# Prunoideae/MitoFlex

Measured on AMD Instinct MI355X. Metric: filtered reads/sec on 5 Gbp PE150 k=31; achieved HBM GB/s vs peak, higher is better.
Workload: dtype u64

## Files before the change

### mitoflex_amd/csrc/mf_api.cpp

```cpp
#include "../../include/mitofilter.h"
#include "mf_common.h"
#include "mf_host.h"
#include "mf_kernels.h"
#include "mf_pipeline.h"
#include "mf_synth.h"
#include "mf_coldtrace.h"
#include "mf_api_internal.h"
#include "mf_devingest.h"

#include <hip/hip_runtime.h>
#include <algorithm>
#include <atomic>
#include <chrono>
#include <map>
#include <mutex>
#include <stdarg.h>
#include <stdio.h>
#include <stdlib.h>
#include <string.h>
#include <sys/stat.h>
#include <string>
#include <thread>
#include <vector>

using namespace mf;

static thread_local std::string t_err;
const std::string &mf_thread_error() { return t_err; }
int fail(int code, const char *fmt, ...)
{
    char buf[1024];
    va_list ap; va_start(ap, fmt); vsnprintf(buf, sizeof buf, fmt, ap); va_end(ap);
    t_err = buf;
    return code;
}

static std::mutex g_ctx_mu;
static std::atomic<int> g_expect_files{0};
static std::map<int, DevCtx> g_ctx;

static int fake_devices()
{
#ifdef MF_TEST_HOOKS
    static const int n = [] { const char *v = getenv("MF_FAKE_DEVICES"); const int k = v ? atoi(v) : 0; return k > 0 && k <= 64 ? k : 0; }();
    return n;
#else
    return 0;
#endif
}
static int physical_count() { int n = 0; return hipGetDeviceCount(&n) == hipSuccess ? n : 0; }
int phys(int device) { const int n = physical_count(); return fake_devices() && n > 0 ? device % n : device; }

int get_ctx(int device, DevCtx **out, int lane)
{
    std::lock_guard<std::mutex> lk(g_ctx_mu);
    auto it = g_ctx.find(device + 4096 * lane);
    if (it != g_ctx.end()) { *out = &it->second; hipError_t e = hipSetDevice(phys(device)); if (e != hipSuccess) return fail(MF_E_HIP, "hipSetDevice(%d): %s", device, hipGetErrorString(e)); return MF_OK; }
    int n = 0;
    mf::cold_mark("get_ctx: a new device context");
    hipError_t e = hipGetDeviceCount(&n);
    mf::cold_mark("get_ctx: HIP runtime answered (initialised)");
    if (e != hipSuccess || n <= 0) return fail(MF_E_NO_DEVICE, "no HIP device visible (%s); libmitofilter_hip has no CPU fallback", e == hipSuccess ? "count=0" : hipGetErrorString(e));
    const int logical = fake_devices() ? fake_devices() : n;
    if (device < 0 || device >= logical) return fail(MF_E_ARG, "device %d out of range (have %d)", device, logical);
    const int pdev = phys(device);
    hipDeviceProp_t prop;
    HIPCHK(hipGetDeviceProperties(&prop, pdev));
    if (strncmp(prop.gcnArchName, "gfx950", 6) != 0)
        return fail(MF_E_NO_DEVICE, "device %d is %s; this library carries gfx950 (MI355X) code only", device, prop.gcnArchName);
    HIPCHK(hipSetDevice(pdev));
    DevCtx c; c.device = device; c.n_cu = prop.multiProcessorCount;
    HIPCHK(hipStreamCreateWithFlags(&c.stream, hipStreamNonBlocking));
    mf::cold_mark("get_ctx: stream made");
    g_ctx[device + 4096 * lane] = c;
    *out = &g_ctx[device + 4096 * lane];
    if (g_expect_files && lane == 0) mf::ingest_prefetch(device);
    return MF_OK;
}

static int ensure_pipeline_streams(DevCtx *c)
{
    { std::lock_guard<std::mutex> lk(g_ctx_mu); if (c->stream2) return MF_OK; }
    int lo = 0, hi = 0;
    hipStream_t s2 = nullptr, s3 = nullptr, s4 = nullptr;
    hipError_t e = hipDeviceGetStreamPriorityRange(&lo, &hi);
    if (e == hipSuccess) e = hipStreamCreateWithPriority(&s2, hipStreamNonBlocking, hi);
    if (e == hipSuccess) e = hipStreamCreateWithPriority(&s4, hipStreamNonBlocking, hi);
    if (e == hipSuccess) e = hipStreamCreateWithFlags(&s3, hipStreamNonBlocking);
    bool publish = e == hipSuccess;
    if (publish) {
        std::lock_guard<std::mutex> lk(g_ctx_mu);
        if (c->stream2) publish = false;
        else { c->stream3 = s3; c->stream4 = s4; c->stream2 = s2; }
    }
    if (!publish) { for (hipStream_t s : {s2, s4, s3}) if (s) (void)hipStreamDestroy(s); }
    if (e != hipSuccess) return fail(MF_E_HIP, "creating the streams of a pipelined call failed: %s", hipGetErrorString(e));
    return MF_OK;
}

struct TablesGuard {
    DevTables *t;
    ~TablesGuard() { if (t) t->release(); }
};
struct EventList {
    std::vector<hipEvent_t> ev;
    hipError_t create(size_t n) { ev.reserve(n); for (size_t i = 0; i < n; i++) { hipEvent_t e; hipError_t r = hipEventCreate(&e); if (r != hipSuccess) return r; ev.push_back(e); } return hipSuccess; }
    ~EventList() { for (hipEvent_t e : ev) hipEventDestroy(e); }
};

static int host_threads()
{
    const char *v = getenv("MF_HOST_THREADS");
    const int n = v && *v ? atoi(v) : (int)std::thread::hardware_concurrency();
    return n < 1 ? 1 : n;
}

static uint32_t env_u32(const char *name, uint32_t dflt)
{
    const char *v = getenv(name);
    return v && *v ? (uint32_t)strtoul(v, nullptr, 10) : dflt;
}

struct PassOptions {
    std::atomic<int> pass{0};
    std::atomic<int> adapt{1};
    std::atomic<int> finish_streams{0};
    std::atomic<int> screen_streams{2};
    std::atomic<int> split_pipe{1};
    std::atomic<int> exact_co{0};
    std::atomic<int> front{-1};
    std::atomic<int> front2_log2b{0};
    std::atomic<int> s8_finish{-1};
    std::atomic<int> canon{-1};
    std::atomic<int> front3_log2b{-1};
    std::atomic<int> depth_index{0};
};
static PassOptions g_opt;
static int set_option(const char *name, const char *value)
{
    const std::string n = name ? name : "", v = value ? value : "";
    if (n == "pass") { if (v == "" || v == "default") g_opt.pass = 0; else if (v == "split") g_opt.pass = 1; else if (v == "serial") g_opt.pass = 2; else return -1; return 0; }
    char *end = nullptr; const long x = strtol(v.c_str(), &end, 10);
    if (v.empty() || *end) return -1;
    if (n == "expect_files") g_expect_files = x != 0;
    else if (n == "short_lived") mf::ingest_short_lived(x != 0);
    else if (n == "adapt") g_opt.adapt = x != 0;
    else if (n == "finish_streams") { if (x < 0 || x > 2) return -1; g_opt.finish_streams = (int)x; }
    else if (n == "screen_streams") { if (x < 1 || x > 2) return -1; g_opt.screen_streams = (int)x; }
    else if (n == "split_pipe") g_opt.split_pipe = x != 0;
    else if (n == "exact_co") g_opt.exact_co = x != 0;
    else if (n == "front") { if (x < -1 || x > 4) return -1; g_opt.front = (int)x; }
    else if (n == "front2_log2b") { if (x != 0 && (x < 6 || x > 24)) return -1; g_opt.front2_log2b = (int)x; }
    else if (n == "s8_finish") { if (x < -1 || x > 1) return -1; g_opt.s8_finish = (int)x; }
    else if (n == "canon") { if (x < -1 || x > 1) return -1; g_opt.canon = (int)x; }
    else if (n == "front3_log2b") { if (x < -1 || (x > 0 && x < 6) || x > 27) return -1; g_opt.front3_log2b = (int)x; }
    else if (n == "depth_index") { if (x < 0 || x > 1) return -1; g_opt.depth_index = (int)x; }
    else return -1;
    return 0;
}
static void options_from_env_once()
{
    static const bool done = [] {
        const char *k = getenv("MF_ENV_KNOBS");
        if (k && k[0] == '1') {
            static const char *const pairs[][2] = {{"pass", "MF_PASS"}, {"adapt", "MF_ADAPT"}, {"finish_streams", "MF_FINISH_STREAMS"}, {"screen_streams", "MF_SCREEN_STREAMS"},
                                                   {"split_pipe", "MF_SPLIT_PIPE"}, {"exact_co", "MF_EXACT_CO"},
                                                   {"front", "MF_FRONT"}, {"front2_log2b", "MF_FRONT2_LOG2B"}, {"front3_log2b", "MF_FRONT3_LOG2B"}, {"canon", "MF_CANON"}, {"s8_finish", "MF_S8_FINISH"},
                                                   {"depth_index", "MF_DEPTH_INDEX"}};
            for (auto &p : pairs) { const char *v = getenv(p[1]); if (v && *v && set_option(p[0], v) != 0) fprintf(stderr, "libmitofilter_hip: %s=%s is not a value of option '%s' (ignored)\n", p[1], v, p[0]); }
        }
        return true;
    }();
    (void)done;
}
int depth_index_option() { return g_opt.depth_index.load(); }

int build_on_device(mf_kmerset *ks, int device, DevTables **out)
{
    std::lock_guard<std::mutex> lk(ks->mu);
    auto it = ks->dev.find(device);
    if (it != ks->dev.end()) { *out = &it->second; return MF_OK; }
    DevCtx *ctx; int rc = get_ctx(device, &ctx); if (rc) return rc;
    hipStream_t st = ctx->stream;
    if (ks->kind == MF_KIND_PROTEIN) {
        const ProtBaitHost &P = ks->pbait;
        DevTables T; TablesGuard guard{&T}; DevScratch tmp;
        uint8_t *d_aa = nullptr, *d_run = nullptr; unsigned long long *d_cnt = nullptr;
        HIPCHK(tmp.alloc(d_aa, P.aa.size())); HIPCHK(tmp.alloc(d_run, P.runlen.size()));
        HIPCHK(hipMemcpyAsync(d_aa, P.aa.data(), P.aa.size(), hipMemcpyHostToDevice, st));
        HIPCHK(hipMemcpyAsync(d_run, P.runlen.data(), P.runlen.size(), hipMemcpyHostToDevice, st));
        HIPCHK(dev_malloc(&T.keys, ks->slots * sizeof(uint64_t)));
        HIPCHK(hipMemsetAsync(T.keys, 0xFF, ks->slots * sizeof(uint64_t), st));
        HIPCHK(launch_build_ptable(d_aa, d_run, P.total, ks->k, T.keys, ks->slots, st));
        HIPCHK(dev_malloc(&T.kbloom, sizeof(uint32_t) << ks->kb_log2w));
        HIPCHK(hipMemsetAsync(T.kbloom, 0, sizeof(uint32_t) << ks->kb_log2w, st));
        HIPCHK(launch_build_pbits(T.keys, ks->slots, T.kbloom, ks->kb_log2w, st));
        HIPCHK(dev_malloc(&T.plut, sizeof ks->codon_lut));
        HIPCHK(hipMemcpyAsync(T.plut, ks->codon_lut, sizeof ks->codon_lut, hipMemcpyHostToDevice, st));
        HIPCHK(tmp.alloc(d_cnt, 16)); HIPCHK(hipMemsetAsync(d_cnt, 0, 16, st));
        HIPCHK(launch_count_keys(T.keys, ks->slots, 1, nullptr, 0, d_cnt, st));
        unsigned long long cnt[2] = {0, 0};
        HIPCHK(hipMemcpyAsync(cnt, d_cnt, 16, hipMemcpyDeviceToHost, st));
        HIPCHK(hipStreamSynchronize(st));
        T.n_keys = cnt[0];
        KmerSetView &V = T.view;
        V.k = ks->k; V.kw = 1; V.slot_mask = ks->slots - 1; V.keys = T.keys;
        V.kb_log2w = ks->kb_log2w; V.kbloom = T.kbloom; V.kb_co_log2w = ks->kb_log2w; V.kbloom_co = T.kbloom;
        V.prot = 1; V.kb_in_lds = ks->kb_in_lds ? 1u : 0u; V.plut = T.plut;
        ks->dev[device] = T; guard.t = nullptr;
        *out = &ks->dev[device];
        return MF_OK;
    }
    const BaitHost &B = ks->bait;
    DevTables T; TablesGuard guard{&T}; DevScratch tmp;
    uint32_t *d_words = nullptr; uint8_t *d_run = nullptr; uint32_t *d_pos = nullptr, *d_flag = nullptr;
    unsigned long long *d_cnt = nullptr;
    HIPCHK(tmp.alloc(d_words, B.words.size() * 4));
    HIPCHK(tmp.alloc(d_run, B.runlen.size()));
    HIPCHK(hipMemcpyAsync(d_words, B.words.data(), B.words.size() * 4, hipMemcpyHostToDevice, st));
    HIPCHK(hipMemcpyAsync(d_run, B.runlen.data(), B.runlen.size(), hipMemcpyHostToDevice, st));
    const size_t key_bytes = ks->slots * ks->kw * sizeof(uint64_t);
    HIPCHK(dev_malloc(&T.keys, key_bytes));
    HIPCHK(hipMemsetAsync(T.keys, 0xFF, key_bytes, st));
    if (ks->kw == 2) {
        if (B.total > 0xFFFFFFF0ull) return fail(MF_E_ARG, "bait longer than 2^32 bases is not supported for k > 32");
        HIPCHK(tmp.alloc(d_pos, ks->slots * 4));
        HIPCHK(hipMemsetAsync(d_pos, 0xFF, ks->slots * 4, st));
    }
    HIPCHK(tmp.alloc(d_flag, 4)); HIPCHK(hipMemsetAsync(d_flag, 0, 4, st));
    HIPCHK(tmp.alloc(d_cnt, 16)); HIPCHK(hipMemsetAsync(d_cnt, 0, 16, st));
    BaitView bv{d_words, B.total, d_run};
    HIPCHK(launch_build_table(bv, ks->k, ks->kw, T.keys, ks->slots, d_pos, st));
    if (ks->geom.s) {
        HIPCHK(dev_malloc(&T.bloom, ks->screen_words() * 4));
        HIPCHK(hipMemsetAsync(T.bloom, 0, ks->screen_words() * 4, st));
        HIPCHK(dev_malloc(&T.stab, (size_t)ks->stab_slots * 4));
        HIPCHK(hipMemsetAsync(T.stab, 0xFF, (size_t)ks->stab_slots * 4, st));
        if (ks->front_mode) {
            HIPCHK(dev_malloc(&T.front2, (size_t)16 << ks->f2_log2b));
            HIPCHK(hipMemsetAsync(T.front2, 0, (size_t)16 << ks->f2_log2b, st));
            if (ks->f3_log2b) {
                HIPCHK(dev_malloc(&T.front3, (size_t)16 << ks->f3_log2b));
                HIPCHK(hipMemsetAsync(T.front3, 0, (size_t)16 << ks->f3_log2b, st));
            }
        }
        if (ks->front_mode == 4) {
            HIPCHK(dev_malloc(&T.pre, sizeof(uint32_t) << ks->pre_log2w));
            HIPCHK(hipMemsetAsync(T.pre, 0, sizeof(uint32_t) << ks->pre_log2w, st));
        }
        HIPCHK(launch_build_screen(bv, ks->geom.s, T.bloom, ks->bloom_log2w, ks->stage2_log2w, T.stab, ks->stab_slots, d_flag,
                                   T.front2, ks->f2_log2b, T.front3, ks->f3_log2b, T.pre, ks->pre_log2w, ks->canon != 0, st));
    }
    HIPCHK(dev_malloc(&T.kbloom, sizeof(uint32_t) << ks->kb_log2w));
    HIPCHK(hipMemsetAsync(T.kbloom, 0, sizeof(uint32_t) << ks->kb_log2w, st));
    HIPCHK(launch_build_kbloom(T.keys, ks->slots, ks->kw, T.kbloom, ks->kb_log2w, st));
    if (ks->kb_log2w > KB_CO_LOG2W) {
        HIPCHK(dev_malloc(&T.kbloom_co, sizeof(uint32_t) << KB_CO_LOG2W));
        HIPCHK(hipMemsetAsync(T.kbloom_co, 0, sizeof(uint32_t) << KB_CO_LOG2W, st));
        HIPCHK(launch_build_kbloom(T.keys, ks->slots, ks->kw, T.kbloom_co, KB_CO_LOG2W, st));
    }
    HIPCHK(launch_count_keys(T.keys, ks->slots, ks->kw, T.stab, T.stab ? ks->stab_slots : 0, d_cnt, st));
    unsigned long long cnt[2] = {0, 0}; uint32_t flag = 0;
    HIPCHK(hipMemcpyAsync(cnt, d_cnt, 16, hipMemcpyDeviceToHost, st));
    HIPCHK(hipMemcpyAsync(&flag, d_flag, 4, hipMemcpyDeviceToHost, st));
    HIPCHK(hipStreamSynchronize(st));
    T.n_keys = cnt[0]; T.n_smers = cnt[1] + (flag ? 1 : 0);
    KmerSetView &V = T.view;
    V.k = ks->k; V.kw = ks->kw; V.slot_mask = ks->slots - 1; V.keys = T.keys;
    V.kb_log2w = ks->kb_log2w; V.kbloom = T.kbloom;
    V.kb_co_log2w = T.kbloom_co ? KB_CO_LOG2W : ks->kb_log2w; V.kbloom_co = T.kbloom_co ? T.kbloom_co : T.kbloom;
    V.s = ks->geom.s; V.stride = ks->geom.stride;
    V.smask = ks->geom.s >= 16 ? 0xFFFFFFFFu : ((1u << (2 * ks->geom.s)) - 1);
    V.bloom_log2w = ks->bloom_log2w; V.stage2_log2w = ks->stage2_log2w; V.bloom = T.bloom;
    V.stab_mask = ks->stab_slots ? ks->stab_slots - 1 : 0; V.stab = T.stab; V.stab_has_ones = flag;
    V.canon = (uint32_t)ks->canon;
    V.s8_finish = ks->s8_finish ? 1u : 0u;
    V.front_mode = ks->front_mode; V.f2_log2b = ks->f2_log2b; V.f3_log2b = ks->f3_log2b; V.front2 = T.front2; V.front3 = T.front3;
    V.pre_log2w = ks->pre_log2w; V.pre = T.pre;
    V.use_stab = (T.n_smers / 2 * STAGE2_K > ((uint64_t)32 << ks->stage2_log2w) * 7 / 10) ? 1u : 0u;
#ifdef MF_DEBUG_KNOBS
    if (getenv("MF_USE_STAB")) V.use_stab = 1u;
#endif
    ks->dev[device] = T; guard.t = nullptr;
    *out = &ks->dev[device];
    return MF_OK;
}

static int kmerset_new(const char *text, size_t len, int k, int device, mf_kmerset **out)
{
    if (!out) return fail(MF_E_ARG, "out is NULL");
    *out = nullptr;
    if (k < 11 || k > 63) return fail(MF_E_ARG, "k=%d out of range [11,63]", k);
    mf_kmerset *ks = new (std::nothrow) mf_kmerset();
    if (!ks) return fail(MF_E_NOMEM, "out of memory");
    ks->k = k; ks->kw = k > 32 ? 2 : 1;
    parse_bait_fasta(text, len, ks->bait);
    ks->n_windows = ks->bait.n_windows(k);
    ks->slots = table_slots_for(ks->n_windows);
    {
        uint32_t lg = 8;
        while (lg < 14 && (1ull << lg) < 2 * ks->n_windows) lg++;
        ks->kb_log2w = env_u32("MF_KBLOOM_LOG2W", lg);
        if (ks->kb_log2w < 8) ks->kb_log2w = 8;
        if (ks->kb_log2w > 15) ks->kb_log2w = 15;
    }
    ks->geom = screen_geom_for(k);
#ifdef MF_DEBUG_KNOBS
    if (getenv("MF_NO_SCREEN")) ks->geom = ScreenGeom{0, 0};
#endif
    if (ks->geom.s) {
        const uint64_t bound = 2 * ks->bait.n_swindows(ks->geom.s);
        uint32_t lg = 8;
        while (lg < 15 && (1ull << lg) < bound) lg++;
        ks->bloom_log2w = env_u32("MF_BLOOM_LOG2W", lg);
        if (ks->bloom_log2w < 8) ks->bloom_log2w = 8;
        if (ks->bloom_log2w > 15) ks->bloom_log2w = 15;
        uint32_t lg2 = 6;
        while (lg2 < 13 && (32ull << lg2) < 8 * bound) lg2++;
        ks->stage2_log2w = env_u32("MF_STAGE2_LOG2W", lg2);
        if (ks->stage2_log2w < 6) ks->stage2_log2w = 6;
        if (ks->stage2_log2w > 13) ks->stage2_log2w = 13;
        uint64_t ss = 1024; while (ss < 2 * bound) ss <<= 1;
        if (ss > (1ull << 31)) { delete ks; return fail(MF_E_ARG, "bait too large for the s-mer screen table"); }
        ks->stab_slots = (uint32_t)ss;
        options_from_env_once();
        uint64_t per_lds_block = bound >> (ks->bloom_log2w - 2);
        ks->s8_finish = ks->geom.stride == 8 && per_lds_block > 5;
        {
            const bool want = g_opt.canon < 0 ? per_lds_block > (ks->geom.stride == 8 ? 18u : 14u) : g_opt.canon == 1;
            ks->canon = !want ? 0 : ks->geom.s == 16 ? 1 : 2;
        }
        const uint64_t keys_bound = ks->canon ? bound / 2 : bound;
        per_lds_block = keys_bound >> (ks->bloom_log2w - 2);
        const uint64_t mode1_max = ks->geom.stride == 8 ? 18 : 26;
        int mode = per_lds_block <= 9 ? 0 : per_lds_block <= mode1_max ? 1 : 2;
        if (ks->geom.stride == 16 && per_lds_block > 5 && per_lds_block <= (ks->canon ? 12u : 14u)) mode = 3;
        if (mode == 2 && keys_bound <= (1u << 21)) mode = 4;
        if (g_opt.front >= 0) mode = g_opt.front;
        ks->front_mode = (uint32_t)mode;
        ks->pre_log2w = mode == 4 ? 15 : 0;
        if (mode) {
            uint32_t lg = 10;
            while (lg < FRONT2_MAX_LOG2B && (4ull << lg) < keys_bound) lg++;
            while (lg < FRONT2_MAX_LOG2B + 2 && (keys_bound >> lg) > 32) lg++;
            if (g_opt.front2_log2b > 0) lg = (uint32_t)g_opt.front2_log2b;
            ks->f2_log2b = lg;
            uint32_t lg3 = 0;
            if ((keys_bound >> lg) > 12) { lg3 = lg + 1; while (lg3 < 27 && (4ull << lg3) < keys_bound) lg3++; }
            if (g_opt.front3_log2b >= 0) lg3 = (uint32_t)g_opt.front3_log2b;
            ks->f3_log2b = (mode == 2 || mode == 4) ? lg3 : 0;
        }
    }
    DevTables *T; int rc = build_on_device(ks, device, &T);
    if (rc) { delete ks; return rc; }
    *out = ks;
    return MF_OK;
}

static int protset_new(const char *text, size_t len, int kp, int genetic_code, int device, mf_kmerset **out)
{
    if (!out) return fail(MF_E_ARG, "out is NULL");
    *out = nullptr;
    if (kp < 4 || kp > 12) return fail(MF_E_ARG, "peptide k=%d out of range [4,12]", kp);
    mf_kmerset *ks = new (std::nothrow) mf_kmerset();
    if (!ks) return fail(MF_E_NOMEM, "out of memory");
    ks->kind = MF_KIND_PROTEIN; ks->k = kp; ks->kw = 1; ks->genetic_code = genetic_code;
    if (!codon_lut_for(genetic_code, kp, ks->codon_lut)) { delete ks; return fail(MF_E_ARG, "genetic code %d is not supported (1, 2, 3, 4, 5, 9, 11, 13, 14, 21)", genetic_code); }
    parse_bait_protein(text, len, ks->pbait);
    ks->n_windows = ks->pbait.n_windows(kp);
    ks->slots = table_slots_for(ks->n_windows);
    {
        uint32_t lg = 8;
        while (lg < 14 && (1ull << lg) < 2 * ks->n_windows) lg++;
        ks->kb_in_lds = ks->n_windows <= (1u << 17);
        if (!ks->kb_in_lds) { lg = 15; while (lg < 24 && (32ull << lg) < 16 * ks->n_windows) lg++; }
        if (getenv("MF_KBLOOM_LOG2W")) {
            lg = env_u32("MF_KBLOOM_LOG2W", lg);
            if (lg < 8) lg = 8;
            if (lg > 24) lg = 24;
            ks->kb_in_lds = lg <= 14;
        }
        ks->kb_log2w = lg;
    }
    DevTables *T; int rc = build_on_device(ks, device, &T);
    if (rc) { delete ks; return rc; }
    *out = ks;
    return MF_OK;
}

extern "C" {

int mf_abi_version(void) { return MF_ABI_VERSION; }
const char *mf_last_error(void) { return t_err.c_str(); }

int mf_device_count(void)
{
    int n = 0;
    hipError_t e = hipGetDeviceCount(&n);
    if (e == hipErrorNoDevice) return 0;
    if (e != hipSuccess) return fail(MF_E_HIP, "hipGetDeviceCount: %s", hipGetErrorString(e));
    return n > 0 && fake_devices() ? fake_devices() : n;
}

int mf_device_name(int device, char *buf, size_t buflen)
{
    if (!buf || !buflen) return fail(MF_E_ARG, "bad buffer");
    hipDeviceProp_t prop;
    HIPCHK(hipGetDeviceProperties(&prop, phys(device)));
    snprintf(buf, buflen, "%s (%s, %d CUs)", prop.name, prop.gcnArchName, prop.multiProcessorCount);
    return MF_OK;
}

int mf_device_synchronize(int device)
{
    HIPCHK(hipSetDevice(phys(device)));
    HIPCHK(hipDeviceSynchronize());
    return MF_OK;
}

int mf_kmerset_build_from_text(const char *text, size_t len, int k, int device, mf_kmerset **out)
{
    if (!text && len) return fail(MF_E_ARG, "fasta_text is NULL");
    return kmerset_new(text ? text : "", len, k, device, out);
}

int mf_kmerset_build_from_fasta(const char *path, int k, int device, mf_kmerset **out)
{
    if (!path) return fail(MF_E_ARG, "fasta_path is NULL");
    std::vector<char> buf; std::string err;
    if (!slurp_file(path, buf, err)) return fail(MF_E_IO, "%s", err.c_str());
    return kmerset_new(buf.data(), buf.size(), k, device, out);
}

int mf_kmerset_build_protein_from_text(const char *text, size_t len, int kp, int genetic_code, int device, mf_kmerset **out)
{
    if (!text && len) return fail(MF_E_ARG, "protein_fasta_text is NULL");
    return protset_new(text ? text : "", len, kp, genetic_code, device, out);
}

int mf_kmerset_build_protein_from_fasta(const char *path, int kp, int genetic_code, int device, mf_kmerset **out)
{
    if (!path) return fail(MF_E_ARG, "protein_fasta_path is NULL");
    std::vector<char> buf; std::string err;
    if (!slurp_file(path, buf, err)) return fail(MF_E_IO, "%s", err.c_str());
    return protset_new(buf.data(), buf.size(), kp, genetic_code, device, out);
}

int mf_kmerset_info(const mf_kmerset *ks, mf_kmerset_info_t *info)
{
    if (!ks || !info) return fail(MF_E_ARG, "NULL argument");
    memset(info, 0, sizeof *info);
    info->k = ks->k; info->key_words = ks->kw; info->slots = ks->slots; info->n_windows = ks->n_windows;
    info->screen_s = ks->geom.s; info->screen_stride = ks->geom.stride;
    info->bloom_words = ks->geom.s ? (uint32_t)ks->screen_words() : 0; info->smer_slots = ks->stab_slots;
    if (!ks->dev.empty()) { info->n_keys = ks->dev.begin()->second.n_keys; info->n_smers = ks->dev.begin()->second.n_smers; }
    info->kind = ks->kind; info->genetic_code = ks->genetic_code;
    info->front_mode = ks->front_mode; info->front2_log2_blocks = ks->front_mode ? ks->f2_log2b : 0; info->front3_log2_blocks = ks->f3_log2b; info->canonical_screen = ks->canon ? 1u : 0u;
    return MF_OK;
}

int mf_kmerset_export(const mf_kmerset *ks_, int device, uint64_t *keys_out, size_t n_u64)
{
    mf_kmerset *ks = const_cast<mf_kmerset *>(ks_);
    if (!ks || !keys_out) return fail(MF_E_ARG, "NULL argument");
    if (n_u64 < ks->slots * ks->kw) return fail(MF_E_ARG, "keys_out too small: need %llu u64", (unsigned long long)(ks->slots * ks->kw));
    DevTables *T; int rc = build_on_device(ks, device, &T); if (rc) return rc;
    HIPCHK(hipMemcpy(keys_out, T->keys, ks->slots * ks->kw * sizeof(uint64_t), hipMemcpyDeviceToHost));
    return MF_OK;
}

int mf_kmerset_free(mf_kmerset *ks)
{
    if (!ks) return MF_OK;
    for (auto &kv : ks->dev) {
        if (hipSetDevice(phys(kv.first)) == hipSuccess) kv.second.release();
    }
    delete ks;
    return MF_OK;
}

}

void reads_release(mf_reads *r)
{
    if (!r) return;
    if (hipSetDevice(phys(r->device)) == hipSuccess) {
        hipFree(r->d_words); hipFree(r->d_offsets); hipFree(r->d_npos); hipFree(r->d_has_n);
        for (int i = 0; i < NSETS; i++) hipFree(r->d_cand[i]);
        for (int i = 0; i < NSETS; i++) {
            hipFree(r->d_bits[i]); hipFree(r->d_recs[i]); hipFree(r->d_rec_counts[i]); if (r->d_counters[i]) hipHostFree(r->d_counters[i]);
            if (r->ev_screen[i]) hipEventDestroy(r->ev_screen[i]);
            if (i < 2 && r->ev_call[i]) hipEventDestroy(r->ev_call[i]);
            if (r->ev_finish[i]) hipEventDestroy(r->ev_finish[i]);
        }
        hipFree(r->d_hits); hipFree(r->d_npos_blk); hipFree(r->d_off_blk);
        hipFree(r->d_alist); hipFree(r->d_assign); hipFree(r->d_apairs); hipFree(r->d_acnt);
        hipFree(r->d_rpos); hipFree(r->d_rtot); hipFree(r->d_rsum); hipFree(r->d_place); hipFree(r->d_score); hipFree(r->d_keep);
        hipFree(r->d_align); hipFree(r->d_awork);
    }
    delete r;
}

#define RCHK(call) do { hipError_t e_ = (call); if (e_ != hipSuccess) return fail(MF_E_HIP, "%s failed: %s", #call, hipGetErrorString(e_)); } while (0)
int reads_reserve(mf_reads *r, bool reuse, uint64_t n_words, uint64_t n_reads, uint32_t uniform_len, uint64_t npos_cap, DevCtx *ctx)
{
    const uint64_t padded = padded_words_for(n_words);
    RCHK(dev_reserve(r->d_words, r->cap_words, padded * 4, reuse));
    if (padded > n_words) RCHK(hipMemsetAsync(r->d_words + n_words, 0, (padded - n_words) * 4, ctx->stream));
    if (!uniform_len) RCHK(dev_reserve(r->d_offsets, r->cap_offsets, (n_reads + 1) * 8, reuse));
    RCHK(dev_reserve(r->d_npos, r->cap_npos, (npos_cap ? npos_cap : 1) * 8, reuse));
    return MF_OK;
}

int reads_finish(mf_reads *r, bool reuse, uint64_t n_words, uint64_t n_reads, uint64_t total_bases, uint32_t uniform_len, uint64_t n_npos, DevCtx *ctx)
{
    hipStream_t st = ctx->stream;
    const uint64_t padded = padded_words_for(n_words);
    if (n_npos >= 0xFFFFFFFFull) return fail(MF_E_ARG, "more than 2^32 invalid bases in one read set");
    const uint64_t n_blk = (total_bases >> NPOS_BLK_SHIFT) + 3;
    RCHK(dev_reserve(r->d_npos_blk, r->cap_npos_blk, n_blk * 4, reuse));
    RCHK(launch_build_npos_blk(r->d_npos, n_npos, n_blk, r->d_npos_blk, st));
    if (!uniform_len) {
        if (n_reads >= 0x7FFFFFFFull) return fail(MF_E_ARG, "more than 2^31 reads in one ragged read set");
        const uint64_t n_oblk = (total_bases >> OFF_BLK_SHIFT) + 2;
        RCHK(dev_reserve(r->d_off_blk, r->cap_off_blk, n_oblk * 8, reuse));
        RCHK(launch_build_off_blk(r->d_offsets, n_reads, n_oblk, r->d_off_blk, st));
    }
    r->bitmap_bytes = ((n_reads + 31) / 32 + 64) * 4;
    if (r->bitmap_bytes > r->cap_bitmap || !r->d_has_n) {
        size_t c[2 + NSETS] = {};
        uint32_t **bm[2 + NSETS] = {&r->d_has_n, &r->d_cand[0]};
        for (int i = 0; i < NSETS; i++) bm[2 + i] = &r->d_bits[i];
        size_t least = ~(size_t)0;
        for (int i = 0; i < 2 + NSETS; i++) {
            if (*bm[i]) { hipFree(*bm[i]); *bm[i] = nullptr; }
            RCHK(dev_reserve(*bm[i], c[i], r->bitmap_bytes, reuse));
            if (c[i] < least) least = c[i];
        }
        r->cap_bitmap = least;
        for (int i = 1; i < NSETS; i++) { hipFree(r->d_cand[i]); r->d_cand[i] = nullptr; }
    }
    RCHK(hipMemsetAsync(r->d_has_n, 0, r->bitmap_bytes, st));
    RCHK(hipMemsetAsync(r->d_cand[0], 0, r->bitmap_bytes, st));
    r->cand_clean[0] = true;
    for (int i = 1; i < NSETS; i++) r->cand_clean[i] = false;
    for (int i = 0; i < NSETS; i++) {
        if (!r->d_counters[i]) RCHK(hipHostMalloc(reinterpret_cast<void **>(&r->d_counters[i]), TallyLayout::bytes(), hipHostMallocDefault));
        memset(r->d_counters[i], 0, TallyLayout::bytes());
        RCHK(hipMemsetAsync(r->d_bits[i], 0, r->bitmap_bytes, st));
        if (!r->ev_screen[i]) RCHK(hipEventCreate(&r->ev_screen[i]));
        if (!r->ev_finish[i]) RCHK(hipEventCreate(&r->ev_finish[i]));
    }
    r->cur = 0;
    ReadsView &V = r->v;
    V = ReadsView{};
    V.words = r->d_words; V.n_words = n_words; V.n_vec = (padded - 16) / 4;
    V.offsets = uniform_len ? nullptr : r->d_offsets; V.off_blk = uniform_len ? nullptr : r->d_off_blk; V.uniform_len = uniform_len; V.n_reads = n_reads; V.total_bases = total_bases;
    V.len_magic = uniform_len > 1 ? ~0ULL / uniform_len + 1 : 0;
    V.len_magic32 = (uniform_len > 1 && uniform_len <= 4096) ? 0xFFFFFFFFu / uniform_len + 1 : 0;
    V.npos = r->d_npos; V.n_npos = n_npos; V.npos_blk = r->d_npos_blk; V.has_n = r->d_has_n;
    {
        uint64_t grid = screen_grid_for(V, ctx->n_cu, 4), cap = screen_rec_cap_for(V, ctx->n_cu, 4);
        for (int key : {8, 16}) { const uint64_t g2 = screen_grid_for(V, ctx->n_cu, key), c2 = screen_rec_cap_for(V, ctx->n_cu, key); if (g2 * c2 > grid * cap) cap = (g2 * c2 + grid - 1) / (grid ? grid : 1); }
        size_t c0 = r->cap_recs, c1 = r->cap_rec_counts;
        RCHK(dev_reserve(r->d_recs[0], c0, (grid * cap ? grid * cap : 1) * 16, reuse));
        RCHK(dev_reserve(r->d_rec_counts[0], c1, (grid ? grid : 1) * 4, reuse));
        if (c0 != r->cap_recs || c1 != r->cap_rec_counts)
            for (int i = 1; i < NSETS; i++) { hipFree(r->d_recs[i]); hipFree(r->d_rec_counts[i]); r->d_recs[i] = nullptr; r->d_rec_counts[i] = nullptr; }
        r->cap_recs = c0; r->cap_rec_counts = c1;
    }
    RCHK(launch_mark_has_n(V, r->d_has_n, st));
    RCHK(hipStreamSynchronize(st));
    return MF_OK;
}

static int reads_fill(mf_reads *r, bool reuse, const uint32_t *words, uint64_t n_words, bool already_padded, const uint64_t *offsets,
                      uint64_t n_reads, uint64_t total_bases, uint32_t uniform_len, const uint64_t *npos, uint64_t n_npos,
                      DevCtx *ctx)
{
    hipStream_t st = ctx->stream;
    int rc = reads_reserve(r, reuse, n_words, n_reads, uniform_len, n_npos, ctx);
    if (rc) return rc;
    const uint64_t copied = already_padded ? padded_words_for(n_words) : n_words;
    if (copied) RCHK(hipMemcpyAsync(r->d_words, words, copied * 4, hipMemcpyHostToDevice, st));
    if (!uniform_len) RCHK(hipMemcpyAsync(r->d_offsets, offsets, (n_reads + 1) * 8, hipMemcpyHostToDevice, st));
    if (n_npos) RCHK(hipMemcpyAsync(r->d_npos, npos, n_npos * 8, hipMemcpyHostToDevice, st));
    return reads_finish(r, reuse, n_words, n_reads, total_bases, uniform_len, n_npos, ctx);
}
#undef RCHK

static int reads_upload(const uint32_t *words, uint64_t n_words, bool already_padded, const uint64_t *offsets, uint64_t n_reads,
                        uint64_t total_bases, uint32_t uniform_len, const uint64_t *npos, uint64_t n_npos, int device,
                        mf_reads **out)
{
    DevCtx *ctx; int rc = get_ctx(device, &ctx); if (rc) return rc;
    mf_reads *r = new (std::nothrow) mf_reads();
    if (!r) return fail(MF_E_NOMEM, "out of memory");
    r->device = device;
    rc = reads_fill(r, false, words, n_words, already_padded, offsets, n_reads, total_bases, uniform_len, npos, n_npos, ctx);
    if (rc) { reads_release(r); return rc; }
    *out = r;
    return MF_OK;
}

extern "C" {

int mf_reads_from_packed(const uint32_t *words, const uint64_t *offsets, uint64_t n_reads,
                         const uint64_t *npos, uint64_t n_npos, int device, mf_reads **out)
{
    if (!out) return fail(MF_E_ARG, "out is NULL");
    *out = nullptr;
    if (!offsets) return fail(MF_E_ARG, "offsets is NULL");
    if (n_npos && !npos) return fail(MF_E_ARG, "npos is NULL");
    if (offsets[0] != 0) return fail(MF_E_ARG, "offsets[0] must be 0");
    for (uint64_t i = 0; i < n_reads; i++) if (offsets[i + 1] < offsets[i]) return fail(MF_E_ARG, "offsets must be non-decreasing");
    for (uint64_t i = 1; i < n_npos; i++) if (npos[i] <= npos[i - 1]) return fail(MF_E_ARG, "npos must be strictly ascending");
    const uint64_t total = offsets[n_reads];
    if (n_npos && npos[n_npos - 1] >= total) return fail(MF_E_ARG, "npos entry beyond the last base");
    const uint64_t n_words = (total + 15) / 16;
    if (n_words && !words) return fail(MF_E_ARG, "words is NULL");
    return reads_upload(words, n_words, false, offsets, n_reads, total, detect_uniform_len(offsets, n_reads), npos, n_npos, device, out);
}

int mf_reads_from_fastq(const char *path, int device, mf_reads **out)
{
    if (!out || !path) return fail(MF_E_ARG, "NULL argument");
    *out = nullptr;
    std::vector<char> buf; std::string err;
    if (!slurp_file(path, buf, err)) return fail(MF_E_IO, "%s", err.c_str());
    std::vector<FqRec> recs; parse_fastq(buf.data(), buf.size(), recs);
    PackedHost P; pack_records(recs.data(), recs.size(), host_threads(), P);
    return reads_upload(P.words.data(), P.n_words, true, P.offsets.data(), recs.size(), P.offsets.back(), P.uniform_len,
                        P.npos.data(), P.npos.size(), device, out);
}

int mf_reads_synth(uint64_t n_reads, uint32_t read_len, uint64_t seed, const char *bait_text, size_t bait_len,
                   uint32_t mito_ppm, uint32_t sub_ppm, uint32_t n_read_ppm, uint32_t n_base_ppm, int device, mf_reads **out,
                   uint32_t **host_words_out, uint64_t *host_n_words_out, uint64_t **host_npos_out, uint64_t *host_n_npos_out)
{
    return mf_reads_synth_ex(n_reads, read_len, seed, bait_text, bait_len, mito_ppm, sub_ppm, n_read_ppm, n_base_ppm, 0, 0, 0, device, out,
                             host_words_out, host_n_words_out, host_npos_out, host_n_npos_out);
}

int mf_reads_synth_ex(uint64_t n_reads, uint32_t read_len, uint64_t seed, const char *bait_text, size_t bait_len,
                      uint32_t mito_ppm, uint32_t sub_ppm, uint32_t n_read_ppm, uint32_t n_base_ppm,
                      uint32_t msat_ppm, uint32_t numt_ppm, uint32_t numt_div_ppm, int device, mf_reads **out,
                      uint32_t **host_words_out, uint64_t *host_n_words_out, uint64_t **host_npos_out, uint64_t *host_n_npos_out)
{
    if (!out) return fail(MF_E_ARG, "out is NULL");
    *out = nullptr;
    if (read_len == 0) return fail(MF_E_ARG, "read_len must be > 0");
    BaitHost B; parse_bait_fasta(bait_text ? bait_text : "", bait_text ? bait_len : 0, B);
    SynthOut S;
    std::string err;
    SynthExtra extra; extra.msat_ppm = msat_ppm; extra.numt_ppm = numt_ppm; extra.numt_div_ppm = numt_div_ppm;
    if (!synth_reads(n_reads, read_len, seed, B, mito_ppm, sub_ppm, n_read_ppm, n_base_ppm,
                     host_threads(), S, err, extra)) return fail(MF_E_ARG, "%s", err.c_str());
    int rc = reads_upload(S.words.data(), S.n_words, true, nullptr, n_reads, n_reads * (uint64_t)read_len, read_len,
                          S.npos.data(), S.npos.size(), device, out);
    if (rc) return rc;
    if (host_words_out) {
        *host_words_out = (uint32_t *)malloc(S.words.size() * 4);
        if (!*host_words_out) return fail(MF_E_NOMEM, "out of memory");
        memcpy(*host_words_out, S.words.data(), S.words.size() * 4);
        if (host_n_words_out) *host_n_words_out = S.n_words;
    }
    if (host_npos_out) {
        *host_npos_out = (uint64_t *)malloc((S.npos.size() + 1) * 8);
        if (!*host_npos_out) return fail(MF_E_NOMEM, "out of memory");
        memcpy(*host_npos_out, S.npos.data(), S.npos.size() * 8);
        if (host_n_npos_out) *host_n_npos_out = S.npos.size();
    }
    return MF_OK;
}

void mf_free_host(void *p) { free(p); }

int mf_reads_info(const mf_reads *r, mf_reads_info_t *info)
{
    if (!r || !info) return fail(MF_E_ARG, "NULL argument");
    info->n_reads = r->v.n_reads; info->total_bases = r->v.total_bases; info->n_invalid = r->v.n_npos;
    info->uniform_len = r->v.uniform_len; info->device = r->device;
    return MF_OK;
}

int mf_reads_free(mf_reads *r) { reads_release(r); return MF_OK; }

}

static uint64_t algorithmic_bytes(const ReadsView &V) { return (2 * V.total_bases + 7) / 8 + (V.n_reads + 7) / 8; }

static unsigned long long *tally_of(mf_reads *r, int set) { return r->tally_override ? r->tally_override : r->d_counters[set]; }
static int clean_cand(mf_reads *r, int q, hipStream_t st)
{
    if (!r->d_cand[q]) { size_t c = 0; HIPCHK(dev_reserve(r->d_cand[q], c, r->cap_bitmap, false)); r->cand_clean[q] = false; }
    if (!r->cand_clean[q]) { HIPCHK(hipMemsetAsync(r->d_cand[q], 0, r->bitmap_bytes, st)); r->cand_clean[q] = true; }
    return MF_OK;
}
static int enqueue_pass(mf_reads *r, const KmerSetView &S, uint32_t thr, int mode, bool count_all, DevCtx *ctx, hipEvent_t *ev, bool overlap, bool more = false)
{
    options_from_env_once();
    const PassKnobs knobs{g_opt.pass, g_opt.finish_streams, g_opt.screen_streams, g_opt.split_pipe, g_opt.exact_co, g_opt.s8_finish};
    const PassInputs in{(int)S.prot, (int)S.s, (int)S.stride, (int)S.kw, (int)S.k, (int)S.s8_finish, thr, mode, count_all, overlap, more, r->fb, r->flip, r->cur, NSETS};
    const PassPlan P = plan_pass(knobs, in);
    const int n_cu = ctx->n_cu, q = P.q; const bool finish = P.kind == PassKind::FINISH;
    hipStream_t const streams[] = {ctx->stream, ctx->stream2, ctx->stream3, ctx->stream4}, ss = streams[(int)P.screen_on], sf = streams[(int)P.later_on];
    const hipEvent_t done = P.two_streams ? r->ev_finish[q] : nullptr;
    KernelTiming tm[3]; const KernelTiming *t0 = nullptr, *t1 = nullptr, *t2 = nullptr;
    if (ev) { for (int i = 0; i < 3; i++) tm[i] = KernelTiming{ev[2 * i], ev[2 * i + 1]}; t0 = &tm[0]; t1 = &tm[1]; t2 = &tm[2]; }
    if (P.screen) {
        size_t c0 = 0, c1 = 0;
        if (!r->d_recs[q]) { HIPCHK(dev_reserve(r->d_recs[q], c0, r->cap_recs, false)); HIPCHK(dev_reserve(r->d_rec_counts[q], c1, r->cap_rec_counts, false)); }
        if (P.wait_prev_finish) HIPCHK(hipStreamWaitEvent(ss, r->ev_finish[q], 0));
        if (P.needs_cand && !finish) { const int rc = clean_cand(r, q, ss); if (rc) return rc; }
        KernelTiming scr_done{nullptr, r->ev_screen[q]};
        HIPCHK(launch_screen(r->v, S, r->d_recs[q], r->d_rec_counts[q], n_cu, ss, t0 ? t0 : (P.two_streams ? &scr_done : nullptr),
                             P.screen_clears_bits ? r->d_bits[q] : nullptr, P.screen_clears_bits ? ((r->v.n_reads + 31) / 32 + 3) / 4 : 0));
        if (P.two_streams) { if (t0) HIPCHK(hipEventRecord(r->ev_screen[q], ss)); HIPCHK(hipStreamWaitEvent(sf, r->ev_screen[q], 0)); }
    }
#ifdef MF_DEBUG_KNOBS
    static const uint32_t nofin = env_u32("MF_NO_FINISH", 0);
    if (finish && nofin) { if (done) HIPCHK(hipEventRecord(done, sf)); } else
#endif
    if (P.kind == PassKind::PROTEIN) HIPCHK(launch_pfilter(r->v, S, thr, count_all, r->d_bits[P.q_out], r->d_hits, tally_of(r, P.q_out), n_cu, sf, t2));
    else if (finish) {
        if (P.exact_behind_finish) { const int rc = clean_cand(r, q, sf); if (rc) return rc; }
        uint32_t *const cand = P.exact_behind_finish ? r->d_cand[q] : nullptr;
        HIPCHK(launch_finish(r->v, S, r->d_recs[q], r->d_rec_counts[q], r->d_bits[q], tally_of(r, q), n_cu, sf, t2, cand ? nullptr : done, cand));
        if (cand) HIPCHK(launch_exact(r->v, S, cand, 1, false, r->d_bits[q], nullptr, tally_of(r, q) + TallyLayout::region(2), n_cu, sf, nullptr, P.exact_coresident, done, true));
    } else {
        uint32_t *const cand = P.needs_cand ? r->d_cand[q] : nullptr;
        if (P.screen) HIPCHK(launch_mark(r->v, S, r->d_recs[q], r->d_rec_counts[q], cand, n_cu, sf, t1));
        HIPCHK(launch_exact(r->v, S, cand, thr, count_all, r->d_bits[P.q_out], P.kind == PassKind::ONE_STREAM ? r->d_hits : nullptr, tally_of(r, P.q_out), n_cu, sf, t2, P.exact_coresident, done));
    }
    r->flip = P.flip; r->cur = P.cur; r->sample_pass = P.sample_pass;
    return MF_OK;
}

int filter_common(const mf_kmerset *ks_, const mf_reads *reads_, uint32_t thr, int mode, uint32_t *out_bits,
                  uint32_t *hits_out, int steps, mf_filter_stats_t *stats, uint64_t *pass_per_step)
{
    mf_kmerset *ks = const_cast<mf_kmerset *>(ks_);
    mf_reads *r = const_cast<mf_reads *>(reads_);
    if (!ks || !r) return fail(MF_E_ARG, "NULL handle");
    if (thr < 1) return fail(MF_E_ARG, "threshold must be >= 1");
    if (mode != MF_MODE_SCREENED && mode != MF_MODE_EXHAUSTIVE) return fail(MF_E_ARG, "bad mode %d", mode);
    if (steps < 1) return fail(MF_E_ARG, "steps must be >= 1");
    static const bool trace = getenv("MF_TRACE") != nullptr;
    const auto tp0 = std::chrono::steady_clock::now();
    auto lap = [&](const char *what) { if (trace) fprintf(stderr, "[mf trace] %-10s %8.1f us\n", what, std::chrono::duration<double, std::micro>(std::chrono::steady_clock::now() - tp0).count()); };
    DevCtx *ctx; int rc = get_ctx(r->device, &ctx, r->lane); if (rc) return rc;
    DevTables *T; rc = build_on_device(ks, r->device, &T); if (rc) return rc;
    hipStream_t st = ctx->stream;
    const bool count_all = hits_out != nullptr;
    lap("setup");
    if (count_all) {
        HIPCHK(dev_reserve(r->d_hits, r->cap_hits, (r->v.n_reads ? r->v.n_reads : 1) * 4, false));
        HIPCHK(hipMemsetAsync(r->d_hits, 0, (r->v.n_reads ? r->v.n_reads : 1) * 4, st));
    }
    int stride = steps <= 8 ? 1 : (int)env_u32("MF_EVENT_STRIDE", 8);
    if (stride < 1) stride = 1;
    const int n_sampled = stride > steps ? 0 : (steps + stride - 1) / stride;
    EventList events;
    HIPCHK(events.create((size_t)n_sampled * 6));
    hipEvent_t *ev = events.ev.data();
    for (int i = 0; i < 2; i++) if (!r->ev_call[i]) HIPCHK(hipEventCreate(&r->ev_call[i]));
    const hipEvent_t e_begin = r->ev_call[0], e_end = r->ev_call[1];
    lap("events");
    const bool pipelined = steps > 1;
    if (pipelined) { rc = ensure_pipeline_streams(ctx); if (rc) return rc; }
    HIPCHK(hipEventRecord(e_begin, st));
    if (pipelined) HIPCHK(hipStreamWaitEvent(ctx->stream3, e_begin, 0));
    struct PinnedTmp { unsigned long long *p = nullptr; ~PinnedTmp() { if (p) (void)hipHostFree(p); } } all_tallies;
    if (pass_per_step) {
        HIPCHK(hipHostMalloc(reinterpret_cast<void **>(&all_tallies.p), (size_t)steps * TallyLayout::bytes(), hipHostMallocDefault));
        memset(all_tallies.p, 0, (size_t)steps * TallyLayout::bytes());
    }
    struct OverrideReset { mf_reads *r; ~OverrideReset() { r->tally_override = nullptr; } } override_reset{r};
    for (int i = 0; i < steps; i++) {
        if (pass_per_step) r->tally_override = all_tallies.p + (size_t)i * TallyLayout::words();
        rc = enqueue_pass(r, T->view, thr, mode, count_all, ctx, n_sampled && i % stride == 0 ? &ev[(size_t)(i / stride) * 6] : nullptr, pipelined, i + 1 < steps);
        if (rc) return rc;
    }
    lap("enqueued");
    for (int i = 0; i < NSETS; i++) HIPCHK(hipStreamWaitEvent(st, r->ev_finish[i], 0));
    HIPCHK(hipEventRecord(e_end, st));
    const int regions = r->sample_pass ? TallyLayout::REGIONS : 1;
    const unsigned long long *part = pass_per_step ? all_tallies.p + (size_t)(steps - 1) * TallyLayout::words() : r->d_counters[r->cur];
    if (out_bits) HIPCHK(hipMemcpyAsync(out_bits, r->d_bits[r->cur], ((r->v.n_reads + 31) / 32) * 4, hipMemcpyDeviceToHost, st));
    if (hits_out && r->v.n_reads) HIPCHK(hipMemcpyAsync(hits_out, r->d_hits, r->v.n_reads * 4, hipMemcpyDeviceToHost, st));
    lap("copies");
    HIPCHK(hipStreamSynchronize(st));
    lap("synced");
    const TallyLayout::Totals cnt = TallyLayout::sum(part, regions);
    for (int s = 0; pass_per_step && s < steps; s++) pass_per_step[s] = TallyLayout::sum(all_tallies.p + (size_t)s * TallyLayout::words(), regions).pass;
    if (g_opt.adapt && !T->view.prot && mode == MF_MODE_SCREENED && T->view.s > 0) r->fb = adapt_after_call(r->fb, r->sample_pass, cnt.cand, r->v.n_reads);
    if (stats) {
        memset(stats, 0, sizeof *stats);
        float tot = 0, scr = 0, mrk = 0, exa = 0, t;
        HIPCHK(hipEventElapsedTime(&tot, e_begin, e_end));
        const bool prot = T->view.prot != 0, screened = !prot && mode == MF_MODE_SCREENED && T->view.s > 0;
        for (int i = 0; i < n_sampled; i++) {
            hipEvent_t *e = &ev[(size_t)i * 6];
            auto span = [&](hipEvent_t a, hipEvent_t b) { t = 0; if (hipEventElapsedTime(&t, a, b) != hipSuccess) { (void)hipGetLastError(); t = 0; } return t; };
            if (screened) { scr += span(e[0], e[1]); mrk += span(e[2], e[3]); }
            exa += span(e[4], e[5]);
        }
        stats->n_reads = r->v.n_reads; stats->n_pass = cnt.pass;
        stats->n_candidates = (mode == MF_MODE_SCREENED && T->view.s > 0) ? cnt.cand : r->v.n_reads;
        stats->ms_total = tot / steps;
        if (n_sampled) { stats->ms_screen = scr / n_sampled; stats->ms_mark = mrk / n_sampled; stats->ms_exact = exa / n_sampled; }
        stats->algorithmic_bytes = algorithmic_bytes(r->v);
    }
    lap("stats");
    return MF_OK;
}

extern "C" {

int mf_filter(const mf_kmerset *ks, const mf_reads *reads, uint32_t threshold, int mode,
              uint32_t *out_bits, uint32_t *hits_out, mf_filter_stats_t *stats)
{
    if (!out_bits && !hits_out && !stats) return fail(MF_E_ARG, "nothing to return: out_bits, hits_out and stats are all NULL");
    return filter_common(ks, reads, threshold, mode, out_bits, hits_out, 1, stats);
}

int mf_filter_resident(const mf_kmerset *ks, const mf_reads *reads, uint32_t threshold, int mode, int steps,
                       mf_filter_stats_t *stats)
{
    return filter_common(ks, reads, threshold, mode, nullptr, nullptr, steps, stats);
}

int mf_filter_resident_passes(const mf_kmerset *ks, const mf_reads *reads, uint32_t threshold, int mode, int steps,
                              uint64_t *n_pass_per_step, mf_filter_stats_t *stats)
{
    if (!n_pass_per_step) return fail(MF_E_ARG, "n_pass_per_step is NULL");
    return filter_common(ks, reads, threshold, mode, nullptr, nullptr, steps, stats, n_pass_per_step);
}

int mf_filter_packed(const mf_kmerset *ks, int device, const uint32_t *words, const uint64_t *offsets, uint64_t n_reads,
                     const uint64_t *npos, uint64_t n_npos, uint32_t threshold, uint32_t *out_bits)
{
    if (!out_bits) return fail(MF_E_ARG, "out_bits is NULL");
    mf_reads *r = nullptr;
    int rc = mf_reads_from_packed(words, offsets, n_reads, npos, n_npos, device, &r);
    if (rc) return rc;
    rc = filter_common(ks, r, threshold, MF_MODE_SCREENED, out_bits, nullptr, 1, nullptr);
    reads_release(r);
    return rc;
}

}

static thread_local mf_ingest_stats_t t_ingest_stats;
static thread_local bool t_ingest_stats_valid = false;
static void publish_ingest_stats(const IngestStats &is)
{
    mf_ingest_stats_t &o = t_ingest_stats;
    memset(&o, 0, sizeof o);
    o.path = MF_INGEST_PATH_DEVICE; o.n_devices = is.n_devices; o.consumers = is.consumers;
    o.input_bytes = is.input_bytes; o.text_bytes = is.text_bytes; o.records = is.records;
    o.seconds = is.seconds; o.decode_busy_seconds = is.decode_busy_seconds;
    o.pool_bytes_peak = is.pool_bytes_peak; o.device_bytes_peak = is.device_bytes_peak;
    o.chunks = is.chunks; o.chunks_linked = is.chunks_linked; o.gaps = is.gaps; o.gap_bytes = is.gap_bytes;
    t_ingest_stats_valid = true;
}

int filter_fastq_files_on(mf_kmerset *ks, const char *fq1, const char *fq2, const char *out1, const char *out2,
                          uint32_t threshold, int pair_mode, const int *devices, int n_devices, uint64_t *kept, uint64_t *total, PassReport *report)
{
    if (!ks || !fq1 || !out1) return fail(MF_E_ARG, "NULL argument");
    if ((fq2 == nullptr) != (out2 == nullptr)) return fail(MF_E_ARG, "fq2 and out2 must be given together");
    if (pair_mode != MF_PAIR_EITHER && pair_mode != MF_PAIR_BOTH) return fail(MF_E_ARG, "bad pair_mode %d", pair_mode);
    if (threshold < 1) return fail(MF_E_ARG, "threshold must be >= 1");
    const int have = mf_device_count();
    if (have <= 0) return fail(MF_E_NO_DEVICE, "no HIP device visible; libmitofilter_hip has no CPU fallback");
    if (!devices || n_devices < 1) return fail(MF_E_ARG, "empty device list");
    for (int i = 0; i < n_devices; i++) {
        if (devices[i] < 0 || devices[i] >= have) return fail(MF_E_ARG, "device %d out of range (have %d)", devices[i], have);
        for (int j = 0; j < i; j++) if (devices[j] == devices[i]) return fail(MF_E_ARG, "device %d listed twice", devices[i]);
    }

    {
        const char *ing = getenv("MF_INGEST");
        const bool force = ing && strcmp(ing, "device") == 0, any_gz = has_gz_ext(fq1) || (fq2 && has_gz_ext(fq2));
        bool big_plain = false;
        if (!any_gz && fq1) {
            struct stat sb; uint64_t sum = 0; bool regular = true;
            for (const char *f : {fq1, fq2}) if (f) { if (stat(f, &sb) == 0 && S_ISREG(sb.st_mode)) sum += (uint64_t)sb.st_size; else regular = false; }
            const char *mn = getenv("MF_INGEST_PLAIN_MIN_MB");
            big_plain = regular && sum > 0 && sum >= (mn && *mn ? strtoull(mn, nullptr, 10) : 0) << 20;
        }
        if (!(ing && strcmp(ing, "host") == 0) && (force || any_gz || big_plain)) {
            std::string derr; IngestStats is;
            const int drc = run_device_ingest(ks, fq1, fq2, out1, out2, threshold, pair_mode == MF_PAIR_BOTH, devices, n_devices, kept, total, derr, &is, report);
            if (drc == MF_OK) {
                publish_ingest_stats(is);
                return MF_OK;
            }
            if (drc != MF_DEVINGEST_DECLINED) return fail(drc, "%s", derr.c_str());
            if (report) report->restart();
            if (getenv("MF_PIPE_TIMING")) fprintf(stderr, "[mf device ingest] declined%s%s: the host pipeline takes the input\n", derr.empty() ? "" : ": ", derr.c_str());
        }
    }
    for (int i = 1; i < n_devices; i++)
        if (devices[i] != devices[0] + i) return fail(MF_E_ARG, "the host pipeline (plain files, pipes, BGZF) takes a run of consecutive devices; got %d after %d", devices[i], devices[i - 1]);
    const int dev_base = devices[0];
    const int hw = (int)std::thread::hardware_concurrency();
    int pack_threads = hw - 4 - n_devices; if (pack_threads < 1) pack_threads = 1; if (pack_threads > 64) pack_threads = 64;
    pack_threads = (int)env_u32("MF_PACK_THREADS", (uint32_t)pack_threads);
    if (pack_threads < 1) pack_threads = 1;
    const uint64_t batch_reads = env_u32("MF_BATCH_READS", 2000000);
    set_dma_allocator([](size_t bytes) -> void * { void *p = nullptr; return hipHostMalloc(&p, bytes, hipHostMallocPortable) == hipSuccess ? p : nullptr; },
                      [](void *p) { (void)hipHostFree(p); });
    struct DmaScope { ~DmaScope() { set_dma_allocator(nullptr, nullptr); } } dma_scope;
    const int lanes = (int)env_u32("MF_WORKERS_PER_DEVICE", 2) < 1 ? 1 : (int)env_u32("MF_WORKERS_PER_DEVICE", 2);
    const int n_workers = n_devices * lanes;
    std::vector<mf_reads *> arena((size_t)n_workers, nullptr);
    if (report) report->held.assign((size_t)n_workers, nullptr);
    BatchFilterFn fn = [ks, threshold, n_devices, dev_base, report, &arena](int worker, const PackedHost &P, uint64_t n, std::vector<uint32_t> &bits, std::string &err) -> int {
        bits.assign((n + 31) / 32 + 1, 0);
        if (report) report->held[(size_t)worker] = nullptr;
        if (n == 0) return MF_OK;
        const int device = dev_base + worker % n_devices, lane = worker / n_devices;
        DevCtx *ctx; int rc = get_ctx(device, &ctx, lane);
        if (rc == MF_OK && !arena[worker]) {
            arena[worker] = new (std::nothrow) mf_reads();
            if (!arena[worker]) rc = fail(MF_E_NOMEM, "out of memory"); else { arena[worker]->device = device; arena[worker]->lane = lane; }
        }
        if (rc == MF_OK)
            rc = reads_fill(arena[worker], true, P.words.data(), P.n_words, true, P.offsets.data(), n, P.offsets[n], P.uniform_len,
                            P.npos.data(), P.npos.size(), ctx);
        if (rc == MF_OK) rc = filter_common(ks, arena[worker], threshold, MF_MODE_SCREENED, bits.data(), nullptr, 1, nullptr);
        if (rc != MF_OK) err = t_err;
        else if (report) report->held[(size_t)worker] = arena[worker];
        return rc;
    };
    PipelineStats ps; std::string perr;
    const auto t_pipe0 = std::chrono::steady_clock::now();
    const int rc = run_fastq_pipeline(fq1, fq2, out1, out2, pair_mode == MF_PAIR_BOTH, n_workers, pack_threads, batch_reads, fn, ps, perr, report);
    {
        mf_ingest_stats_t &o = t_ingest_stats;
        memset(&o, 0, sizeof o);
        o.path = MF_INGEST_PATH_HOST; o.n_devices = n_devices; o.records = ps.total * (fq2 ? 2 : 1);
        o.seconds = std::chrono::duration<double>(std::chrono::steady_clock::now() - t_pipe0).count();
        t_ingest_stats_valid = rc == MF_OK;
    }
    {
        const auto t0 = std::chrono::steady_clock::now();
        for (mf_reads *a : arena) reads_release(a);
        if (getenv("MF_PIPE_TIMING"))
            fprintf(stderr, "[mf pipeline] device buffers released in %.3f s\n", std::chrono::duration<double>(std::chrono::steady_clock::now() - t0).count());
    }
    if (rc != MF_OK) return fail(rc, "%s", perr.c_str());
    if (kept) *kept = ps.kept;
    if (total) *total = ps.total;
    return MF_OK;
}

extern "C" {

int mf_filter_fastq_files(mf_kmerset *ks, const char *fq1, const char *fq2, const char *out1, const char *out2,
                          uint32_t threshold, int pair_mode, int n_devices, uint64_t *kept, uint64_t *total)
{
    const int have = mf_device_count();
    if (have <= 0) return fail(MF_E_NO_DEVICE, "no HIP device visible; libmitofilter_hip has no CPU fallback");
    if (n_devices < 1) n_devices = 1;
    if (n_devices > have) n_devices = have;
    std::vector<int> devs((size_t)n_devices);
    for (int i = 0; i < n_devices; i++) devs[(size_t)i] = i;
    return filter_fastq_files_on(ks, fq1, fq2, out1, out2, threshold, pair_mode, devs.data(), n_devices, kept, total, nullptr);
}

int mf_filter_fastq_files_on(mf_kmerset *ks, const char *fq1, const char *fq2, const char *out1, const char *out2,
                             uint32_t threshold, int pair_mode, const int *devices, int n_devices, uint64_t *kept, uint64_t *total)
{
    return filter_fastq_files_on(ks, fq1, fq2, out1, out2, threshold, pair_mode, devices, n_devices, kept, total, nullptr);
}

int mf_set_option(const char *name, const char *value)
{
    options_from_env_once();
    if (set_option(name, value) != 0) return fail(MF_E_ARG, "unknown option or value: %s=%s (options: pass=default|split|serial, adapt=0|1, finish_streams=0|1|2, screen_streams=1|2, split_pipe=0|1, exact_co=0|1, front=-1|0|1|2|3|4, canon=-1|0|1, s8_finish=-1|0|1, front2_log2b=0|6..24, front3_log2b=-1|0|6..27, expect_files=0|1, short_lived=0|1, depth_index=0|1)", name ? name : "(null)", value ? value : "(null)");
    return MF_OK;
}

int mf_last_ingest_stats(mf_ingest_stats_t *out)
{
    if (!out) return fail(MF_E_ARG, "NULL argument");
    if (!t_ingest_stats_valid) return fail(MF_E_ARG, "no file-level call has succeeded on this thread");
    *out = t_ingest_stats;
    return MF_OK;
}

int mf_release_cached(uint64_t *bytes)
{
    const size_t n = mf::release_cached_device_memory(true);
    if (bytes) *bytes = n;
    return MF_OK;
}

int mf_h2d_bandwidth(int device, size_t bytes, int reps, double *gb_per_s)
{
    if (!gb_per_s || !bytes || reps < 1) return fail(MF_E_ARG, "bad argument");
    DevCtx *ctx; int rc = get_ctx(device, &ctx); if (rc) return rc;
    void *h = nullptr, *d = nullptr; hipEvent_t e0 = nullptr, e1 = nullptr;
    struct Free { void *&h, *&d; hipEvent_t &e0, &e1; ~Free() { if (h) (void)hipHostFree(h); if (d) (void)hipFree(d); if (e0) (void)hipEventDestroy(e0); if (e1) (void)hipEventDestroy(e1); } } fr{h, d, e0, e1};
    HIPCHK(hipHostMalloc(&h, bytes, hipHostMallocDefault));
    memset(h, 0x5A, bytes);
    HIPCHK(dev_malloc(&d, bytes));
    HIPCHK(hipEventCreate(&e0)); HIPCHK(hipEventCreate(&e1));
    double best = 0;
    for (int i = 0; i <= reps; i++) {
        HIPCHK(hipEventRecord(e0, ctx->stream));
        HIPCHK(hipMemcpyAsync(d, h, bytes, hipMemcpyHostToDevice, ctx->stream));
        HIPCHK(hipEventRecord(e1, ctx->stream));
        HIPCHK(hipEventSynchronize(e1));
        float ms = 0; HIPCHK(hipEventElapsedTime(&ms, e0, e1));
        if (i && ms > 0) best = std::max(best, (double)bytes / (ms * 1e-3) / 1e9);
    }
    *gb_per_s = best;
    return MF_OK;
}

}

struct QualDevice {
    const int device;
    DevCtx *ctx = nullptr; hipStream_t st = nullptr;
    struct Scratch { void *p = nullptr; size_t cap = 0; } d_text, d_recs, d_cnt, d_hash, d_flags;
    struct Table {
        unsigned long long *keys = nullptr, *first = nullptr;
        hipError_t release()
        {
            if (!keys && !first) return hipSuccess;
            const hipError_t a = hipFree(keys), b = hipFree(first);
            keys = first = nullptr;
            return a != hipSuccess ? a : b;
// ... 128 lines not shown
```

### mitoflex_amd/csrc/mf_api_internal.h

```cpp
#pragma once
#include "../../include/mitofilter.h"
#include "mf_common.h"
#include "mf_host.h"
#include "mf_kernels.h"
#include "mf_assign.h"
#include "mf_place.h"
#include "mf_align_launch.h"
#include <hip/hip_runtime.h>
#include <algorithm>
#include <map>
#include <mutex>
#include <string>
#include <vector>

struct DevCtx { int device = -1; hipStream_t stream = nullptr, stream2 = nullptr, stream3 = nullptr, stream4 = nullptr; int n_cu = 0; };

int fail(int code, const char *fmt, ...);
const std::string &mf_thread_error();
int phys(int device);
int get_ctx(int device, DevCtx **out, int lane = 0);
#define HIPCHK(call)                                                                                  \
    do { hipError_t e_ = (call);                                                                      \
         if (e_ != hipSuccess) return fail(MF_E_HIP, "%s failed: %s (%s:%d)", #call, hipGetErrorString(e_), __FILE__, __LINE__); \
    } while (0)

namespace mf { size_t release_cached_device_memory(bool all); }
inline hipError_t dev_malloc(void **p, size_t bytes)
{
    hipError_t e = hipMalloc(p, bytes);
    if (e == hipErrorOutOfMemory) {
        (void)hipGetLastError();
        if (mf::release_cached_device_memory(false)) e = hipMalloc(p, bytes);
        if (e != hipSuccess) (void)hipGetLastError();
    }
    return e;
}
template <class T> inline hipError_t dev_malloc(T **p, size_t bytes) { return dev_malloc(reinterpret_cast<void **>(p), bytes); }

template <class T> inline hipError_t dev_reserve(T *&p, size_t &cap, size_t bytes, bool slack)
{
    if (bytes <= cap && p) return hipSuccess;
    if (p) { hipError_t e = hipFree(p); p = nullptr; cap = 0; if (e != hipSuccess) return e; }
    const size_t want = slack ? bytes + bytes / 4 + 4096 : (bytes ? bytes : 16);
    hipError_t e = dev_malloc(&p, want);
    if (e == hipSuccess) cap = want;
    return e;
}


struct DevTables {
    uint64_t *keys = nullptr;
    uint32_t *bloom = nullptr, *stab = nullptr, *kbloom = nullptr, *kbloom_co = nullptr, *plut = nullptr;
    uint32_t *front2 = nullptr, *front3 = nullptr, *pre = nullptr;
    mf::KmerSetView view{};
    uint64_t n_keys = 0, n_smers = 0;
    uint32_t *owner = nullptr;
    uint32_t *gowner = nullptr;
    uint32_t *rep = nullptr, *pos_rep = nullptr; mf::DepthItem *ditems = nullptr; uint32_t n_ditems = 0; uint64_t dcnt_n = 0;
    mf::Anchor *anchor = nullptr; uint64_t *place_starts = nullptr; bool place_built = false;
    uint32_t *pile_words = nullptr; uint8_t *pile_runlen = nullptr; uint32_t *pile_valid = nullptr; bool pile_built = false;
    uint64_t pile_words_n = 0, pile_valid_n = 0;
    template <class T> static hipError_t drop(T *&p) { const hipError_t e = hipFree(p); p = nullptr; return e; }
    void release()
    {
        drop(keys); drop(bloom); drop(stab); drop(kbloom); drop(kbloom_co); drop(plut); drop(front2); drop(front3); drop(pre);
        drop(owner); drop(gowner); drop(rep); drop(pos_rep); drop(ditems);
        drop(anchor); drop(place_starts); place_built = false;
        drop(pile_words); drop(pile_runlen); drop(pile_valid); pile_built = false;
    }
};
struct mf_kmerset {
    int k = 0, kw = 1;
    int kind = MF_KIND_NUCLEOTIDE, genetic_code = 0;
    mf::ProtBaitHost pbait;
    uint32_t codon_lut[256] = {0};
    bool kb_in_lds = true;
    mf::BaitHost bait;
    uint64_t n_windows = 0, slots = 0;
    mf::ScreenGeom geom{0, 0};
    uint32_t bloom_log2w = 0, stage2_log2w = 0, stab_slots = 0, kb_log2w = 0;
    uint32_t front_mode = 0, f2_log2b = 0, f3_log2b = 0, pre_log2w = 0;
    int canon = 0;
    bool s8_finish = false;
    size_t screen_words() const { return ((size_t)1 << bloom_log2w) + ((size_t)1 << stage2_log2w); }
    std::vector<uint32_t> rec_group;
    std::vector<std::string> group_names;
    std::mutex mu;
    std::map<int, DevTables> dev;
    const std::vector<std::string> &names() const { return kind == MF_KIND_PROTEIN ? pbait.names : bait.names; }
    uint32_t n_records() const { return (uint32_t)names().size(); }
    uint32_t n_groups() const { return rec_group.empty() ? n_records() : (uint32_t)group_names.size(); }
    const std::string &group_name(uint64_t i) const { return rec_group.empty() ? names()[i] : group_names[i]; }
    const std::vector<uint64_t> &rec_len() const { return kind == MF_KIND_PROTEIN ? pbait.rec_len : bait.rec_len; }
    uint64_t positions() const { return kind == MF_KIND_PROTEIN ? pbait.total : bait.total; }
};

struct DevScratch {
    std::vector<void *> bufs;
    template <class T> hipError_t alloc(T *&p, size_t bytes) { hipError_t e = dev_malloc(&p, bytes); if (e == hipSuccess) bufs.push_back(p); return e; }
    template <class T> T *release(T *p) { bufs.erase(std::remove(bufs.begin(), bufs.end(), (void *)p), bufs.end()); return p; }
    ~DevScratch() { for (void *p : bufs) hipFree(p); }
};
int build_on_device(mf_kmerset *ks, int device, DevTables **out);
int depth_index_option();

#ifndef MF_NSETS
#define MF_NSETS 3
#endif
constexpr int NSETS = MF_NSETS;
struct mf_reads {
    int device = 0, lane = 0;
    mf::ReadsView v{};
    uint32_t *d_words = nullptr; uint64_t *d_offsets = nullptr, *d_npos = nullptr;
    uint32_t *d_has_n = nullptr, *d_hits = nullptr, *d_npos_blk = nullptr; uint64_t *d_off_blk = nullptr;
    uint32_t *d_cand[NSETS] = {}, *d_bits[NSETS] = {};
    void *d_recs[NSETS] = {}; uint32_t *d_rec_counts[NSETS] = {};
    unsigned long long *d_counters[NSETS] = {};
    hipEvent_t ev_screen[NSETS] = {}, ev_finish[NSETS] = {};
    hipEvent_t ev_call[2] = {};
    bool cand_clean[NSETS] = {}, sample_pass = false;
    mf::PassFeedback fb;
    int cur = 0, flip = 0;
    unsigned long long *tally_override = nullptr;
    size_t bitmap_bytes = 0;
    uint32_t *d_alist = nullptr, *d_assign = nullptr; uint64_t *d_apairs = nullptr; unsigned long long *d_acnt = nullptr;
    size_t cap_alist = 0, cap_assign = 0, cap_apairs = 0, cap_acnt = 0;
    unsigned long long *d_rtot = nullptr, *d_rsum = nullptr; void *d_rpos = nullptr;
    size_t cap_rtot = 0, cap_rsum = 0, cap_rpos = 0;
    uint32_t *rpos_u32() const { return static_cast<uint32_t *>(d_rpos); }
    mf::PlaceOut *d_place = nullptr; size_t cap_place = 0;
    mf::ScoreOut *d_score = nullptr; size_t cap_score = 0;
    uint32_t *d_keep = nullptr; size_t cap_keep = 0;
    mf::AlignOut *d_align = nullptr; size_t cap_align = 0;
    unsigned long long *d_awork = nullptr; size_t cap_awork = 0;
    size_t cap_words = 0, cap_offsets = 0, cap_npos = 0, cap_bitmap = 0, cap_recs = 0, cap_rec_counts = 0, cap_hits = 0, cap_npos_blk = 0, cap_off_blk = 0;
};


void reads_release(mf_reads *r);
int reads_reserve(mf_reads *r, bool reuse, uint64_t n_words, uint64_t n_reads, uint32_t uniform_len, uint64_t npos_cap, DevCtx *ctx);
int reads_finish(mf_reads *r, bool reuse, uint64_t n_words, uint64_t n_reads, uint64_t total_bases, uint32_t uniform_len, uint64_t n_npos, DevCtx *ctx);
int filter_common(const mf_kmerset *ks, const mf_reads *reads, uint32_t thr, int mode, uint32_t *out_bits, uint32_t *hits_out, int steps,
                  mf_filter_stats_t *stats, uint64_t *pass_per_step = nullptr);
namespace mf { struct PassReport; }
int filter_fastq_files_on(mf_kmerset *ks, const char *fq1, const char *fq2, const char *out1, const char *out2,
                          uint32_t threshold, int pair_mode, const int *devices, int n_devices, uint64_t *kept, uint64_t *total, mf::PassReport *report);
```

### mitoflex_amd/csrc/mf_kernels.h

```cpp
#pragma once
#include <hip/hip_runtime.h>
#include "mf_common.h"
#include "mf_kernels_cfg.h"
#include "mf_passplan.h"

namespace mf {

struct BaitView {
    const uint32_t *words;
    uint64_t        total;
    const uint8_t  *runlen;
};

struct KernelTiming { hipEvent_t start, stop; };

uint64_t screen_grid_for(const ReadsView &R, int n_cu, int stride);
uint64_t screen_rec_cap_for(const ReadsView &R, int n_cu, int stride);
hipError_t launch_screen(const ReadsView &R, const KmerSetView &S, void *recs, uint32_t *rec_counts, int n_cu, hipStream_t st,
                         const KernelTiming *tm = nullptr, uint32_t *clear = nullptr, uint64_t clear_vec4 = 0);
hipError_t launch_finish(const ReadsView &R, const KmerSetView &S, const void *recs, const uint32_t *rec_counts, uint32_t *bits,
                         unsigned long long *partials, int n_cu, hipStream_t st, const KernelTiming *tm = nullptr, hipEvent_t done = nullptr, uint32_t *cand = nullptr);
hipError_t launch_mark(const ReadsView &R, const KmerSetView &S, const void *recs, const uint32_t *rec_counts, uint32_t *cand, int n_cu,
                       hipStream_t st, const KernelTiming *tm = nullptr);
hipError_t launch_exact(const ReadsView &R, const KmerSetView &S, uint32_t *cand, uint32_t thr, bool count_all,
                        uint32_t *out_bits, uint32_t *hits_out, unsigned long long *counters, int n_cu, hipStream_t st,
                        const KernelTiming *tm = nullptr, bool coresident = false, hipEvent_t done = nullptr, bool merge = false);
hipError_t launch_build_kbloom(const uint64_t *keys, uint64_t slots, int kw, uint32_t *kbloom, uint32_t kb_log2w, hipStream_t st);
hipError_t launch_build_table(const BaitView &B, int k, int kw, uint64_t *keys, uint64_t slots, uint32_t *postab_scratch,
                              hipStream_t st);
hipError_t launch_build_screen(const BaitView &B, int s, uint32_t *bloom, uint32_t log2w, uint32_t log2w2, uint32_t *stab,
                               uint32_t stab_slots, uint32_t *has_ones, uint32_t *front2, uint32_t f2_log2b, uint32_t *front3, uint32_t f3_log2b,
                               uint32_t *pre, uint32_t pre_log2w, bool canon, hipStream_t st);
hipError_t launch_count_keys(const uint64_t *keys, uint64_t slots, int kw, const uint32_t *stab, uint64_t stab_slots,
                             unsigned long long *out2, hipStream_t st);
struct QualRec { uint32_t s_off, s_len, q_off, q_len; };
hipError_t launch_qualscan(const uint8_t *text, const QualRec *recs, uint32_t n, uint32_t quality, uint32_t *n_count, uint32_t *bad_count,
                           uint64_t *hashes , hipStream_t st);
hipError_t launch_dedup(const uint64_t *hashes, const uint8_t *alive, uint32_t n, uint64_t base, unsigned long long *keys,
                        unsigned long long *first, uint64_t slots, unsigned long long *zero_idx, unsigned long long *n_keys, uint8_t *dup,
                        hipStream_t st);
hipError_t launch_dedup_rehash(const unsigned long long *old_keys, const unsigned long long *old_first, uint64_t old_slots,
                               unsigned long long *keys, unsigned long long *first, uint64_t slots, hipStream_t st);
hipError_t launch_build_ptable(const uint8_t *aa, const uint8_t *runlen, uint64_t total, int kp, uint64_t *keys, uint64_t slots,
                               hipStream_t st);
hipError_t launch_build_pbits(const uint64_t *keys, uint64_t slots, uint32_t *kbloom, uint32_t kb_log2w, hipStream_t st);
hipError_t launch_pfilter(const ReadsView &R, const KmerSetView &S, uint32_t thr, bool count_all, uint32_t *out_bits,
                          uint32_t *hits_out, unsigned long long *counters, int n_cu, hipStream_t st, const KernelTiming *tm = nullptr);
hipError_t launch_build_npos_blk(const uint64_t *npos, uint64_t n_npos, uint64_t n_blk, uint32_t *blk, hipStream_t st);
hipError_t launch_build_off_blk(const uint64_t *offsets, uint64_t n_reads, uint64_t n_blk, uint64_t *blk, hipStream_t st);
hipError_t launch_mark_has_n(const ReadsView &R, uint32_t *has_n, hipStream_t st);

}
```

### mitoflex_amd/csrc/mf_kernels.hip

```cpp
#include "mf_common.h"
#include "mf_kernels.h"
#include "mf_keys_dev.h"
#include <hip/hip_ext.h>
#include <stdlib.h>
#include <algorithm>
#include <atomic>

namespace mf {

__device__ __forceinline__ uint64_t lower_bound_u64(const uint64_t *__restrict__ a, uint64_t n, uint64_t v)
{
    uint64_t lo = 0, hi = n;
    while (lo < hi) { uint64_t mid = (lo + hi) >> 1; if (a[mid] < v) lo = mid + 1; else hi = mid; }
    return lo;
}

__device__ __forceinline__ uint64_t read_holding(const ReadsView &R, uint64_t g, uint32_t s, uint64_t *start = nullptr, uint64_t *end = nullptr)
{
    if (g + s > R.total_bases) return ~0ULL;
    if (R.uniform_len) {
        uint64_t r = R.uniform_len > 1 ? __umul64hi(g, R.len_magic) : g;
        uint64_t off = g - r * R.uniform_len;
        if (start) *start = g - off;
        if (end) *end = g - off + R.uniform_len;
        return off + s <= R.uniform_len ? r : ~0ULL;
    }
    return offblk_lookup(R.off_blk, R.offsets, R.n_reads, g, s, start, end);
}

__device__ __forceinline__ bool stab_contains(const KmerSetView &S, uint32_t sm)
{
    if (sm == EMPTY32) return S.stab_has_ones != 0;
    uint32_t slot = smer_hash(sm) & S.stab_mask;
    uint32_t e = S.stab[slot];
    while (e < sm) { slot = (slot + 1) & S.stab_mask; e = S.stab[slot]; }
    return e == sm;
}


typedef uint32_t u32x4 __attribute__((ext_vector_type(4)));
typedef __attribute__((address_space(3))) uint32_t lds_u32;
typedef __attribute__((address_space(3))) unsigned long long lds_u64;
__device__ __forceinline__ uint32_t lds_ld(const lds_u32 *p) { return __hip_atomic_load(p, __ATOMIC_RELAXED, __HIP_MEMORY_SCOPE_WORKGROUP); }
__device__ __forceinline__ void lds_st(lds_u32 *p, uint32_t v) { __hip_atomic_store(p, v, __ATOMIC_RELAXED, __HIP_MEMORY_SCOPE_WORKGROUP); }
__device__ __forceinline__ unsigned long long lds_ld(const lds_u64 *p) { return __hip_atomic_load(p, __ATOMIC_RELAXED, __HIP_MEMORY_SCOPE_WORKGROUP); }
__device__ __forceinline__ void lds_st(lds_u64 *p, unsigned long long v) { __hip_atomic_store(p, v, __ATOMIC_RELAXED, __HIP_MEMORY_SCOPE_WORKGROUP); }
__device__ __forceinline__ uint32_t lds_add(lds_u32 *p, uint32_t v) { return __hip_atomic_fetch_add(p, v, __ATOMIC_RELAXED, __HIP_MEMORY_SCOPE_WORKGROUP); }
#define MF_COMPILER_FENCE() __atomic_signal_fence(__ATOMIC_SEQ_CST)

template <int BYTE>
__device__ __forceinline__ uint32_t lshl_by_byte(uint32_t amt, uint32_t data)
{
    uint32_t r;
    if (BYTE == 0) return data << (amt & 31u);
    if (BYTE == 1) asm("v_lshlrev_b32_sdwa %0, %1, %2 dst_sel:DWORD dst_unused:UNUSED_PAD src0_sel:BYTE_1 src1_sel:DWORD" : "=v"(r) : "v"(amt), "v"(data));
    if (BYTE == 2) asm("v_lshlrev_b32_sdwa %0, %1, %2 dst_sel:DWORD dst_unused:UNUSED_PAD src0_sel:BYTE_2 src1_sel:DWORD" : "=v"(r) : "v"(amt), "v"(data));
    if (BYTE == 3) asm("v_lshlrev_b32_sdwa %0, %1, %2 dst_sel:DWORD dst_unused:UNUSED_PAD src0_sel:BYTE_3 src1_sel:DWORD" : "=v"(r) : "v"(amt), "v"(data));
    return r;
}

__device__ __forceinline__ uint32_t canon16(uint32_t x)
{
    const uint32_t y = __brev(~x);
    const uint32_t rc = (0xAAAAAAAAu & (y << 1)) | (0x55555555u & (y >> 1));
    return x < rc ? x : rc;
}
template <int CANON>
__device__ __forceinline__ uint32_t canon_key(uint32_t x, uint32_t smask, uint32_t rc_shift)
{
    if (CANON == 0) return x;
    if (CANON == 1) return canon16(x);
    const uint32_t y = __brev(~x);
    const uint32_t rc = ((0xAAAAAAAAu & (y << 1)) | (0x55555555u & (y >> 1))) >> rc_shift;
    const uint32_t xm = x & smask;
    return xm < rc ? xm : rc;
}

struct __attribute__((aligned(16))) ScreenRec { uint32_t chunk, tid, hitmask, pad; };

template <int SPW, int U, int CANON = 0>
__global__ void __launch_bounds__(1024)
screen_kernel(ReadsView R, KmerSetView S, ScreenRec *__restrict__ recs, uint32_t rec_cap, uint32_t *__restrict__ rec_counts,
              uint4 *__restrict__ clear, uint64_t clear_vec4)
{
    extern __shared__ uint4 s_tab4[];
    const uint32_t nb4 = (1u << S.bloom_log2w) >> 2;
    uint32_t &s_nrec = *reinterpret_cast<uint32_t *>(s_tab4 + nb4);
    const u32x4 *__restrict__ w4 = reinterpret_cast<const u32x4 *>(R.words);
    const uint64_t chunk = (uint64_t)blockDim.x * U;
    const uint64_t n_chunks = R.n_vec / chunk;
    const uint32_t idx_lo = stage1_index_lo(S.s, S.bloom_log2w), idx_bits = S.bloom_log2w - 2;
    const uint64_t cstep = gridDim.x;
    ScreenRec *__restrict__ my_recs = recs + (size_t)blockIdx.x * rec_cap;

    auto load = [&](uint64_t c, u32x4 (&d)[U], uint32_t (&x)[U]) {
#pragma unroll
        for (int u = 0; u < U; u++) {
            const uint64_t v = c * chunk + (uint64_t)u * blockDim.x + threadIdx.x;
            d[u] = __builtin_nontemporal_load(&w4[v]);
            if (SPW == 2) x[u] = R.words[4 * v + 4];
        }
    };
    auto stage1 = [&](uint64_t c, const u32x4 (&d)[U], const uint32_t (&x)[U]) {
        uint32_t hitmask = 0;
#pragma unroll
        for (int u = 0; u < U; u++) {
            const uint32_t wv[5] = {d[u].x, d[u].y, d[u].z, d[u].w, SPW == 2 ? x[u] : 0u};
#pragma unroll
            for (int q = 0; q < 4; q++) {
#pragma unroll
                for (int j = 0; j < SPW; j++) {
                    static_assert(CANON != 1 || SPW == 1, "sixteen-base samples come with stride 16");
                    const uint32_t raw = (SPW == 1 || j == 0) ? wv[q] : alignbit(wv[q + 1], wv[q], 16u);
                    const uint32_t sm = canon_key<CANON>(raw, S.smask, 32u - 2u * (uint32_t)S.s);
                    const uint32_t h = bloom_hash(sm);
                    const uint4 blk = s_tab4[__builtin_amdgcn_ubfe(h, idx_lo, idx_bits)];
                    const uint32_t t = lshl_by_byte<0>(sm, blk.x) & lshl_by_byte<1>(sm, blk.y) & lshl_by_byte<2>(sm, blk.z) & lshl_by_byte<1>(h, blk.w);
                    hitmask = alignbit(hitmask, t, 31);
                }
            }
        }
        if (hitmask) {
            const uint32_t slot = atomicAdd(&s_nrec, 1u);
            ScreenRec rec; rec.chunk = (uint32_t)c; rec.tid = threadIdx.x; rec.hitmask = hitmask; rec.pad = 0;
            my_recs[slot] = rec;
        }
    };

    u32x4 a[U], b[U]; uint32_t ax[U], bx[U];
    uint64_t c = blockIdx.x;
    if (c < n_chunks) load(c, a, ax);
    {
        const uint4 z = make_uint4(0, 0, 0, 0);
        for (uint64_t i = (uint64_t)blockIdx.x * blockDim.x + threadIdx.x; i < clear_vec4; i += cstep * blockDim.x) clear[i] = z;
        const uint4 *__restrict__ src = reinterpret_cast<const uint4 *>(S.bloom);
        for (uint32_t i = threadIdx.x; i < nb4; i += blockDim.x) s_tab4[i] = src[i];
        if (threadIdx.x == 0) s_nrec = 0;
    }
    __syncthreads();
    if (c < n_chunks) for (;;) {
        if (c + cstep >= n_chunks) { stage1(c, a, ax); break; }
        load(c + cstep, b, bx);
        stage1(c, a, ax);
        c += cstep;
        if (c + cstep >= n_chunks) { stage1(c, b, bx); break; }
        load(c + cstep, a, ax);
        stage1(c, b, bx);
        c += cstep;
    }
    __syncthreads();
    if (threadIdx.x == 0) rec_counts[blockIdx.x] = s_nrec;
}

constexpr int S2_QCAP = 64;
constexpr size_t S2_LDS_EXTRA = 16 + (size_t)(SCREEN_BLOCK / 64) * (64 * 4 + S2_QCAP * 8);

__device__ __forceinline__ uint32_t lds_or(lds_u32 *p, uint32_t v) { return __hip_atomic_fetch_or(p, v, __ATOMIC_RELAXED, __HIP_MEMORY_SCOPE_WORKGROUP); }
__device__ __forceinline__ uint32_t lds_xchg(lds_u32 *p, uint32_t v) { return __hip_atomic_exchange(p, v, __ATOMIC_RELAXED, __HIP_MEMORY_SCOPE_WORKGROUP); }
__device__ __forceinline__ uint32_t block_test(uint32_t sm, uint32_t h, const uint4 blk)
{
    return lshl_by_byte<0>(sm, blk.x) & lshl_by_byte<1>(sm, blk.y) & lshl_by_byte<2>(sm, blk.z) & lshl_by_byte<1>(h, blk.w);
}

template <int SPW, int U, bool LDSF, int G = 8, bool PRE = false, int CANON = 0>
__global__ void __launch_bounds__(1024, G == 8 ? 4 : 8)
screen2_kernel(ReadsView R, KmerSetView S, ScreenRec *__restrict__ recs, uint32_t rec_cap, uint32_t *__restrict__ rec_counts,
               uint4 *__restrict__ clear, uint64_t clear_vec4)
{
    extern __shared__ uint4 s_tab4[];
    constexpr int NS = U * 4 * SPW;
    const uint32_t nb4 = LDSF ? (1u << S.bloom_log2w) >> 2 : PRE ? (1u << S.pre_log2w) >> 2 : 0u;
    uint32_t &s_nrec = *reinterpret_cast<uint32_t *>(s_tab4 + nb4);
    const uint32_t lane = threadIdx.x & 63, wid = threadIdx.x >> 6;
    const lds_u32 *s_pre = (const lds_u32 *)reinterpret_cast<const uint32_t *>(s_tab4);
    const uint32_t pre_lo = PRE ? pre_index_lo(S.s, S.pre_log2w) : 0u, pre_bits = PRE ? S.pre_log2w + 5 : 0u;
    lds_u32 *s_ver = (lds_u32 *)(reinterpret_cast<uint32_t *>(s_tab4 + nb4 + 1)) + wid * 64;
    lds_u32 *s_qsm = (lds_u32 *)(reinterpret_cast<uint32_t *>(s_tab4 + nb4 + 1 + (SCREEN_BLOCK / 64) * 16)) + wid * (2 * S2_QCAP);
    lds_u32 *s_qid = s_qsm + S2_QCAP;
    const u32x4 *__restrict__ w4 = reinterpret_cast<const u32x4 *>(R.words);
    const uint4 *__restrict__ f2 = reinterpret_cast<const uint4 *>(S.front2);
    const uint4 *__restrict__ f3 = reinterpret_cast<const uint4 *>(S.front3);
    const uint64_t chunk = (uint64_t)blockDim.x * U;
    const uint64_t n_chunks = R.n_vec / chunk;
    const uint32_t idx_lo = LDSF ? stage1_index_lo(S.s, S.bloom_log2w) : 0u, idx_bits = LDSF ? S.bloom_log2w - 2 : 0u;
    const uint32_t lo2 = stage1_index_lo(S.s, S.f2_log2b + 2), b2 = S.f2_log2b;
    const uint32_t lo3 = stage1_index_lo(S.s, S.f3_log2b + 2), b3 = S.f3_log2b;
    const uint64_t cstep = gridDim.x;
    ScreenRec *__restrict__ my_recs = recs + (size_t)blockIdx.x * rec_cap;

    auto load = [&](uint64_t c, u32x4 (&d)[U], uint32_t (&x)[U]) {
#pragma unroll
        for (int u = 0; u < U; u++) {
            const uint64_t v = c * chunk + (uint64_t)u * blockDim.x + threadIdx.x;
            d[u] = __builtin_nontemporal_load(&w4[v]);
            if (SPW == 2) x[u] = R.words[4 * v + 4];
        }
    };
    auto record = [&](uint64_t c, uint32_t mask) {
        const uint32_t slot = atomicAdd(&s_nrec, 1u);
        ScreenRec rec; rec.chunk = (uint32_t)c; rec.tid = threadIdx.x; rec.hitmask = mask; rec.pad = 0;
        my_recs[slot] = rec;
    };
    auto samples = [&](const u32x4 (&d)[U], const uint32_t (&x)[U], uint32_t (&sm)[NS]) {
#pragma unroll
        for (int u = 0; u < U; u++) {
            const uint32_t wv[5] = {d[u].x, d[u].y, d[u].z, d[u].w, SPW == 2 ? x[u] : 0u};
#pragma unroll
            for (int q = 0; q < 4; q++)
#pragma unroll
                for (int j = 0; j < SPW; j++) {
                    static_assert(CANON != 1 || SPW == 1, "sixteen-base samples come with stride 16");
                    const uint32_t raw = (SPW == 1 || j == 0) ? wv[q] : alignbit(wv[q + 1], wv[q], 16u);
                    sm[(u * 4 + q) * SPW + j] = canon_key<CANON>(raw, S.smask, 32u - 2u * (uint32_t)S.s);
                }
        }
    };

    uint32_t p_n = 0, p_sm = 0, p_id = 0, p_off = 0; uint4 p_blk = make_uint4(0, 0, 0, 0);
    uint64_t prev_c = 0;
    const char *__restrict__ f2_bytes = reinterpret_cast<const char *>(S.front2);
    auto issue_prev = [&] {
        p_blk = *reinterpret_cast<const uint4 *>(f2_bytes + p_off);
    };
    auto settle_prev = [&] {
        const uint32_t pt = block_test(p_sm, bloom_hash(p_sm), p_blk);
        if (lane < p_n && (int32_t)pt < 0) lds_or(&s_ver[p_id & 63u], 1u << (p_id >> 8));
        MF_COMPILER_FENCE();
        const uint32_t v = lds_xchg(&s_ver[lane], 0u);
        if (v) record(prev_c, v);
    };

    auto process = [&](uint64_t c, const u32x4 (&d)[U], const uint32_t (&x)[U]) {
        uint32_t sm[NS];
        samples(d, x, sm);
        if (LDSF) {
            uint32_t base = 0;
            uint32_t hms[NS / 8];
#pragma unroll
            for (int g0 = 0; g0 < NS; g0 += 8) {
                uint32_t hm = 0;
#pragma unroll
                for (int i = 0; i < 8; i++) {
                    const uint32_t h = bloom_hash(sm[g0 + i]);
                    const uint4 blk = s_tab4[__builtin_amdgcn_ubfe(h, idx_lo, idx_bits)];
                    hm = alignbit(hm, block_test(sm[g0 + i], h, blk), 31);
                }
                hms[g0 / 8] = hm;
            }
            settle_prev();
            constexpr int GL = 8;
#pragma unroll
            for (int g0 = 0; g0 < NS; g0 += GL) {
                const uint32_t hm = hms[g0 / GL];
#pragma unroll
                for (int i = 0; i < GL; i++) {
                    const bool hit = (hm >> (GL - 1 - i)) & 1u;
                    const uint64_t bm = __builtin_amdgcn_ballot_w64(hit);
                    if (bm) {
                        const uint32_t off = base + __builtin_amdgcn_mbcnt_hi((uint32_t)(bm >> 32), __builtin_amdgcn_mbcnt_lo((uint32_t)bm, 0u));
                        const uint32_t bit = (uint32_t)(NS - 1 - (g0 + i));
                        if (hit) {
                            if (off < (uint32_t)S2_QCAP) { lds_st(&s_qsm[off], sm[g0 + i]); lds_st(&s_qid[off], lane | (bit << 8)); }
                            else lds_or(&s_ver[lane], 1u << bit);
                        }
                        base += (uint32_t)__popcll(bm);
                    }
                }
            }
            MF_COMPILER_FENCE();
            p_n = base < (uint32_t)S2_QCAP ? base : (uint32_t)S2_QCAP;
            prev_c = c;
            p_sm = lds_ld(&s_qsm[lane]); p_id = lds_ld(&s_qid[lane]);
            p_off = lane < p_n ? __builtin_amdgcn_ubfe(bloom_hash(p_sm), lo2, b2) << 4 : 0u;
        } else {
            uint32_t mask = 0;
#pragma unroll
            for (int g0 = 0; g0 < NS; g0 += G) {
                uint4 blk[G];
                uint32_t pre = (1u << G) - 1u;
                if (PRE) {
                    pre = 0;
#pragma unroll
                    for (int i = 0; i < G; i++) {
                        const uint32_t bi = __builtin_amdgcn_ubfe(bloom_hash(sm[g0 + i]), pre_lo, pre_bits);
                        const uint32_t w = lds_ld(&s_pre[bi >> 5]);
                        pre = alignbit(pre, w << (~bi & 31u), 31);
                    }
                }
#pragma unroll
                for (int i = 0; i < G; i++) if (!PRE || ((pre >> (G - 1 - i)) & 1u)) blk[i] = f2[__builtin_amdgcn_ubfe(bloom_hash(sm[g0 + i]), lo2, b2)];
                uint32_t m = 0;
#pragma unroll
                for (int i = 0; i < G; i++) {
                    const uint32_t t = (!PRE || ((pre >> (G - 1 - i)) & 1u)) ? block_test(sm[g0 + i], bloom_hash(sm[g0 + i]), blk[i]) : 0u;
                    m = alignbit(m, t, 31);
                }
                if (b3 && __ballot(m != 0)) {
#pragma unroll
                    for (int i = 0; i < G; i++) if ((m >> (G - 1 - i)) & 1u) blk[i] = f3[__builtin_amdgcn_ubfe(bloom_hash(sm[g0 + i]), lo3, b3)];
                    uint32_t m3 = 0;
#pragma unroll
                    for (int i = 0; i < G; i++) {
                        const uint32_t t = ((m >> (G - 1 - i)) & 1u) ? block_test(sm[g0 + i], bloom_hash(sm[g0 + i]), blk[i]) : 0u;
                        m3 = alignbit(m3, t, 31);
                    }
                    m = m3;
                }
                mask = (mask << G) | m;
            }
            if (mask) record(c, mask);
        }
    };

    u32x4 a[U], b[U]; uint32_t ax[U], bx[U];
    uint64_t c = blockIdx.x;
    if (c < n_chunks) load(c, a, ax);
    {
        const uint4 z = make_uint4(0, 0, 0, 0);
        for (uint64_t i = (uint64_t)blockIdx.x * blockDim.x + threadIdx.x; i < clear_vec4; i += cstep * blockDim.x) clear[i] = z;
        if (LDSF || PRE) {
            const uint4 *__restrict__ src = reinterpret_cast<const uint4 *>(LDSF ? S.bloom : S.pre);
            for (uint32_t i = threadIdx.x; i < nb4; i += blockDim.x) s_tab4[i] = src[i];
        }
        lds_st(&s_ver[lane], 0u); lds_st(&s_qsm[lane], 0u); lds_st(&s_qid[lane], 0u);
        if (threadIdx.x == 0) s_nrec = 0;
    }
    __syncthreads();
    if (c < n_chunks) for (;;) {
        {
            const bool last = c + cstep >= n_chunks;
            const uint64_t cn = last ? c : c + cstep;
            if (LDSF) issue_prev();
            load(cn, b, bx);
            process(c, a, ax);
            if (last) break;
            c = cn;
        }
        {
            const bool last = c + cstep >= n_chunks;
            const uint64_t cn = last ? c : c + cstep;
            if (LDSF) issue_prev();
            load(cn, a, ax);
            process(c, b, bx);
            if (last) break;
            c = cn;
        }
    }
    if (LDSF) { issue_prev(); settle_prev(); }
    __syncthreads();
    if (threadIdx.x == 0) rec_counts[blockIdx.x] = s_nrec;
}

constexpr int S3_QN = 128;
constexpr size_t S3_LDS_EXTRA = 16 + (size_t)(SCREEN_BLOCK / 64) * (S3_QN * 10);

template <int U, int CANON = 0>
__global__ void __launch_bounds__(1024)
screen3_kernel(ReadsView R, KmerSetView S, ScreenRec *__restrict__ recs, uint32_t rec_cap, uint32_t *__restrict__ rec_counts,
               uint4 *__restrict__ clear, uint64_t clear_vec4)
{
    extern __shared__ uint4 s_tab4[];
    constexpr int NS = U * 4;
    static_assert(NS == 8, "the sample select below is written for eight samples a slice");
    const uint32_t nb4 = (1u << S.bloom_log2w) >> 2;
    uint32_t &s_nrec = *reinterpret_cast<uint32_t *>(s_tab4 + nb4);
    const uint32_t lane = threadIdx.x & 63, wid = threadIdx.x >> 6;
    typedef __attribute__((address_space(3))) unsigned short lds_u16;
    lds_u32 *s_qsm = (lds_u32 *)(reinterpret_cast<uint32_t *>(s_tab4 + nb4 + 1)) + wid * (S3_QN * 10 / 4);
    lds_u32 *s_qch = s_qsm + S3_QN;
    lds_u16 *s_qid = (lds_u16 *)(s_qch + S3_QN);
    const u32x4 *__restrict__ w4 = reinterpret_cast<const u32x4 *>(R.words);
    const uint4 *__restrict__ f2 = reinterpret_cast<const uint4 *>(S.front2);
    const uint64_t chunk = (uint64_t)blockDim.x * U;
    const uint64_t n_chunks = R.n_vec / chunk;
    const uint32_t idx_lo = stage1_index_lo(S.s, S.bloom_log2w), idx_bits = S.bloom_log2w - 2;
    const uint32_t lo2 = stage1_index_lo(S.s, S.f2_log2b + 2), b2 = S.f2_log2b;
    const uint64_t cstep = gridDim.x;
    ScreenRec *__restrict__ my_recs = recs + (size_t)blockIdx.x * rec_cap;
    uint32_t q_n = 0;
    uint32_t e_w = 0, t_w = 0;

    auto load = [&](uint64_t c, u32x4 (&d)[U]) {
#pragma unroll
        for (int u = 0; u < U; u++) d[u] = __builtin_nontemporal_load(&w4[c * chunk + (uint64_t)u * blockDim.x + threadIdx.x]);
    };
    auto record = [&](uint32_t c32, uint32_t tid, uint32_t mask) {
        const uint32_t slot = atomicAdd(&s_nrec, 1u);
        ScreenRec rec; rec.chunk = c32; rec.tid = tid; rec.hitmask = mask; rec.pad = 0;
        my_recs[slot] = rec;
    };
    auto drain = [&] {
        const uint32_t cnt = q_n < 64u ? q_n : 64u;
        const uint32_t esm = lds_ld(&s_qsm[lane]), ech = lds_ld(&s_qch[lane]), eid = s_qid[lane];
        const uint32_t tsm = lds_ld(&s_qsm[64 + lane]), tch = lds_ld(&s_qch[64 + lane]), tid2 = s_qid[64 + lane];
        if (lane < cnt) {
            const uint32_t hh = bloom_hash(esm);
            const uint4 blk = f2[__builtin_amdgcn_ubfe(hh, lo2, b2)];
            if ((int32_t)block_test(esm, hh, blk) < 0) record(ech, eid & 1023u, 1u << (eid >> 10));
        }
        MF_COMPILER_FENCE();
        lds_st(&s_qsm[lane], tsm); lds_st(&s_qch[lane], tch); s_qid[lane] = (unsigned short)tid2;
        q_n -= cnt;
    };
    auto stage1 = [&](uint64_t c, const u32x4 (&d)[U]) {
        uint32_t hitmask = 0;
        uint32_t sm[NS] = {d[0].x, d[0].y, d[0].z, d[0].w, d[1].x, d[1].y, d[1].z, d[1].w};
        if (CANON) {
#pragma unroll
            for (int i = 0; i < NS; i++) sm[i] = canon_key<CANON>(sm[i], S.smask, 32u - 2u * (uint32_t)S.s);
        }
#pragma unroll
        for (int i = 0; i < NS; i++) {
            const uint32_t h = bloom_hash(sm[i]);
            const uint4 blk = s_tab4[__builtin_amdgcn_ubfe(h, idx_lo, idx_bits)];
            hitmask = alignbit(hitmask, block_test(sm[i], h, blk), 31);
        }
        uint32_t todo = hitmask;
        {
            t_w++;
            const bool roomy = e_w + 256u <= 64u * t_w;
            const bool single = (hitmask & (hitmask - 1u)) == 0;
            const bool direct = hitmask != 0 && ((hitmask & (hitmask << 1)) != 0 || (!single && !roomy));
            if (direct) { record((uint32_t)c, threadIdx.x, hitmask); todo = 0; }
            e_w += (uint32_t)__popcll(__builtin_amdgcn_ballot_w64(direct));
        }
        for (;;) {
            const uint64_t bm = __builtin_amdgcn_ballot_w64(todo != 0);
            if (!bm) break;
            const uint32_t off = q_n + __builtin_amdgcn_mbcnt_hi((uint32_t)(bm >> 32), __builtin_amdgcn_mbcnt_lo((uint32_t)bm, 0u));
            if (todo) {
                const uint32_t bit = 31u - (uint32_t)__clz(todo), i = (uint32_t)(NS - 1) - bit;
                const uint32_t lo = (i & 1u) ? ((i & 2u) ? sm[3] : sm[1]) : ((i & 2u) ? sm[2] : sm[0]);
                const uint32_t hi = (i & 1u) ? ((i & 2u) ? sm[7] : sm[5]) : ((i & 2u) ? sm[6] : sm[4]);
                lds_st(&s_qsm[off], (i & 4u) ? hi : lo); lds_st(&s_qch[off], (uint32_t)c); s_qid[off] = (unsigned short)(threadIdx.x | (bit << 10));
                todo &= ~(1u << bit);
            }
            q_n += (uint32_t)__popcll(bm);
            e_w += (uint32_t)__popcll(bm);
            MF_COMPILER_FENCE();
            if (q_n >= 64u) drain();
        }
    };

    u32x4 a[U], b[U];
    uint64_t c = blockIdx.x;
    if (c < n_chunks) load(c, a);
    {
        const uint4 z = make_uint4(0, 0, 0, 0);
        for (uint64_t i = (uint64_t)blockIdx.x * blockDim.x + threadIdx.x; i < clear_vec4; i += cstep * blockDim.x) clear[i] = z;
        const uint4 *__restrict__ src = reinterpret_cast<const uint4 *>(S.bloom);
        for (uint32_t i = threadIdx.x; i < nb4; i += blockDim.x) s_tab4[i] = src[i];
        if (threadIdx.x == 0) s_nrec = 0;
    }
    __syncthreads();
    if (c < n_chunks) for (;;) {
        if (c + cstep >= n_chunks) { stage1(c, a); break; }
        load(c + cstep, b);
        stage1(c, a);
        c += cstep;
        if (c + cstep >= n_chunks) { stage1(c, b); break; }
        load(c + cstep, a);
        stage1(c, b);
        c += cstep;
    }
    while (q_n) drain();
    __syncthreads();
    if (threadIdx.x == 0) rec_counts[blockIdx.x] = s_nrec;
}

constexpr int MARK_SPLIT = 1;
constexpr int MARK_BLOCK = 1024;

template <int SPW, int U>
__global__ void __launch_bounds__(MARK_BLOCK)
mark_kernel(ReadsView R, KmerSetView S, const ScreenRec *__restrict__ recs, uint32_t rec_cap, const uint32_t *__restrict__ rec_counts,
            uint32_t screen_block, uint32_t split, uint32_t *__restrict__ cand)
{
    const uint32_t *__restrict__ s_st2 = S.bloom + ((size_t)1 << S.bloom_log2w);
    const uint32_t st2_shift = 32 - (S.stage2_log2w + 5);
    const uint32_t smask = S.smask;
    const uint64_t chunk = (uint64_t)screen_block * U;
    const bool fast = R.len_magic32 != 0;
    const uint32_t list = blockIdx.x / split, part = blockIdx.x % split;
    const uint32_t n = rec_counts[list];
    const ScreenRec *__restrict__ my = recs + (size_t)list * rec_cap;
    const uint32_t lane = threadIdx.x & 63;
    for (uint32_t base = part * blockDim.x + (threadIdx.x & ~63u); base < n; base += split * blockDim.x) {
        const uint32_t i = base + lane;
        uint32_t pend_w = EMPTY32, pend_b = 0;
        auto mark = [&](uint64_t r) {
            const uint32_t w = (uint32_t)(r >> 5), b = 1u << (r & 31);
            if (w == pend_w) { pend_b |= b; return; }
            if (pend_b) atomicOr(&cand[pend_w], pend_b);
            pend_w = w; pend_b = b;
        };
        if (i < n) {
        const ScreenRec rec = my[i];
        constexpr int NS = U * 4 * SPW;
        auto off_of = [&](int idx) -> uint32_t {
            const int j = idx % SPW, q = (idx / SPW) & 3, u = idx / (4 * SPW);
            return ((((uint32_t)u * screen_block + rec.tid) * 4 + q) << 4) + (uint32_t)j * 8;
        };
        const uint64_t cb = (uint64_t)rec.chunk * chunk * 64;
        uint64_t rq = 0; uint32_t rrem = 0;
        if (fast) { rq = __umul64hi(cb, R.len_magic); rrem = (uint32_t)(cb - rq * R.uniform_len); }
        uint32_t m = rec.hitmask;
        auto verify = [&](int idx, uint64_t r_known) {
            const uint64_t g0 = cb + off_of(idx);
            const uint64_t wi = g0 >> 4;
            uint32_t sm = R.words[wi];
            if (SPW == 2) sm = alignbit(R.words[wi + 1], sm, 16u * (idx % SPW));
            sm &= smask;
            const uint32_t rc = revcomp_s(sm, S.s);
            const uint32_t cn_ = sm < rc ? sm : rc;
            const uint32_t ha = stage2_hash_a(cn_), hb = stage2_hash_b(cn_);
            uint32_t ok = 1;
#pragma unroll
            for (int p = 0; p < STAGE2_K; p++) {
                const uint32_t pos = (ha + (uint32_t)p * hb) >> st2_shift;
                ok &= s_st2[pos >> 5] >> (pos & 31);
            }
            if (!(ok & 1u)) return;
            if (S.use_stab && !stab_contains(S, sm)) return;
            uint64_t r = r_known;
            if (r == ~0ULL) { r = read_holding(R, g0, (uint32_t)S.s); if (r == ~0ULL) return; }
            mark(r);
        };
        if (!fast) {
            uint64_t cur_r = ~0ULL, cur_lo = 0, cur_hi = 0; int cur_idx = 0; uint32_t cur_n = 0;
            auto flush = [&] {
                if (cur_n >= 2) mark(cur_r);
                else if (cur_n == 1) verify(cur_idx, cur_r);
            };
            while (m) {
                const int bit = 31 - __clz(m);
                m &= ~(1u << bit);
                const int idx = NS - 1 - bit;
                const uint64_t g0 = cb + off_of(idx);
                if (cur_r != ~0ULL && g0 >= cur_lo && g0 + (uint64_t)S.s <= cur_hi) { cur_n++; continue; }
                flush();
                cur_n = 0; cur_r = ~0ULL;
                if (g0 < cur_hi && cur_hi != 0 && g0 >= cur_lo) continue;
                uint64_t lo_, hi_;
                const uint64_t r = read_holding(R, g0, (uint32_t)S.s, &lo_, &hi_);
                if (r == ~0ULL) continue;
                cur_r = r; cur_lo = lo_; cur_hi = hi_; cur_idx = idx; cur_n = 1;
            }
            flush();
        } else {
        uint64_t cur_r = ~0ULL; int cur_idx = 0; uint32_t cur_n = 0;
        auto flush = [&] {
            if (cur_n >= 2) mark(cur_r);
            else if (cur_n == 1) verify(cur_idx, cur_r);
        };
        while (m) {
            const int bit = 31 - __clz(m);
            m &= ~(1u << bit);
            const int idx = NS - 1 - bit;
            const uint32_t off = off_of(idx);
            const uint32_t t = rrem + off;
            const uint32_t dq = __umulhi(t, R.len_magic32);
            const uint32_t offr = t - dq * R.uniform_len;
            if (offr + (uint32_t)S.s > R.uniform_len || cb + off + S.s > R.total_bases) continue;
            const uint64_t r = rq + dq;
            if (r == cur_r) { cur_n++; continue; }
            flush();
            cur_r = r; cur_idx = idx; cur_n = 1;
        }
        flush();
        }
        }
#pragma unroll
        for (int d = 1; d < 64; d <<= 1) {
            const uint32_t ow = __shfl_up(pend_w, d), ob = __shfl_up(pend_b, d);
            if (lane >= (uint32_t)d && ow == pend_w) pend_b |= ob;
        }
        const uint32_t next_w = __shfl_down(pend_w, 1);
        if (pend_b && (lane == 63 || next_w != pend_w)) atomicOr(&cand[pend_w], pend_b);
    }
}

constexpr int ITEM_POS = 16;
constexpr int EXACT_BLOCK = 1024;
constexpr int EXACT_BLOCK_CO = 512;

__device__ __forceinline__ uint64_t funnel64(uint64_t lo, uint64_t hi, int sh)
{
    return sh ? (lo >> sh) | (hi << (64 - sh)) : lo;
}

typedef uint32_t u32x4_a4 __attribute__((ext_vector_type(4), aligned(4)));
typedef uint32_t u32x2_a4 __attribute__((ext_vector_type(2), aligned(4)));

template <int KW>
__device__ __forceinline__ bool table_has(const KmerSetView &S, uint64_t klo, uint64_t khi, uint32_t h)
{
    uint64_t slot = h & S.slot_mask;
    if (KW == 1) {
        uint64_t e = S.keys[slot];
        while (e < klo) { slot = (slot + 1) & S.slot_mask; e = S.keys[slot]; }
        return e == klo;
    } else {
        const ulonglong2 *__restrict__ kt = reinterpret_cast<const ulonglong2 *>(S.keys);
        ulonglong2 e = kt[slot];
        while ((e.y < khi) || (e.y == khi && e.x < klo)) { slot = (slot + 1) & S.slot_mask; e = kt[slot]; }
        return e.x == klo && e.y == khi;
    }
}

template <int KW>
__device__ __forceinline__ void item_hits(const ReadsView &R, const KmerSetView &S, const uint2 *__restrict__ s_kb2,
                                          uint32_t kb_shift, uint64_t b0, uint64_t n_pos, uint64_t p0, bool hasn,
                                          uint32_t thr, lds_u32 *cnt, const bool COUNT_ALL)
{
    const int k = S.k;
    const uint64_t mask_lo = (KW == 1 && k < 32) ? (1ULL << (2 * k)) - 1 : ~0ULL;
    const uint64_t mask_hi = KW == 2 ? (1ULL << (2 * k - 64)) - 1 : 0;
    const uint64_t bit = 2 * (b0 + p0);
    const uint32_t *__restrict__ w = R.words + (bit >> 5);
    const uint32_t sh = (uint32_t)bit & 31;
    constexpr int NW = KW == 1 ? 4 : 6;
    uint32_t raw[NW + 1];
    {
        const u32x4_a4 v = *reinterpret_cast<const u32x4_a4 *>(w);
        raw[0] = v.x; raw[1] = v.y; raw[2] = v.z; raw[3] = v.w;
        if (KW == 1) raw[4] = w[4];
        else { const u32x2_a4 v2 = *reinterpret_cast<const u32x2_a4 *>(w + 4); raw[4] = v2.x; raw[5] = v2.y; raw[NW] = w[6]; }
    }
    uint32_t a[NW];
#pragma unroll
    for (int i = 0; i < NW; i++) a[i] = alignbit(raw[i + 1], raw[i], sh);
    const uint64_t x0 = (uint64_t)a[0] | ((uint64_t)a[1] << 32), x1 = (uint64_t)a[2] | ((uint64_t)a[3] << 32);
    uint64_t x2 = 0;
    if (KW == 2) x2 = (uint64_t)a[NW - 2] | ((uint64_t)a[NW - 1] << 32);

    uint64_t r0 = 0, r1 = 0;
    if (KW == 1) {
        const uint64_t y0 = ~swap_pairs_rev64(x1), y1 = ~swap_pairs_rev64(x0);
        const int drop = 2 * (64 - k - (ITEM_POS - 1));
        if (drop >= 64) { r0 = y1 >> (drop - 64); r1 = 0; }
        else { r0 = (y0 >> drop) | (y1 << (64 - drop)); r1 = y1 >> drop; }
    }
    auto key_at = [&](int i, uint64_t &klo, uint64_t &khi) {
        if (KW == 1) {
            const uint64_t fwd = funnel64(x0, x1, 2 * i) & mask_lo;
            const uint64_t rc = funnel64(r0, r1, 2 * (ITEM_POS - 1 - i)) & mask_lo;
            klo = fwd < rc ? fwd : rc; khi = 0;
        } else {
            const uint64_t lo = funnel64(x0, x1, 2 * i), hi = funnel64(x1, x2, 2 * i) & mask_hi;
            uint64_t rlo, rhi; revcomp2(lo, hi, k, rlo, rhi);
            const bool f = (hi < rhi) || (hi == rhi && lo < rlo);
            klo = f ? lo : rlo; khi = f ? hi : rhi;
        }
    };

    uint32_t pos_mask = 0;
#pragma unroll
    for (int i = 0; i < ITEM_POS; i++) {
        uint64_t klo, khi;
        key_at(i, klo, khi);
        const uint32_t hb = KW == 1 ? kbit_hash1(klo) : kbit_hash2(klo, khi);
        const uint2 blk = s_kb2[hb >> kb_shift];
        const uint32_t g = kbit_pos(hb);
        const uint32_t t = (blk.x >> (g & 31)) & (blk.y >> ((g >> 5) & 31));
        pos_mask |= (t & 1u) << i;
    }
    const uint64_t left = n_pos - p0;
    if (left < ITEM_POS) pos_mask &= (1u << left) - 1;
    if (hasn && pos_mask) {
        const uint64_t len = n_pos + k - 1;
        const uint64_t n_lo = npos_lower_bound(R, b0), n_hi = npos_lower_bound(R, b0 + len);
        for (uint64_t n = n_lo; n < n_hi; n++) {
            const int64_t d = (int64_t)(R.npos[n] - (b0 + p0));
#pragma unroll
            for (int i = 0; i < ITEM_POS; i++) if (d >= i && d < i + k) pos_mask &= ~(1u << i);
        }
    }
    while (pos_mask) {
        if (!COUNT_ALL && lds_ld(cnt) >= thr) break;
        const int i = __ffs(pos_mask) - 1;
        pos_mask &= pos_mask - 1;
        uint64_t klo, khi;
        key_at(i, klo, khi);
        const uint32_t h = (uint32_t)(KW == 1 ? hash_key1(klo) : hash_key2(klo, khi));
        if (table_has<KW>(S, klo, khi, h)) lds_add(cnt, 1u);
    }
}

__device__ __forceinline__ uint32_t nth_set_bit(uint32_t w, uint32_t n)
{
    uint32_t pos = 0;
#pragma unroll
    for (int s = 16; s >= 1; s >>= 1) {
        const uint32_t c = __popc((w >> pos) & ((1u << s) - 1));
        if (n >= c) { n -= c; pos += s; }
    }
    return pos;
}

__device__ __forceinline__ uint32_t nth_set_lane(uint64_t ballot, uint32_t m)
{
    uint32_t posn = 0;
#pragma unroll
    for (int sft = 32; sft >= 1; sft >>= 1) {
        const uint32_t cnt_lo = (uint32_t)__popcll(ballot & ((1ull << sft) - 1));
        if (m >= cnt_lo) { m -= cnt_lo; ballot >>= sft; posn += sft; } else ballot &= (1ull << sft) - 1;
    }
    return posn;
}

template <int KW>
__device__ __forceinline__ void run_candidates(const ReadsView &R, const KmerSetView &S, const uint2 *__restrict__ s_kb2, uint32_t kb_shift,
                                               uint32_t thr, bool two_phase, int lane, bool owner, uint64_t b0, uint32_t np,
                                               uint32_t hasn, lds_u32 *my_cnt, const bool COUNT_ALL)
{
    my_cnt[lane] = 0;
    const uint32_t b0_lo = (uint32_t)b0, b0_hi = (uint32_t)(b0 >> 32);
    auto wave_max = [&](uint32_t v) -> uint32_t {
#pragma unroll
        for (int o = 32; o > 0; o >>= 1) { const uint32_t t = __shfl_xor(v, o); v = t > v ? t : v; }
        return v;
    };
    constexpr uint32_t EARLY_ITEMS = 2;
    const uint32_t items_all = (wave_max(owner ? np : 0) + ITEM_POS - 1) / ITEM_POS;
    uint32_t it_lo = 0, it_hi = (COUNT_ALL || !two_phase || items_all <= EARLY_ITEMS) ? items_all : EARLY_ITEMS;
    uint64_t who = __ballot(owner);
    for (int phase = 0; phase < 2; phase++) {
        if (phase == 1) {
            if (it_hi >= items_all) break;
            const bool need = owner && my_cnt[lane] < thr && np > EARLY_ITEMS * ITEM_POS;
            who = __ballot(need);
            it_lo = EARLY_ITEMS;
            it_hi = (wave_max(need ? np : 0) + ITEM_POS - 1) / ITEM_POS;
        }
        const uint32_t nc = (uint32_t)__popcll(who);
        if (!nc) break;
        const uint32_t map = phase == 0 ? (uint32_t)lane : nth_set_lane(who, (uint32_t)lane);
        for (uint32_t ib = it_lo; ib < it_hi; ib += 32) {
            const uint32_t nit = it_hi - ib < 32 ? it_hi - ib : 32;
            int lg = 0; while (lg < 5 && (1u << lg) < nit) lg++;
            const uint32_t n_items = nc << lg;
            for (uint32_t t0 = 0; t0 < n_items; t0 += 64) {
                const uint32_t t = t0 + lane;
                const int ci = (int)__shfl(map, (int)((t >> lg) & 63)) & 63;
                const uint32_t it = ib + (t & ((1u << lg) - 1));
                const uint64_t cb0 = ((uint64_t)__shfl(b0_hi, ci) << 32) | __shfl(b0_lo, ci);
                const uint32_t cnp = __shfl(np, ci), chn = __shfl(hasn, ci);
                const uint32_t p0 = it * ITEM_POS;
                if (t < n_items && it < it_hi && p0 < cnp)
                    item_hits<KW>(R, S, s_kb2, kb_shift, cb0, cnp, p0, chn != 0, thr, &my_cnt[ci], COUNT_ALL);
            }
        }
    }
}

constexpr int WC_PER_LANE = 4;
constexpr int WC_WORDS = 64 * WC_PER_LANE;

template <int KW, bool COUNT_ALL, int BLOCK>
__global__ void __launch_bounds__(BLOCK)
exact_kernel(ReadsView R, KmerSetView S, uint32_t *__restrict__ cand, uint32_t thr,
             uint32_t *__restrict__ out_bits, uint32_t *__restrict__ hits_out, unsigned long long *__restrict__ partials, uint32_t merge)
{
    extern __shared__ uint4 s_mem4[];
    constexpr int WAVES = BLOCK / 64;
    uint32_t *s_res = reinterpret_cast<uint32_t *>(s_mem4);
    uint32_t *s_cnt = s_res + WAVES * WC_WORDS;
    constexpr int HEAD4 = (WAVES * WC_WORDS + WAVES * 64) / 4;
    const uint2 *s_kb2 = reinterpret_cast<const uint2 *>(s_mem4 + HEAD4);
    {
        const uint32_t nb4 = (1u << S.kb_log2w) >> 2;
        const uint4 *__restrict__ src = reinterpret_cast<const uint4 *>(S.kbloom);
        uint4 *dst = s_mem4 + HEAD4;
        for (uint32_t i = threadIdx.x; i < nb4; i += blockDim.x) dst[i] = src[i];
    }
    __syncthreads();
    const uint32_t kb_shift = 32 - (S.kb_log2w - 1);
    const int lane = threadIdx.x & 63, wid = threadIdx.x >> 6;
    uint32_t *my_res = s_res + wid * WC_WORDS; lds_u32 *my_cnt = (lds_u32 *)(s_cnt + wid * 64);
    const uint64_t n_bw = (R.n_reads + 31) >> 5;
    const uint64_t n_wc = (n_bw + WC_WORDS - 1) / WC_WORDS;
    const int k = S.k;
    uint32_t tot_pass = 0, tot_cand = 0;

    const uint64_t wc_step = (uint64_t)gridDim.x * WAVES;
    static_assert(WC_PER_LANE == 4, "a lane's words are a uint4");
    auto load_cw = [&](uint64_t wc) -> uint4 {
        const uint64_t wi = wc * WC_WORDS + (uint64_t)lane * WC_PER_LANE;
        uint32_t w[WC_PER_LANE];
#pragma unroll
        for (int j = 0; j < WC_PER_LANE; j++) {
            const bool in = wc < n_wc && wi + j < n_bw;
            w[j] = in ? (cand ? cand[wi + j] : 0xFFFFFFFFu) : 0u;
            if (in && cand && w[j]) cand[wi + j] = 0;
        }
        return make_uint4(w[0], w[1], w[2], w[3]);
    };
    uint4 cw_next = load_cw((uint64_t)blockIdx.x * WAVES + wid);
    for (uint64_t wc = (uint64_t)blockIdx.x * WAVES + wid; wc < n_wc; wc += wc_step) {
        const uint64_t wbase = wc * WC_WORDS;
        uint32_t cw[WC_PER_LANE] = {cw_next.x, cw_next.y, cw_next.z, cw_next.w}, pre[WC_PER_LANE + 1];
        pre[0] = 0;
#pragma unroll
        for (int j = 0; j < WC_PER_LANE; j++) {
            const uint64_t wi = wbase + (uint64_t)lane * WC_PER_LANE + j;
            if (wi < n_bw) { const uint64_t rem = R.n_reads - wi * 32; if (rem < 32) cw[j] &= (1u << rem) - 1; }
            pre[j + 1] = pre[j] + __popc(cw[j]);
            my_res[lane * WC_PER_LANE + j] = 0;
        }
        cw_next = load_cw(wc + wc_step);
        tot_cand += pre[WC_PER_LANE];
        uint32_t incl = pre[WC_PER_LANE];
#pragma unroll
        for (int o = 1; o < 64; o <<= 1) { const uint32_t t = __shfl_up(incl, o); if (lane >= o) incl += t; }
        const uint32_t total = __shfl(incl, 63);
        const uint32_t pre_packed = pre[1] | (pre[2] << 8) | (pre[3] << 16);
        for (uint32_t cbase = 0; cbase < total; cbase += 64) {
            const uint32_t ncand = total - cbase < 64 ? total - cbase : 64;
            const bool active = (uint32_t)lane < ncand;
            const uint32_t c = active ? cbase + lane : total - 1;
            int lo = 0, hi = 63;
#pragma unroll
            for (int it = 0; it < 6; it++) { const int mid = (lo + hi) >> 1; if (__shfl(incl, mid) > c) hi = mid; else lo = mid + 1; }
            const int src = lo;
            const uint32_t sp = __shfl(pre_packed, src);
            const uint32_t w0 = __shfl(cw[0], src), w1 = __shfl(cw[1], src), w2 = __shfl(cw[2], src), w3 = __shfl(cw[3], src);
            const uint32_t tot_src = (sp >> 16 & 255u) + __popc(w3);
            uint32_t n = c - (__shfl(incl, src) - tot_src);
            const uint32_t p1 = sp & 255u, p2 = (sp >> 8) & 255u, p3 = (sp >> 16) & 255u;
            const int j = n >= p3 ? 3 : n >= p2 ? 2 : n >= p1 ? 1 : 0;
            const uint32_t w = j == 3 ? w3 : j == 2 ? w2 : j == 1 ? w1 : w0;
            n -= j == 3 ? p3 : j == 2 ? p2 : j == 1 ? p1 : 0u;
            const uint32_t b = nth_set_bit(w, n);
            const uint32_t wslot = (uint32_t)src * WC_PER_LANE + j;
            const uint64_t r = (wbase + wslot) * 32 + b;
            uint64_t b0 = 0; uint32_t np = 0, hasn = 0;
            if (active) {
                uint64_t len;
                if (R.uniform_len) { b0 = r * R.uniform_len; len = R.uniform_len; }
                else { b0 = R.offsets[r]; len = R.offsets[r + 1] - b0; }
                const uint64_t n_pos = len >= (uint64_t)k ? len - k + 1 : 0;
                np = n_pos > 0xFFFFFFFFull ? 0xFFFFFFFFu : (uint32_t)n_pos;
                hasn = (R.has_n[r >> 5] >> (r & 31)) & 1u;
            }
            run_candidates<KW>(R, S, s_kb2, kb_shift, thr, cand != nullptr, lane, active, b0, np, hasn, my_cnt, COUNT_ALL);
            if (active) {
                const uint32_t h = my_cnt[lane];
                if (COUNT_ALL) hits_out[r] = h;
                if (h >= thr) atomicOr(&my_res[wslot], 1u << b);
            }
        }
#pragma unroll
        for (int j = 0; j < WC_PER_LANE; j++) {
            const uint64_t wi = wbase + (uint64_t)lane * WC_PER_LANE + j;
            const uint32_t res = my_res[lane * WC_PER_LANE + j];
            if (wi < n_bw) { if (!merge) out_bits[wi] = res; else if (res) atomicOr(&out_bits[wi], res); }
            tot_pass += __popc(res);
        }
    }
#pragma unroll
    for (int o = 32; o > 0; o >>= 1) { tot_pass += __shfl_down(tot_pass, o); tot_cand += __shfl_down(tot_cand, o); }
    __syncthreads();
    if (lane == 0) { s_cnt[wid * 2] = tot_pass; s_cnt[wid * 2 + 1] = tot_cand; }
    __syncthreads();
    if (threadIdx.x == 0) {
        unsigned long long p = 0, c = 0;
        for (int w = 0; w < WAVES; w++) { p += s_cnt[w * 2]; c += s_cnt[w * 2 + 1]; }
        partials[2 * blockIdx.x] = p; partials[2 * blockIdx.x + 1] = c;
    }
    if (blockIdx.x == 0)
        for (uint32_t i = 2 * gridDim.x + threadIdx.x; i < 2 * EXACT_MAX_GRID; i += blockDim.x) partials[i] = 0;
}

template <int KW>
__device__ __forceinline__ bool sample_item(const ReadsView &R, const KmerSetView &S, const uint2 *__restrict__ s_kb2, uint32_t kb_shift,
                                            bool active, uint64_t r, uint64_t b0, uint64_t n_pos, uint64_t p0)
{
    const int k = S.k;
    const uint64_t mask_lo = (KW == 1 && k < 32) ? (1ULL << (2 * k)) - 1 : ~0ULL;
    const uint64_t mask_hi = KW == 2 ? (1ULL << (2 * k - 64)) - 1 : 0;
    constexpr int NW = KW == 1 ? 4 : 6;
    uint64_t x0 = 0, x1 = 0, x2 = 0, r0 = 0, r1 = 0;
    uint32_t hasn = 0, pm = 0;
    auto key_at = [&](int i, uint64_t &klo, uint64_t &khi) {
        if (KW == 1) {
            const uint64_t fwd = funnel64(x0, x1, 2 * i) & mask_lo;
            const uint64_t rc = funnel64(r0, r1, 2 * (ITEM_POS - 1 - i)) & mask_lo;
            klo = fwd < rc ? fwd : rc; khi = 0;
        } else {
            const uint64_t lo = funnel64(x0, x1, 2 * i), hi = funnel64(x1, x2, 2 * i) & mask_hi;
            uint64_t rlo, rhi; revcomp2(lo, hi, k, rlo, rhi);
            const bool fl = (hi < rhi) || (hi == rhi && lo < rlo);
            klo = fl ? lo : rlo; khi = fl ? hi : rhi;
        }
    };
    if (active) {
        const uint64_t bit = 2 * (b0 + p0);
        const uint32_t *__restrict__ w = R.words + (bit >> 5);
        const uint32_t sh = (uint32_t)bit & 31;
        uint32_t raw[NW + 1];
        {
            const u32x4_a4 v = *reinterpret_cast<const u32x4_a4 *>(w);
            raw[0] = v.x; raw[1] = v.y; raw[2] = v.z; raw[3] = v.w;
            if (KW == 1) raw[4] = w[4];
            else { const u32x2_a4 v2 = *reinterpret_cast<const u32x2_a4 *>(w + 4); raw[4] = v2.x; raw[5] = v2.y; raw[NW] = w[6]; }
        }
        hasn = (R.has_n[r >> 5] >> (r & 31)) & 1u;
        uint32_t a[NW];
#pragma unroll
        for (int i = 0; i < NW; i++) a[i] = alignbit(raw[i + 1], raw[i], sh);
        x0 = (uint64_t)a[0] | ((uint64_t)a[1] << 32); x1 = (uint64_t)a[2] | ((uint64_t)a[3] << 32);
        if (KW == 2) x2 = (uint64_t)a[NW - 2] | ((uint64_t)a[NW - 1] << 32);
        if (KW == 1) {
            const uint64_t y0 = ~swap_pairs_rev64(x1), y1 = ~swap_pairs_rev64(x0);
            const int drop = 2 * (64 - k - (ITEM_POS - 1));
            if (drop >= 64) { r0 = y1 >> (drop - 64); r1 = 0; }
            else { r0 = (y0 >> drop) | (y1 << (64 - drop)); r1 = y1 >> drop; }
        }
#pragma unroll
        for (int i = 0; i < ITEM_POS; i++) {
            uint64_t klo, khi;
            key_at(i, klo, khi);
            const uint32_t hb = KW == 1 ? kbit_hash1(klo) : kbit_hash2(klo, khi);
            const uint2 blk = s_kb2[hb >> kb_shift];
            const uint32_t g = kbit_pos(hb);
            const uint32_t t = (blk.x >> (g & 31)) & (blk.y >> ((g >> 5) & 31));
            pm |= (t & 1u) << i;
        }
        const uint64_t left = n_pos - p0;
        if (left < (uint64_t)ITEM_POS) pm &= (1u << left) - 1;
        if (hasn && pm) {
            const uint64_t len = n_pos + k - 1;
            const uint64_t n_lo = npos_lower_bound(R, b0), n_hi = npos_lower_bound(R, b0 + len);
            for (uint64_t n = n_lo; n < n_hi; n++) {
                const int64_t d = (int64_t)(R.npos[n] - (b0 + p0));
#pragma unroll
                for (int i = 0; i < ITEM_POS; i++) if (d >= i && d < i + k) pm &= ~(1u << i);
            }
        }
    }
    bool hit = false;
    while (__ballot(pm != 0)) {
        uint64_t klo[4], khi[4], slot[4]; bool v[4];
#pragma unroll
        for (int j = 0; j < 4; j++) {
            v[j] = pm != 0;
            const int i = v[j] ? __ffs(pm) - 1 : 0;
            pm &= pm - 1;
            key_at(i, klo[j], khi[j]);
            slot[j] = (KW == 1 ? hash_key1(klo[j]) : hash_key2(klo[j], khi[j])) & S.slot_mask;
        }
        if (KW == 1) {
            uint64_t e[4];
#pragma unroll
            for (int j = 0; j < 4; j++) e[j] = v[j] ? S.keys[slot[j]] : EMPTY64;
#pragma unroll
            for (int j = 0; j < 4; j++) {
                while (e[j] < klo[j]) { slot[j] = (slot[j] + 1) & S.slot_mask; e[j] = S.keys[slot[j]]; }
                hit |= v[j] && e[j] == klo[j];
            }
        } else {
            const ulonglong2 *__restrict__ kt = reinterpret_cast<const ulonglong2 *>(S.keys);
            ulonglong2 e[4];
#pragma unroll
            for (int j = 0; j < 4; j++) e[j] = v[j] ? kt[slot[j]] : make_ulonglong2(EMPTY64, EMPTY64);
#pragma unroll
            for (int j = 0; j < 4; j++) {
                while ((e[j].y < khi[j]) || (e[j].y == khi[j] && e[j].x < klo[j])) { slot[j] = (slot[j] + 1) & S.slot_mask; e[j] = kt[slot[j]]; }
                hit |= v[j] && e[j].x == klo[j] && e[j].y == khi[j];
            }
        }
        if (hit) pm = 0;
    }
    return hit;
}

constexpr int FINISH_BLOCK = 256;
constexpr int FINISH_GRID = 1024;
static_assert(FINISH_GRID <= EXACT_MAX_GRID, "tally buffer");

template <int SPW, int U, int KW, int PHASE>
__global__ void __launch_bounds__(FINISH_BLOCK)
finish_kernel(ReadsView R, KmerSetView S, const ScreenRec *__restrict__ recs, uint32_t rec_cap, const uint32_t *__restrict__ rec_counts,
              uint32_t n_lists, uint32_t screen_block, uint32_t *__restrict__ bits, unsigned long long *__restrict__ partials, uint32_t *__restrict__ cand)
{
    __shared__ uint32_t s_pre[EXACT_MAX_GRID + 1];
    __shared__ uint32_t s_tot[2];
    {
        uint32_t c[4], sum = 0;
#pragma unroll
        for (int j = 0; j < 4; j++) { const uint32_t i = threadIdx.x * 4 + j; c[j] = i < n_lists ? rec_counts[i] : 0u; sum += c[j]; }
        uint32_t incl = sum;
#pragma unroll
        for (int o = 1; o < 64; o <<= 1) { const uint32_t t = __shfl_up(incl, o); if ((threadIdx.x & 63) >= (uint32_t)o) incl += t; }
        __shared__ uint32_t s_wave[FINISH_BLOCK / 64];
        if ((threadIdx.x & 63) == 63) s_wave[threadIdx.x >> 6] = incl;
        if (threadIdx.x < 2) s_tot[threadIdx.x] = 0;
        __syncthreads();
        uint32_t base = incl - sum;
        for (uint32_t w = 0; w < (threadIdx.x >> 6); w++) base += s_wave[w];
#pragma unroll
        for (int j = 0; j < 4; j++) { const uint32_t i = threadIdx.x * 4 + j; if (i <= n_lists) s_pre[i] = base; base += c[j]; }
        __syncthreads();
    }
    const uint32_t total = s_pre[n_lists];
    constexpr int NSAMP = U * 4 * SPW, SPP = 4 * SPW;
    const int k = S.k;
    const uint32_t smask = S.smask;
    const bool fast = R.len_magic32 != 0;
    const uint64_t chunk_bases = (uint64_t)screen_block * U * 64;
    const uint64_t mask_lo = (KW == 1 && k < 32) ? (1ULL << (2 * k)) - 1 : ~0ULL;
    const uint64_t mask_hi = KW == 2 ? (1ULL << (2 * k - 64)) - 1 : 0;
    const uint32_t n_adj = (uint32_t)((S.k - S.s + S.stride - 1) / S.stride) + 1;
    const uint32_t run_span = (uint32_t)S.s + (n_adj - 1) * (uint32_t)S.stride;
    uint32_t run_ok = 0;
    for (int i = 0; i < NSAMP; i++) if ((uint32_t)(i % SPP) + n_adj <= (uint32_t)SPP) run_ok |= 1u << (NSAMP - 1 - i);
    uint32_t n_pass = 0, n_items = 0;
    uint32_t pend_old = 0, pend_bit = 0;
    auto load_rec = [&](uint32_t ri) -> ScreenRec {
        uint32_t lo = 0, hi = n_lists;
        while (hi - lo > 1) { const uint32_t mid = (lo + hi) >> 1; if (s_pre[mid] <= ri) lo = mid; else hi = mid; }
        return recs[(size_t)lo * rec_cap + (ri - s_pre[lo])];
    };
    const uint32_t stride_r = gridDim.x * FINISH_BLOCK;
    uint32_t ri = blockIdx.x * FINISH_BLOCK + threadIdx.x;
    const ScreenRec no_rec{0xFFFFFFFFu, 0xFFFFFFFFu, 0, 0};
    ScreenRec rec_next = no_rec;
    if (ri < total) rec_next = load_rec(ri);
    for (uint32_t base = blockIdx.x * FINISH_BLOCK; base < total; base += stride_r, ri += stride_r) {
        const ScreenRec rec = rec_next;
        rec_next = no_rec;
        if (ri + stride_r < total) rec_next = load_rec(ri + stride_r);
        const uint64_t cb = (uint64_t)rec.chunk * chunk_bases;
        uint64_t rq = 0; uint32_t rrem = 0;
        if (fast) { rq = __umul64hi(cb, R.len_magic); rrem = (uint32_t)(cb - rq * R.uniform_len); }
        uint32_t m = rec.hitmask;
        uint32_t runs = m & run_ok;
        for (uint32_t j = 1; j < n_adj; j++) runs &= m << j;
        if (PHASE == 0 && SPW == 1 && KW == 2 && fast) {
            const uint32_t nb_chunk = __shfl_down(rec.chunk, 1), nb_tid = __shfl_down(rec.tid, 1), nb_mask = __shfl_down(rec.hitmask, 1);
            const bool nb = (threadIdx.x & 63) != 63 && nb_chunk == rec.chunk && nb_tid == rec.tid + 1 && rec.hitmask != 0;
            runs = 0;
#pragma unroll
            for (int u = 0; u < U; u++) {
                const int sh = 4 * (U - 1 - u);
                const uint32_t e = (((rec.hitmask >> sh) & 15u) << 4) | (nb ? (nb_mask >> sh) & 15u : 0u);
                uint32_t re = e;
                for (uint32_t j = 1; j < n_adj; j++) re &= e << j;
                runs |= ((re >> 4) & 15u) << sh;
            }
        }
        uint32_t lf_runs = 0; bool lf = false;
        if (PHASE == 0 && SPW == 1) {
            const uint32_t lc = __shfl_up(rec.chunk, 1), lt = __shfl_up(rec.tid, 1);
            lf_runs = __shfl_up(runs, 1);
            lf = (threadIdx.x & 63) != 0 && lc == rec.chunk && lt + 1 == rec.tid;
        }
        if (PHASE == 0) m = runs; else runs = 0;
        uint64_t passed_r = ~0ULL, passed_r2 = ~0ULL;
        while (m) {
            bool is_run = false, got = false; uint64_t g0 = 0, r = 0;
            constexpr int NKW = KW == 1 ? 3 : 5;
            uint32_t raw[NKW];
            while (m) {
                is_run = PHASE == 0;
                const int bit = 31 - __clz(m);
                m &= ~(1u << bit);
                const int idx = NSAMP - 1 - bit;
                const int sj = idx % SPW, sq = (idx / SPW) & 3, su = idx / (4 * SPW);
                const uint32_t off = ((((uint32_t)su * screen_block + rec.tid) * 4 + sq) << 4) + (uint32_t)sj * 8;
                g0 = cb + off;
                const uint32_t span = is_run ? run_span : (uint32_t)S.s;
                if (fast) {
                    const uint32_t t = rrem + off;
                    const uint32_t dq = __umulhi(t, R.len_magic32);
                    const uint32_t offr = t - dq * R.uniform_len;
                    if (offr + span > R.uniform_len || g0 + span > R.total_bases) continue;
// ... 177 lines not shown
        slot = (slot + 1) & stab_mask;
    }
}

__global__ void build_screen_kernel(BaitView B, int s, uint32_t *bloom, uint32_t log2w, uint32_t log2w2, uint32_t *stab,
                                    uint32_t stab_mask, uint32_t *has_ones, uint32_t *front2, uint32_t f2_log2b, uint32_t *front3, uint32_t f3_log2b,
                                    uint32_t *pre, uint32_t pre_log2w, bool canon)
{
    const uint64_t p = (uint64_t)blockIdx.x * blockDim.x + threadIdx.x;
    if (p >= B.total || B.runlen[p] < s) return;
    const uint64_t bit = 2 * p; const uint64_t wi = bit >> 5; const uint32_t sh = (uint32_t)bit & 31;
    uint32_t fwd = alignbit(B.words[wi + 1], B.words[wi], sh);
    if (s < 16) fwd &= (1u << (2 * s)) - 1;
    const uint32_t rc = revcomp_s(fwd, s);
    const uint32_t cn = fwd < rc ? fwd : rc;
    const uint32_t k0 = canon ? cn : fwd, k1 = canon ? cn : rc;
    stage1_insert(k0, s, bloom, log2w); if (!canon) stage1_insert(k1, s, bloom, log2w);
    if (front2) { stage1_insert(k0, s, front2, f2_log2b + 2); if (!canon) stage1_insert(k1, s, front2, f2_log2b + 2); }
    if (front3) { stage1_insert(k0, s, front3, f3_log2b + 2); if (!canon) stage1_insert(k1, s, front3, f3_log2b + 2); }
    if (pre) {
        const uint32_t lo = pre_index_lo(s, pre_log2w), nb = pre_log2w + 5;
        for (uint32_t v : {k0, k1}) { const uint32_t bi = (bloom_hash(v) >> lo) & ((1u << nb) - 1u); atomicOr(&pre[bi >> 5], 1u << (bi & 31u)); }
    }
    stab_insert(fwd, stab, stab_mask, has_ones); stab_insert(rc, stab, stab_mask, has_ones);
    const uint32_t ha = stage2_hash_a(cn), hb = stage2_hash_b(cn);
    uint32_t *st2 = bloom + ((size_t)1 << log2w);
#pragma unroll
    for (int i = 0; i < STAGE2_K; i++) {
        const uint32_t pos = (ha + (uint32_t)i * hb) >> (32 - (log2w2 + 5));
        atomicOr(&st2[pos >> 5], 1u << (pos & 31));
    }
}

__global__ void build_kbloom_kernel(const uint64_t *keys, uint64_t slots, int kw, uint32_t *kbloom, uint32_t kb_log2w)
{
    const uint64_t i = (uint64_t)blockIdx.x * blockDim.x + threadIdx.x;
    if (i >= slots) return;
    const uint64_t lo = keys[i * kw], hi = kw == 2 ? keys[i * kw + 1] : 0;
    if (lo == EMPTY64 && (kw == 1 || hi == EMPTY64)) return;
    const uint32_t hb = kw == 1 ? kbit_hash1(lo) : kbit_hash2(lo, hi), g = kbit_pos(hb);
    uint32_t *blk = kbloom + 2 * (size_t)(hb >> (32 - (kb_log2w - 1)));
    atomicOr(&blk[0], 1u << (g & 31));
    atomicOr(&blk[1], 1u << ((g >> 5) & 31));
}

__global__ void count_keys_kernel(const uint64_t *keys, uint64_t slots, int kw, const uint32_t *stab, uint64_t stab_slots,
                                  unsigned long long *out)
{
    const uint64_t i = (uint64_t)blockIdx.x * blockDim.x + threadIdx.x;
    uint32_t a = 0, b = 0;
    if (i < slots) a = !(keys[i * kw] == EMPTY64 && (kw == 1 || keys[i * kw + 1] == EMPTY64));
    if (stab && i < stab_slots) b = stab[i] != EMPTY32;
    const uint32_t ca = (uint32_t)__popcll(__ballot(a)), cb = (uint32_t)__popcll(__ballot(b));
    if ((threadIdx.x & 63) == 0) {
        if (ca) atomicAdd(&out[0], (unsigned long long)ca);
        if (cb) atomicAdd(&out[1], (unsigned long long)cb);
    }
}

__global__ void build_npos_blk_kernel(const uint64_t *__restrict__ npos, uint64_t n_npos, uint64_t n_blk, uint32_t *__restrict__ blk)
{
    const uint64_t b = (uint64_t)blockIdx.x * blockDim.x + threadIdx.x;
    if (b >= n_blk) return;
    blk[b] = (uint32_t)lower_bound_u64(npos, n_npos, b << NPOS_BLK_SHIFT);
}

__global__ void build_off_blk_kernel(const uint64_t *__restrict__ offsets, uint64_t n_reads, uint64_t n_blk, uint64_t *__restrict__ blk)
{
    const uint64_t b = (uint64_t)blockIdx.x * blockDim.x + threadIdx.x;
    if (b >= n_blk) return;
    blk[b] = offblk_make(offsets, n_reads, b).pack();
}

__global__ void mark_has_n_kernel(ReadsView R, uint32_t *has_n)
{
    const uint64_t i = (uint64_t)blockIdx.x * blockDim.x + threadIdx.x;
    if (i >= R.n_npos) return;
    const uint64_t r = read_holding(R, R.npos[i], 1);
    if (r != ~0ULL) atomicOr(&has_n[r >> 5], 1u << (r & 31));
}

__device__ __forceinline__ uint32_t byte_window80(uint32_t addr, uint32_t lo, uint32_t hi)
{
    const uint32_t b0 = lo > addr ? lo - addr : 0u, b1 = hi < addr + 4 ? (hi > addr ? hi - addr : 0u) : 4u;
    if (b1 <= b0) return 0u;
    const uint32_t upto1 = b1 >= 4 ? 0xFFFFFFFFu : ((1u << (8 * b1)) - 1), upto0 = b0 >= 4 ? 0xFFFFFFFFu : ((1u << (8 * b0)) - 1);
    return upto1 & ~upto0 & 0x80808080u;
}

constexpr int QS_LANES = 8;

__device__ __forceinline__ uint32_t count_n_bytes(const uint4 v, uint32_t blk, uint32_t lo, uint32_t hi)
{
    const uint32_t w[4] = {v.x, v.y, v.z, v.w};
    uint32_t c = 0;
#pragma unroll
    for (int j = 0; j < 4; j++) {
        const uint32_t x = w[j] ^ 0x4E4E4E4Eu;
        const uint32_t z = ~(((x & 0x7F7F7F7Fu) + 0x7F7F7F7Fu) | x | 0x7F7F7F7Fu);
        c += __popc(z & byte_window80(blk * 16 + 4 * j, lo, hi));
    }
    return c;
}

__device__ __forceinline__ uint32_t count_lowq_bytes(const uint4 v, uint32_t blk, uint32_t lo, uint32_t hi, uint32_t q1)
{
    const uint32_t w[4] = {v.x, v.y, v.z, v.w};
    uint32_t c = 0;
#pragma unroll
    for (int j = 0; j < 4; j++) {
        const uint32_t d = (w[j] | 0x80808080u) - q1;
        c += __popc(~d & ~w[j] & byte_window80(blk * 16 + 4 * j, lo, hi));
    }
    return c;
}

__global__ void __launch_bounds__(256)
qualscan_kernel(const uint8_t *__restrict__ text, const QualRec *__restrict__ recs, uint32_t n, uint32_t quality,
                uint32_t *__restrict__ n_count, uint32_t *__restrict__ bad_count)
{
    const uint32_t t = blockIdx.x * blockDim.x + threadIdx.x;
    const uint32_t r = t / QS_LANES, l = t % QS_LANES;
    uint32_t nn = 0, nb = 0;
    if (r < n) {
        const QualRec rec = recs[r];
        const uint4 *__restrict__ t4 = reinterpret_cast<const uint4 *>(text);
        const uint32_t s_lo = rec.s_off, s_hi = rec.s_off + rec.s_len, q_lo = rec.q_off, q_hi = rec.q_off + rec.q_len;
        const uint32_t sb0 = s_lo >> 4, nsb = rec.s_len ? ((s_hi - 1) >> 4) - sb0 + 1 : 0;
        const uint32_t qb0 = q_lo >> 4, nqb = rec.q_len ? ((q_hi - 1) >> 4) - qb0 + 1 : 0;
        const uint32_t q1 = (quality + 1) * 0x01010101u;
        const uint32_t nmax = nsb > nqb ? nsb : nqb;
        const uint4 zero = make_uint4(0, 0, 0, 0);
        for (uint32_t i = l; i < nmax; i += 2 * QS_LANES) {
            const uint32_t i2 = i + QS_LANES;
            const uint4 s0 = i < nsb ? t4[sb0 + i] : zero, s1 = i2 < nsb ? t4[sb0 + i2] : zero;
            const uint4 q0 = i < nqb ? t4[qb0 + i] : zero, q2 = i2 < nqb ? t4[qb0 + i2] : zero;
            if (i < nsb) nn += count_n_bytes(s0, sb0 + i, s_lo, s_hi);
            if (i2 < nsb) nn += count_n_bytes(s1, sb0 + i2, s_lo, s_hi);
            if (i < nqb) nb += count_lowq_bytes(q0, qb0 + i, q_lo, q_hi, q1);
            if (i2 < nqb) nb += count_lowq_bytes(q2, qb0 + i2, q_lo, q_hi, q1);
        }
    }
#pragma unroll
    for (int o = QS_LANES / 2; o > 0; o >>= 1) { nn += __shfl_xor(nn, o, QS_LANES); nb += __shfl_xor(nb, o, QS_LANES); }
    if (r < n && l == 0) { n_count[r] = nn; bad_count[r] = nb; }
}

__device__ __forceinline__ void sip_round(uint64_t &v0, uint64_t &v1, uint64_t &v2, uint64_t &v3)
{
    auto rotl = [](uint64_t x, int b) { return (x << b) | (x >> (64 - b)); };
    v0 += v1; v1 = rotl(v1, 13); v1 ^= v0; v0 = rotl(v0, 32);
    v2 += v3; v3 = rotl(v3, 16); v3 ^= v2;
    v0 += v3; v3 = rotl(v3, 21); v3 ^= v0;
    v2 += v1; v1 = rotl(v1, 17); v1 ^= v2; v2 = rotl(v2, 32);
}

__global__ void __launch_bounds__(256)
seqhash_kernel(const uint8_t *__restrict__ text, const QualRec *__restrict__ recs, uint32_t n, uint64_t *__restrict__ hashes)
{
    const uint32_t r = blockIdx.x * blockDim.x + threadIdx.x;
    if (r >= n) return;
    const QualRec rec = recs[r];
    const uint32_t *__restrict__ w = reinterpret_cast<const uint32_t *>(text) + (rec.s_off >> 2);
    const uint32_t sh = (rec.s_off & 3) * 8;
    const uint64_t len = (uint64_t)rec.s_len + 1;
    uint64_t v0 = 0x736F6D6570736575ULL, v1 = 0x646F72616E646F6DULL, v2 = 0x6C7967656E657261ULL, v3 = 0x7465646279746573ULL;
    uint32_t d0 = w[0];
    uint64_t i = 0;
    auto block = [&](uint64_t at) -> uint64_t {
        const uint32_t *p = w + (at >> 2);
        const uint32_t d1 = p[1], d2 = p[2];
        const uint64_t m = ((uint64_t)alignbit(d2, d1, sh) << 32) | alignbit(d1, d0, sh);
        d0 = d2;
        return m;
    };
    for (; i + 8 <= (uint64_t)rec.s_len; i += 8) {
        const uint64_t m = block(i);
        v3 ^= m; sip_round(v0, v1, v2, v3); v0 ^= m;
    }
    const uint32_t t = (uint32_t)(rec.s_len - i);
    uint64_t tailv = block(i);
    tailv = t == 0 ? 0 : (tailv & (~0ULL >> (64 - 8 * t)));
    tailv |= 0xFFULL << (8 * t);
    if (t == 7) { v3 ^= tailv; sip_round(v0, v1, v2, v3); v0 ^= tailv; tailv = 0; }
    const uint64_t b = ((len & 0xFF) << 56) | tailv;
    v3 ^= b; sip_round(v0, v1, v2, v3); v0 ^= b;
    v2 ^= 0xFF;
    sip_round(v0, v1, v2, v3); sip_round(v0, v1, v2, v3); sip_round(v0, v1, v2, v3);
    hashes[r] = v0 ^ v1 ^ v2 ^ v3;
}

__device__ __forceinline__ uint64_t dedup_mix(uint64_t x) { x ^= x >> 32; x *= 0xD6E8FEB86659FD93ULL; x ^= x >> 32; return x; }

__global__ void __launch_bounds__(256)
dedup_insert_kernel(const uint64_t *__restrict__ hashes, const uint8_t *__restrict__ alive, uint32_t n, uint64_t base,
                    unsigned long long *__restrict__ keys, unsigned long long *__restrict__ first, uint64_t mask,
                    unsigned long long *__restrict__ zero_idx, unsigned long long *__restrict__ n_keys)
{
    const uint32_t i = blockIdx.x * blockDim.x + threadIdx.x;
    if (i >= n || !alive[i]) return;
    const uint64_t h = hashes[i];
    if (h == 0) { atomicMin(zero_idx, (unsigned long long)(base + i)); return; }
    uint64_t slot = dedup_mix(h) & mask;
    for (;;) {
        unsigned long long k = keys[slot];
        if (k == 0) { k = atomicCAS(&keys[slot], 0ull, (unsigned long long)h); if (k == 0) { atomicAdd(n_keys, 1ull); k = h; } }
        if (k == h) { atomicMin(&first[slot], (unsigned long long)(base + i)); return; }
        slot = (slot + 1) & mask;
    }
}

__global__ void __launch_bounds__(256)
dedup_check_kernel(const uint64_t *__restrict__ hashes, const uint8_t *__restrict__ alive, uint32_t n, uint64_t base,
                   const unsigned long long *__restrict__ keys, const unsigned long long *__restrict__ first, uint64_t mask,
                   const unsigned long long *__restrict__ zero_idx, uint8_t *__restrict__ dup)
{
    const uint32_t i = blockIdx.x * blockDim.x + threadIdx.x;
    if (i >= n) return;
    uint8_t d = 0;
    if (alive[i]) {
        const uint64_t h = hashes[i];
        if (h == 0) d = *zero_idx != base + i;
        else {
            uint64_t slot = dedup_mix(h) & mask;
            while (keys[slot] != h) slot = (slot + 1) & mask;
            d = first[slot] != base + i;
        }
    }
    dup[i] = d;
}

__global__ void __launch_bounds__(256)
dedup_rehash_kernel(const unsigned long long *__restrict__ old_keys, const unsigned long long *__restrict__ old_first, uint64_t old_slots,
                    unsigned long long *__restrict__ keys, unsigned long long *__restrict__ first, uint64_t mask)
{
    const uint64_t i = (uint64_t)blockIdx.x * blockDim.x + threadIdx.x;
    if (i >= old_slots) return;
    const unsigned long long h = old_keys[i];
    if (h == 0) return;
    uint64_t slot = dedup_mix(h) & mask;
    while (atomicCAS(&keys[slot], 0ull, h) != 0) slot = (slot + 1) & mask;
    first[slot] = old_first[i];
}

hipError_t launch_dedup(const uint64_t *hashes, const uint8_t *alive, uint32_t n, uint64_t base, unsigned long long *keys,
                        unsigned long long *first, uint64_t slots, unsigned long long *zero_idx, unsigned long long *n_keys, uint8_t *dup,
                        hipStream_t st)
{
    if (n == 0) return hipSuccess;
    hipLaunchKernelGGL(dedup_insert_kernel, dim3((n + 255) / 256), dim3(256), 0, st, hashes, alive, n, base, keys, first, slots - 1, zero_idx, n_keys);
    hipLaunchKernelGGL(dedup_check_kernel, dim3((n + 255) / 256), dim3(256), 0, st, hashes, alive, n, base, keys, first, slots - 1, zero_idx, dup);
    return hipGetLastError();
}

hipError_t launch_dedup_rehash(const unsigned long long *old_keys, const unsigned long long *old_first, uint64_t old_slots,
                               unsigned long long *keys, unsigned long long *first, uint64_t slots, hipStream_t st)
{
    hipLaunchKernelGGL(dedup_rehash_kernel, dim3((unsigned)((old_slots + 255) / 256)), dim3(256), 0, st, old_keys, old_first, old_slots, keys, first, slots - 1);
    return hipGetLastError();
}

hipError_t launch_qualscan(const uint8_t *text, const QualRec *recs, uint32_t n, uint32_t quality, uint32_t *n_count, uint32_t *bad_count,
                           uint64_t *hashes, hipStream_t st)
{
    if (n == 0) return hipSuccess;
    hipLaunchKernelGGL(qualscan_kernel, dim3((unsigned)(((uint64_t)n * QS_LANES + 255) / 256)), dim3(256), 0, st, text, recs, n, quality, n_count, bad_count);
    if (hashes) hipLaunchKernelGGL(seqhash_kernel, dim3((n + 255) / 256), dim3(256), 0, st, text, recs, n, hashes);
    return hipGetLastError();
}

static inline unsigned grid_for(uint64_t n, unsigned block) { return (unsigned)((n + block - 1) / block); }

uint64_t screen_grid_for(const ReadsView &R, int n_cu, int stride)
{
    const uint64_t n_chunks = R.n_vec / ((uint64_t)SCREEN_BLOCK * SCREEN_U);
    uint64_t wg = (uint64_t)n_cu;
    if (stride == 16 && n_cu >= 16) wg = (uint64_t)n_cu * SCREEN_CU_NUM / SCREEN_CU_DEN;
    if (stride == 4) wg = (uint64_t)n_cu * 2;
    return n_chunks < wg ? n_chunks : wg;
}
uint64_t screen_rec_cap_for(const ReadsView &R, int n_cu, int stride)
{
    const uint64_t n_chunks = R.n_vec / ((uint64_t)SCREEN_BLOCK * SCREEN_U);
    const uint64_t grid = screen_grid_for(R, n_cu, stride);
    return grid ? (n_chunks + grid - 1) / grid * SCREEN_BLOCK : 0;
}

#define MF_LAUNCH(kernel, grid, block, lds, st, tm, ...)                                                             \
    do {                                                                                                             \
        if (tm) hipExtLaunchKernelGGL(kernel, grid, block, (uint32_t)(lds), st, (tm)->start, (tm)->stop, 0, __VA_ARGS__); \
        else hipLaunchKernelGGL(kernel, grid, block, lds, st, __VA_ARGS__);                                           \
    } while (0)

template <auto Kernel> static void raise_lds_limit_once(size_t max_bytes)
{
    static std::atomic<uint64_t> done{0};
    int dev = 0; (void)hipGetDevice(&dev);
    const uint64_t bit = 1ull << (dev & 63);
    if (done.load(std::memory_order_acquire) & bit) return;
    (void)hipFuncSetAttribute(reinterpret_cast<const void *>(Kernel), hipFuncAttributeMaxDynamicSharedMemorySize, (int)max_bytes);
    done.fetch_or(bit, std::memory_order_release);
}

template <int SPW, int CANON>
static void launch_screen_spw(const ReadsView &R, const KmerSetView &S, void *recs, uint32_t *rec_counts, int n_cu, hipStream_t st,
                              const KernelTiming *tm, uint32_t *clear, uint64_t clear_vec4)
{
    const int key = screen_grid_key(S.stride, S.front_mode, S.canon);
    const uint64_t grid = screen_grid_for(R, n_cu, key);
    if (grid == 0) return;
    const uint32_t cap = (uint32_t)screen_rec_cap_for(R, n_cu, key);
    if constexpr (SPW == 1) if (S.front_mode == 3) {
        const size_t lds = (sizeof(uint32_t) << S.bloom_log2w) + S3_LDS_EXTRA;
        raise_lds_limit_once<&screen3_kernel<SCREEN_U, CANON>>(128 * 1024 + S3_LDS_EXTRA);
        MF_LAUNCH((screen3_kernel<SCREEN_U, CANON>), dim3((unsigned)grid), dim3(SCREEN_BLOCK), lds, st, tm, R, S,
                  static_cast<ScreenRec *>(recs), cap, rec_counts, reinterpret_cast<uint4 *>(clear), clear ? clear_vec4 : (uint64_t)0);
        return;
    }
    if (S.front_mode == 1 || S.front_mode == 3) {
        const size_t lds = (sizeof(uint32_t) << S.bloom_log2w) + S2_LDS_EXTRA;
        raise_lds_limit_once<&screen2_kernel<SPW, SCREEN_U, true, 8, false, CANON>>(128 * 1024 + S2_LDS_EXTRA);
        MF_LAUNCH((screen2_kernel<SPW, SCREEN_U, true, 8, false, CANON>), dim3((unsigned)grid), dim3(SCREEN_BLOCK), lds, st, tm, R, S,
                  static_cast<ScreenRec *>(recs), cap, rec_counts, reinterpret_cast<uint4 *>(clear), clear ? clear_vec4 : (uint64_t)0);
        return;
    }
    if (S.front_mode == 4) {
        const size_t lds = (sizeof(uint32_t) << S.pre_log2w) + S2_LDS_EXTRA;
        raise_lds_limit_once<&screen2_kernel<SPW, SCREEN_U, false, 8, true, CANON>>(128 * 1024 + S2_LDS_EXTRA);
        MF_LAUNCH((screen2_kernel<SPW, SCREEN_U, false, 8, true, CANON>), dim3((unsigned)grid), dim3(SCREEN_BLOCK), lds, st, tm, R, S,
                  static_cast<ScreenRec *>(recs), cap, rec_counts, reinterpret_cast<uint4 *>(clear), clear ? clear_vec4 : (uint64_t)0);
        return;
    }
    if (S.front_mode == 2) {
        MF_LAUNCH((screen2_kernel<SPW, SCREEN_U, false, 4, false, CANON>), dim3((unsigned)grid), dim3(SCREEN_BLOCK), S2_LDS_EXTRA, st, tm, R, S,
                  static_cast<ScreenRec *>(recs), cap, rec_counts, reinterpret_cast<uint4 *>(clear), clear ? clear_vec4 : (uint64_t)0);
        return;
    }
    const size_t lds1 = (sizeof(uint32_t) << S.bloom_log2w) + 16;
    raise_lds_limit_once<&screen_kernel<SPW, SCREEN_U, CANON>>(128 * 1024 + 16);
    MF_LAUNCH((screen_kernel<SPW, SCREEN_U, CANON>), dim3((unsigned)grid), dim3(SCREEN_BLOCK), lds1, st, tm, R, S,
              static_cast<ScreenRec *>(recs), cap, rec_counts, reinterpret_cast<uint4 *>(clear), clear ? clear_vec4 : (uint64_t)0);
}

template <int SPW>
static void launch_mark_spw(const ReadsView &R, const KmerSetView &S, const void *recs, const uint32_t *rec_counts, uint32_t *cand, int n_cu,
                            hipStream_t st, const KernelTiming *tm)
{
    const int key = screen_grid_key(S.stride, S.front_mode, S.canon);
    const uint64_t grid = screen_grid_for(R, n_cu, key);
    if (grid == 0) return;
    const uint32_t cap = (uint32_t)screen_rec_cap_for(R, n_cu, key);
    static const uint32_t split = getenv("MF_MARK_SPLIT") ? (uint32_t)atoi(getenv("MF_MARK_SPLIT")) : (uint32_t)MARK_SPLIT;
    static const uint32_t mblock = getenv("MF_MARK_BLOCK") ? (uint32_t)atoi(getenv("MF_MARK_BLOCK")) : (uint32_t)MARK_BLOCK;
    MF_LAUNCH((mark_kernel<SPW, SCREEN_U>), dim3((unsigned)grid * split), dim3(mblock), 0, st, tm, R, S,
              static_cast<const ScreenRec *>(recs), cap, rec_counts, (uint32_t)SCREEN_BLOCK, split, cand);
}

hipError_t launch_screen(const ReadsView &R, const KmerSetView &S, void *recs, uint32_t *rec_counts, int n_cu, hipStream_t st,
                         const KernelTiming *tm, uint32_t *clear, uint64_t clear_vec4)
{
    if (S.stride == 16 && S.canon == 1) launch_screen_spw<1, 1>(R, S, recs, rec_counts, n_cu, st, tm, clear, clear_vec4);
    else if (S.stride == 16 && S.canon) launch_screen_spw<1, 2>(R, S, recs, rec_counts, n_cu, st, tm, clear, clear_vec4);
    else if (S.stride == 16) launch_screen_spw<1, 0>(R, S, recs, rec_counts, n_cu, st, tm, clear, clear_vec4);
    else if (S.canon) launch_screen_spw<2, 2>(R, S, recs, rec_counts, n_cu, st, tm, clear, clear_vec4);
    else launch_screen_spw<2, 0>(R, S, recs, rec_counts, n_cu, st, tm, clear, clear_vec4);
    return hipGetLastError();
}

hipError_t launch_finish(const ReadsView &R, const KmerSetView &S, const void *recs, const uint32_t *rec_counts, uint32_t *bits,
                         unsigned long long *partials, int n_cu, hipStream_t st, const KernelTiming *tm, hipEvent_t done, uint32_t *cand)
{
    const int key = screen_grid_key(S.stride, S.front_mode, S.canon);
    const uint64_t lists = screen_grid_for(R, n_cu, key);
    if (lists == 0) {
        (void)hipMemsetAsync(partials, 0, TallyLayout::bytes(), st);
        if (done) (void)hipEventRecord(done, st);
        return hipGetLastError();
    }
    const uint32_t cap = (uint32_t)screen_rec_cap_for(R, n_cu, key);
    const ScreenRec *rc = static_cast<const ScreenRec *>(recs);
    static const bool time_phase1 = getenv("MF_TIME_PHASE1") != nullptr;
    const KernelTiming *none = nullptr, *tm0 = time_phase1 ? none : tm, *tm1 = time_phase1 ? tm : none;
    KernelTiming last{nullptr, done};
    bool done_attached = false;
    if (done && !tm1) { tm1 = &last; done_attached = true; }
    static const unsigned fgrid = std::min<unsigned>(EXACT_MAX_GRID, std::max<unsigned>(64, getenv("MF_FINISH_GRID") ? (unsigned)atoi(getenv("MF_FINISH_GRID")) : FINISH_GRID));
#define MF_LAUNCH_FINISH(SPW, KW) do { \
        MF_LAUNCH((finish_kernel<SPW, SCREEN_U, KW, 0>), dim3(fgrid), dim3(FINISH_BLOCK), 0, st, tm0, R, S, rc, cap, rec_counts, \
                  (uint32_t)lists, (uint32_t)SCREEN_BLOCK, bits, partials, cand); \
        MF_LAUNCH((finish_kernel<SPW, SCREEN_U, KW, 1>), dim3(fgrid), dim3(FINISH_BLOCK), 0, st, tm1, R, S, rc, cap, rec_counts, \
                  (uint32_t)lists, (uint32_t)SCREEN_BLOCK, bits, partials, cand); } while (0)
    if (S.stride == 16) { if (S.kw == 1) MF_LAUNCH_FINISH(1, 1); else MF_LAUNCH_FINISH(1, 2); }
    else                { if (S.kw == 1) MF_LAUNCH_FINISH(2, 1); else MF_LAUNCH_FINISH(2, 2); }
#undef MF_LAUNCH_FINISH
    if (done && !done_attached) (void)hipEventRecord(done, st);
    return hipGetLastError();
}

hipError_t launch_mark(const ReadsView &R, const KmerSetView &S, const void *recs, const uint32_t *rec_counts, uint32_t *cand, int n_cu,
                       hipStream_t st, const KernelTiming *tm)
{
    if (S.stride == 16) launch_mark_spw<1>(R, S, recs, rec_counts, cand, n_cu, st, tm);
    else launch_mark_spw<2>(R, S, recs, rec_counts, cand, n_cu, st, tm);
    return hipGetLastError();
}

hipError_t launch_exact(const ReadsView &R, const KmerSetView &S_, uint32_t *cand, uint32_t thr, bool count_all,
                        uint32_t *out_bits, uint32_t *hits_out, unsigned long long *partials, int n_cu, hipStream_t st,
                        const KernelTiming *tm, bool coresident, hipEvent_t done, bool merge)
{
    const uint64_t n_bw = (R.n_reads + 31) >> 5;
    const uint64_t n_wc = (n_bw + WC_WORDS - 1) / WC_WORDS;
    if (n_wc == 0) { if (done) (void)hipEventRecord(done, st); return hipGetLastError(); }
    KmerSetView S = S_;
    if (coresident && !count_all) { S.kbloom = S_.kbloom_co; S.kb_log2w = S_.kb_co_log2w; } else coresident = false;
    const int waves = (coresident ? EXACT_BLOCK_CO : EXACT_BLOCK) / 64;
    const size_t lds = (sizeof(uint32_t) << S.kb_log2w) + (size_t)(waves * WC_WORDS + waves * 64) * sizeof(uint32_t);
    const int per_cu = coresident ? 1 : 2 * lds <= 160 * 1024 ? 2 : 1;
    uint64_t grid = (n_wc + waves - 1) / waves;
    if (grid > (uint64_t)n_cu * per_cu) grid = (uint64_t)n_cu * per_cu;
    if (grid > EXACT_MAX_GRID) grid = EXACT_MAX_GRID;
    KernelTiming with_done{nullptr, done};
    const KernelTiming *tmx = tm ? tm : (done ? &with_done : nullptr);
#define MF_LAUNCH_EXACT(KW, CA, BLK) do { \
        raise_lds_limit_once<&exact_kernel<KW, CA, BLK>>(160 * 1024); \
        MF_LAUNCH((exact_kernel<KW, CA, BLK>), dim3((unsigned)grid), dim3(BLK), lds, st, tmx, R, S, cand, thr, out_bits, hits_out, partials, merge ? 1u : 0u); } while (0)
    if (coresident) { if (S.kw == 1) MF_LAUNCH_EXACT(1, false, EXACT_BLOCK_CO); else MF_LAUNCH_EXACT(2, false, EXACT_BLOCK_CO); }
    else if (S.kw == 1) { if (count_all) MF_LAUNCH_EXACT(1, true, EXACT_BLOCK); else MF_LAUNCH_EXACT(1, false, EXACT_BLOCK); }
    else                { if (count_all) MF_LAUNCH_EXACT(2, true, EXACT_BLOCK); else MF_LAUNCH_EXACT(2, false, EXACT_BLOCK); }
#undef MF_LAUNCH_EXACT
    if (done && tm) (void)hipEventRecord(done, st);
    return hipGetLastError();
}

hipError_t launch_build_kbloom(const uint64_t *keys, uint64_t slots, int kw, uint32_t *kbloom, uint32_t kb_log2w, hipStream_t st)
{
    hipLaunchKernelGGL(build_kbloom_kernel, dim3(grid_for(slots, 256)), dim3(256), 0, st, keys, slots, kw, kbloom, kb_log2w);
    return hipGetLastError();
}

hipError_t launch_build_table(const BaitView &B, int k, int kw, uint64_t *keys, uint64_t slots, uint32_t *postab_scratch, hipStream_t st)
{
    if (B.total == 0) return hipSuccess;
    const unsigned grid = grid_for(B.total, 256);
    if (kw == 1) {
        hipLaunchKernelGGL(build_keys1_kernel, dim3(grid), dim3(256), 0, st, B, k, keys, slots - 1);
    } else {
        hipLaunchKernelGGL(build_pos2_kernel, dim3(grid), dim3(256), 0, st, B, k, postab_scratch, slots - 1);
        hipLaunchKernelGGL(materialize2_kernel, dim3(grid_for(slots, 256)), dim3(256), 0, st, B, k, postab_scratch, slots, keys);
    }
    return hipGetLastError();
}

hipError_t launch_build_screen(const BaitView &B, int s, uint32_t *bloom, uint32_t log2w, uint32_t log2w2, uint32_t *stab,
                               uint32_t stab_slots, uint32_t *has_ones, uint32_t *front2, uint32_t f2_log2b, uint32_t *front3, uint32_t f3_log2b,
                               uint32_t *pre, uint32_t pre_log2w, bool canon, hipStream_t st)
{
    if (B.total == 0) return hipSuccess;
    hipLaunchKernelGGL(build_screen_kernel, dim3(grid_for(B.total, 256)), dim3(256), 0, st, B, s, bloom, log2w, log2w2, stab, stab_slots - 1, has_ones,
                       front2, f2_log2b, front3, f3_log2b, pre, pre_log2w, canon);
    return hipGetLastError();
}

hipError_t launch_count_keys(const uint64_t *keys, uint64_t slots, int kw, const uint32_t *stab, uint64_t stab_slots,
                             unsigned long long *out2, hipStream_t st)
{
    const uint64_t n = slots > stab_slots ? slots : stab_slots;
    hipLaunchKernelGGL(count_keys_kernel, dim3(grid_for(n, 256)), dim3(256), 0, st, keys, slots, kw, stab, stab_slots, out2);
    return hipGetLastError();
}

hipError_t launch_build_npos_blk(const uint64_t *npos, uint64_t n_npos, uint64_t n_blk, uint32_t *blk, hipStream_t st)
{
    hipLaunchKernelGGL(build_npos_blk_kernel, dim3(grid_for(n_blk, 256)), dim3(256), 0, st, npos, n_npos, n_blk, blk);
    return hipGetLastError();
}

hipError_t launch_build_off_blk(const uint64_t *offsets, uint64_t n_reads, uint64_t n_blk, uint64_t *blk, hipStream_t st)
{
    hipLaunchKernelGGL(build_off_blk_kernel, dim3(grid_for(n_blk, 256)), dim3(256), 0, st, offsets, n_reads, n_blk, blk);
    return hipGetLastError();
}

hipError_t launch_mark_has_n(const ReadsView &R, uint32_t *has_n, hipStream_t st)
{
    if (R.n_npos == 0) return hipSuccess;
    hipLaunchKernelGGL(mark_has_n_kernel, dim3(grid_for(R.n_npos, 256)), dim3(256), 0, st, R, has_n);
    return hipGetLastError();
}

}
```

### mitoflex_amd/csrc/mf_passplan.h

```cpp
#pragma once
#include "../../include/mitofilter.h"
#include "mf_kernels_cfg.h"
namespace mf {
struct TallyLayout {
    static constexpr int REGIONS = 3;
    static constexpr size_t region(int i) { return (size_t)i * EXACT_MAX_GRID * 2; }
    static constexpr size_t words() { return region(REGIONS); }
    static constexpr size_t bytes() { return words() * sizeof(unsigned long long); }
    struct Totals { unsigned long long pass = 0, cand = 0; };
    static Totals sum(const unsigned long long *block, int regions) { Totals t; for (size_t i = 0; i < region(regions); i += 2) { t.pass += block[i]; t.cand += block[i + 1]; } return t; }
};
struct PassKnobs { int pass, finish_streams, screen_streams, split_pipe, exact_co, s8_finish; };
struct PassFeedback { bool prefer_split = false, finish_two = false, split_serial = false; };
struct PassInputs {
    int prot, s, stride, kw, k, s8_finish;
    unsigned thr; int mode; bool count_all, overlap, more;
    PassFeedback fb; int flip, cur, nsets;
};
enum class PassKind { PROTEIN, FINISH, SPLIT_PIPELINED, ONE_STREAM };
enum class PassStream { MAIN, FINISH_A, SCREEN_ALT, FINISH_B };
struct PassPlan {
    PassKind kind = PassKind::ONE_STREAM; int q = 0, q_out = 0;
    PassStream screen_on = PassStream::MAIN, later_on = PassStream::MAIN;
    bool two_streams = false, wait_prev_finish = false, screen = false, screen_clears_bits = false, needs_cand = false, exact_behind_finish = false, exact_coresident = false;
    int flip = 0, cur = 0; bool sample_pass = false;
};
inline PassPlan plan_pass(const PassKnobs &kn, const PassInputs &in)
{
    PassPlan p; p.flip = in.flip; p.cur = p.q_out = in.cur;
    if (in.prot) { p.kind = PassKind::PROTEIN; return p; }
    const bool screened = in.mode == MF_MODE_SCREENED && in.s > 0;
    const bool s8 = kn.s8_finish < 0 ? in.s8_finish != 0 : kn.s8_finish == 1;
    const bool finish = screened && kn.pass != 1 && !in.fb.prefer_split && in.thr == 1 && !in.count_all && (in.stride == 16 || kn.pass == 2 || s8);
    const bool split = !finish && screened && !in.count_all && in.overlap && kn.split_pipe && kn.pass != 2 && !in.fb.split_serial;
    if (!finish && !split) { p.screen = p.needs_cand = screened; return p; }
    const bool two = split || (in.overlap && kn.pass == 0);
    const int odd = (p.flip ^= 1);
    p.kind = finish ? PassKind::FINISH : PassKind::SPLIT_PIPELINED;
    p.screen = true; p.two_streams = p.wait_prev_finish = two;
    p.q = p.q_out = p.cur = (in.cur + 1) % (two && in.kw == 2 ? in.nsets : 2);
    p.screen_on = two && kn.screen_streams == 2 && odd ? PassStream::SCREEN_ALT : PassStream::MAIN;
    const bool fin2 = finish && (kn.finish_streams == 2 || (kn.finish_streams == 0 && (in.fb.finish_two || in.kw == 2)));
    p.later_on = !two ? PassStream::MAIN : fin2 && odd ? PassStream::FINISH_B : PassStream::FINISH_A;
    p.screen_clears_bits = p.sample_pass = finish;
#ifndef MF_FINISH_EXACT
#define MF_FINISH_EXACT (in.k >= 48)
#endif
    p.exact_behind_finish = finish && MF_FINISH_EXACT;
    p.needs_cand = split || p.exact_behind_finish;
    p.exact_coresident = finish ? p.exact_behind_finish && in.more : in.more || kn.exact_co;
    return p;
}
inline PassFeedback adapt_after_call(PassFeedback f, bool sample_pass, unsigned long long cand, unsigned long long n_reads)
{
    if (n_reads < 100000) return f;
    if (sample_pass) { if (cand > n_reads) f.prefer_split = true; f.finish_two = cand > n_reads / 20; return f; }
    if (f.prefer_split && cand < n_reads / 8) f.prefer_split = false;
    if (cand > n_reads / 20) f.split_serial = true; else if (cand < n_reads / 40) f.split_serial = false;
    return f;
}
}
```

Measured before the change: 163.3 billion.

## Alternate screen sweep direction and keep the tail in cache across passes

The screen kernels now walk the read chunks forward on one pass and backward on the next. The final chunks of each sweep, about 128 MB, are loaded with normal cached loads instead of nontemporal ones, so the next reversed pass can find them still in the last-level cache and read less from HBM. Bloom-table staging into LDS is also batched into a 4-deep unrolled load-then-store loop. The cost is extra sweep state kept across calls, and the cached tail may evict other data.

```diff
diff --git a/mitoflex_amd/csrc/mf_api.cpp b/mitoflex_amd/csrc/mf_api.cpp
--- a/mitoflex_amd/csrc/mf_api.cpp
+++ b/mitoflex_amd/csrc/mf_api.cpp
@@ -128,6 +128,7 @@
     std::atomic<int> screen_streams{2};
     std::atomic<int> split_pipe{1};
     std::atomic<int> exact_co{0};
+    std::atomic<int> sweep{1};
     std::atomic<int> front{-1};
     std::atomic<int> front2_log2b{0};
     std::atomic<int> s8_finish{-1};
@@ -140,6 +141,7 @@
 {
     const std::string n = name ? name : "", v = value ? value : "";
     if (n == "pass") { if (v == "" || v == "default") g_opt.pass = 0; else if (v == "split") g_opt.pass = 1; else if (v == "serial") g_opt.pass = 2; else return -1; return 0; }
+    if (n == "sweep") { if (v == "alternate") g_opt.sweep = 1; else if (v == "forward") g_opt.sweep = 0; else return -1; return 0; }
     char *end = nullptr; const long x = strtol(v.c_str(), &end, 10);
     if (v.empty() || *end) return -1;
     if (n == "expect_files") g_expect_files = x != 0;
@@ -164,7 +166,7 @@
         const char *k = getenv("MF_ENV_KNOBS");
         if (k && k[0] == '1') {
             static const char *const pairs[][2] = {{"pass", "MF_PASS"}, {"adapt", "MF_ADAPT"}, {"finish_streams", "MF_FINISH_STREAMS"}, {"screen_streams", "MF_SCREEN_STREAMS"},
-                                                   {"split_pipe", "MF_SPLIT_PIPE"}, {"exact_co", "MF_EXACT_CO"},
+                                                   {"split_pipe", "MF_SPLIT_PIPE"}, {"exact_co", "MF_EXACT_CO"}, {"sweep", "MF_SWEEP"},
                                                    {"front", "MF_FRONT"}, {"front2_log2b", "MF_FRONT2_LOG2B"}, {"front3_log2b", "MF_FRONT3_LOG2B"}, {"canon", "MF_CANON"}, {"s8_finish", "MF_S8_FINISH"},
                                                    {"depth_index", "MF_DEPTH_INDEX"}};
             for (auto &p : pairs) { const char *v = getenv(p[1]); if (v && *v && set_option(p[0], v) != 0) fprintf(stderr, "libmitofilter_hip: %s=%s is not a value of option '%s' (ignored)\n", p[1], v, p[0]); }
@@ -701,7 +703,7 @@
 {
     options_from_env_once();
     const PassKnobs knobs{g_opt.pass, g_opt.finish_streams, g_opt.screen_streams, g_opt.split_pipe, g_opt.exact_co, g_opt.s8_finish};
-    const PassInputs in{(int)S.prot, (int)S.s, (int)S.stride, (int)S.kw, (int)S.k, (int)S.s8_finish, thr, mode, count_all, overlap, more, r->fb, r->flip, r->cur, NSETS};
+    const PassInputs in{(int)S.prot, (int)S.s, (int)S.stride, (int)S.kw, (int)S.k, (int)S.s8_finish, thr, mode, count_all, overlap, more, r->fb, r->flip, r->cur, NSETS, r->sweep, g_opt.sweep != 0};
     const PassPlan P = plan_pass(knobs, in);
     const int n_cu = ctx->n_cu, q = P.q; const bool finish = P.kind == PassKind::FINISH;
     hipStream_t const streams[] = {ctx->stream, ctx->stream2, ctx->stream3, ctx->stream4}, ss = streams[(int)P.screen_on], sf = streams[(int)P.later_on];
@@ -715,7 +717,7 @@
         if (P.needs_cand && !finish) { const int rc = clean_cand(r, q, ss); if (rc) return rc; }
         KernelTiming scr_done{nullptr, r->ev_screen[q]};
         HIPCHK(launch_screen(r->v, S, r->d_recs[q], r->d_rec_counts[q], n_cu, ss, t0 ? t0 : (P.two_streams ? &scr_done : nullptr),
-                             P.screen_clears_bits ? r->d_bits[q] : nullptr, P.screen_clears_bits ? ((r->v.n_reads + 31) / 32 + 3) / 4 : 0));
+                             P.screen_clears_bits ? r->d_bits[q] : nullptr, P.screen_clears_bits ? ((r->v.n_reads + 31) / 32 + 3) / 4 : 0, P.rev, P.keep_tail));
         if (P.two_streams) { if (t0) HIPCHK(hipEventRecord(r->ev_screen[q], ss)); HIPCHK(hipStreamWaitEvent(sf, r->ev_screen[q], 0)); }
     }
 #ifdef MF_DEBUG_KNOBS
@@ -733,7 +735,7 @@
         if (P.screen) HIPCHK(launch_mark(r->v, S, r->d_recs[q], r->d_rec_counts[q], cand, n_cu, sf, t1));
         HIPCHK(launch_exact(r->v, S, cand, thr, count_all, r->d_bits[P.q_out], P.kind == PassKind::ONE_STREAM ? r->d_hits : nullptr, tally_of(r, P.q_out), n_cu, sf, t2, P.exact_coresident, done));
     }
-    r->flip = P.flip; r->cur = P.cur; r->sample_pass = P.sample_pass;
+    r->flip = P.flip; r->cur = P.cur; r->sample_pass = P.sample_pass; r->sweep = P.sweep;
     return MF_OK;
 }
 
diff --git a/mitoflex_amd/csrc/mf_api_internal.h b/mitoflex_amd/csrc/mf_api_internal.h
--- a/mitoflex_amd/csrc/mf_api_internal.h
+++ b/mitoflex_amd/csrc/mf_api_internal.h
@@ -121,6 +121,7 @@
     bool cand_clean[NSETS] = {}, sample_pass = false;
     mf::PassFeedback fb;
     int cur = 0, flip = 0;
+    int sweep = 0;
     unsigned long long *tally_override = nullptr;
     size_t bitmap_bytes = 0;
     uint32_t *d_alist = nullptr, *d_assign = nullptr; uint64_t *d_apairs = nullptr; unsigned long long *d_acnt = nullptr;
diff --git a/mitoflex_amd/csrc/mf_kernels.h b/mitoflex_amd/csrc/mf_kernels.h
--- a/mitoflex_amd/csrc/mf_kernels.h
+++ b/mitoflex_amd/csrc/mf_kernels.h
@@ -17,7 +17,7 @@
 uint64_t screen_grid_for(const ReadsView &R, int n_cu, int stride);
 uint64_t screen_rec_cap_for(const ReadsView &R, int n_cu, int stride);
 hipError_t launch_screen(const ReadsView &R, const KmerSetView &S, void *recs, uint32_t *rec_counts, int n_cu, hipStream_t st,
-                         const KernelTiming *tm = nullptr, uint32_t *clear = nullptr, uint64_t clear_vec4 = 0);
+                         const KernelTiming *tm = nullptr, uint32_t *clear = nullptr, uint64_t clear_vec4 = 0, bool rev = false, bool keep_tail = false);
 hipError_t launch_finish(const ReadsView &R, const KmerSetView &S, const void *recs, const uint32_t *rec_counts, uint32_t *bits,
                          unsigned long long *partials, int n_cu, hipStream_t st, const KernelTiming *tm = nullptr, hipEvent_t done = nullptr, uint32_t *cand = nullptr);
 hipError_t launch_mark(const ReadsView &R, const KmerSetView &S, const void *recs, const uint32_t *rec_counts, uint32_t *cand, int n_cu,
diff --git a/mitoflex_amd/csrc/mf_kernels.hip b/mitoflex_amd/csrc/mf_kernels.hip
--- a/mitoflex_amd/csrc/mf_kernels.hip
+++ b/mitoflex_amd/csrc/mf_kernels.hip
@@ -4,6 +4,7 @@
 #include <hip/hip_ext.h>
 #include <stdlib.h>
 #include <algorithm>
+#include <type_traits>
 #include <atomic>
 
 namespace mf {
@@ -76,28 +77,81 @@
     return xm < rc ? xm : rc;
 }
 
+template <int BLOCK>
+__device__ __forceinline__ void stage_lds_table(uint4 *dst, const uint4 *__restrict__ src, uint32_t nb4)
+{
+    constexpr int B = 4;
+    for (uint32_t base = 0; base < nb4; base += (uint32_t)(B * BLOCK)) {
+        uint4 t[B]; uint32_t off[B];
+#pragma unroll
+        for (int j = 0; j < B; j++) {
+            const uint32_t i = base + (uint32_t)(j * BLOCK) + threadIdx.x;
+            off[j] = (i < nb4 ? i : nb4 - 1u) << 4;
+            t[j] = *reinterpret_cast<const uint4 *>(reinterpret_cast<const char *>(src) + off[j]);
+        }
+#pragma unroll
+        for (int j = 0; j < B; j++) *reinterpret_cast<uint4 *>(reinterpret_cast<char *>(dst) + off[j]) = t[j];
+    }
+}
+template <int U> struct ScreenChunk {
+    static constexpr uint32_t VECS = (uint32_t)SCREEN_BLOCK * U;
+    static_assert((VECS & (VECS - 1)) == 0, "a chunk is a power of two of vectors");
+    static constexpr uint32_t LOG2 = 31 - __builtin_clz(VECS);
+};
+constexpr uint64_t SWEEP_KEEP_BYTES = 128ull << 20;
+constexpr std::true_type NT{}; constexpr std::false_type KEEP{};
+template <class LA, class LB, class SA, class SB>
+__device__ __forceinline__ void sweep_turns(uint64_t c, uint64_t cstep, uint64_t n_chunks, uint64_t nt_turns, LA loadA, LB loadB, SA stageA, SB stageB)
+{
+    if (c < nt_turns) {
+        for (;;) {
+            loadB(NT, c + cstep);
+            stageA(c);
+            c += cstep;
+            if (c + cstep >= nt_turns) break;
+            loadA(NT, c + cstep);
+            stageB(c);
+            c += cstep;
+        }
+        loadA(KEEP, c + cstep < n_chunks ? c + cstep : c);
+        stageB(c);
+        c += cstep;
+    }
+    if (c < n_chunks) for (;;) {
+        if (c + cstep >= n_chunks) { stageA(c); break; }
+        loadB(KEEP, c + cstep);
+        stageA(c);
+        c += cstep;
+        if (c + cstep >= n_chunks) { stageB(c); break; }
+        loadA(KEEP, c + cstep);
+        stageB(c);
+        c += cstep;
+    }
+}
+
 struct __attribute__((aligned(16))) ScreenRec { uint32_t chunk, tid, hitmask, pad; };
 
 template <int SPW, int U, int CANON = 0>
 __global__ void __launch_bounds__(1024)
 screen_kernel(ReadsView R, KmerSetView S, ScreenRec *__restrict__ recs, uint32_t rec_cap, uint32_t *__restrict__ rec_counts,
-              uint4 *__restrict__ clear, uint64_t clear_vec4)
+              uint4 *__restrict__ clear, uint64_t clear_vec4, uint32_t rev, uint64_t nt_turns)
 {
     extern __shared__ uint4 s_tab4[];
     const uint32_t nb4 = (1u << S.bloom_log2w) >> 2;
     uint32_t &s_nrec = *reinterpret_cast<uint32_t *>(s_tab4 + nb4);
     const u32x4 *__restrict__ w4 = reinterpret_cast<const u32x4 *>(R.words);
-    const uint64_t chunk = (uint64_t)blockDim.x * U;
-    const uint64_t n_chunks = R.n_vec / chunk;
+    const uint64_t chunk = ScreenChunk<U>::VECS;
+    const uint64_t n_chunks = R.n_vec >> ScreenChunk<U>::LOG2;
+    auto chunk_of = [&](uint64_t c) { return rev ? n_chunks - 1 - c : c; };
     const uint32_t idx_lo = stage1_index_lo(S.s, S.bloom_log2w), idx_bits = S.bloom_log2w - 2;
     const uint64_t cstep = gridDim.x;
     ScreenRec *__restrict__ my_recs = recs + (size_t)blockIdx.x * rec_cap;
 
-    auto load = [&](uint64_t c, u32x4 (&d)[U], uint32_t (&x)[U]) {
+    auto load = [&](auto nt, uint64_t c, u32x4 (&d)[U], uint32_t (&x)[U]) {
 #pragma unroll
         for (int u = 0; u < U; u++) {
-            const uint64_t v = c * chunk + (uint64_t)u * blockDim.x + threadIdx.x;
-            d[u] = __builtin_nontemporal_load(&w4[v]);
+            const uint64_t v = chunk_of(c) * chunk + (uint64_t)u * blockDim.x + threadIdx.x;
+            d[u] = decltype(nt)::value ? __builtin_nontemporal_load(&w4[v]) : w4[v];
             if (SPW == 2) x[u] = R.words[4 * v + 4];
         }
     };
@@ -122,32 +176,23 @@
         }
         if (hitmask) {
             const uint32_t slot = atomicAdd(&s_nrec, 1u);
-            ScreenRec rec; rec.chunk = (uint32_t)c; rec.tid = threadIdx.x; rec.hitmask = hitmask; rec.pad = 0;
+            ScreenRec rec; rec.chunk = (uint32_t)chunk_of(c); rec.tid = threadIdx.x; rec.hitmask = hitmask; rec.pad = 0;
             my_recs[slot] = rec;
         }
     };
 
     u32x4 a[U], b[U]; uint32_t ax[U], bx[U];
     uint64_t c = blockIdx.x;
-    if (c < n_chunks) load(c, a, ax);
+    if (c < n_chunks) load(NT, c, a, ax);
     {
+        stage_lds_table<SCREEN_BLOCK>(s_tab4, reinterpret_cast<const uint4 *>(S.bloom), nb4);
+        if (threadIdx.x == 0) s_nrec = 0;
         const uint4 z = make_uint4(0, 0, 0, 0);
         for (uint64_t i = (uint64_t)blockIdx.x * blockDim.x + threadIdx.x; i < clear_vec4; i += cstep * blockDim.x) clear[i] = z;
-        const uint4 *__restrict__ src = reinterpret_cast<const uint4 *>(S.bloom);
-        for (uint32_t i = threadIdx.x; i < nb4; i += blockDim.x) s_tab4[i] = src[i];
-        if (threadIdx.x == 0) s_nrec = 0;
     }
     __syncthreads();
-    if (c < n_chunks) for (;;) {
-        if (c + cstep >= n_chunks) { stage1(c, a, ax); break; }
-        load(c + cstep, b, bx);
-        stage1(c, a, ax);
-        c += cstep;
-        if (c + cstep >= n_chunks) { stage1(c, b, bx); break; }
-        load(c + cstep, a, ax);
-        stage1(c, b, bx);
-        c += cstep;
-    }
+    sweep_turns(c, cstep, n_chunks, nt_turns, [&](auto nt, uint64_t t) { load(nt, t, a, ax); }, [&](auto nt, uint64_t t) { load(nt, t, b, bx); },
+                [&](uint64_t t) { stage1(t, a, ax); }, [&](uint64_t t) { stage1(t, b, bx); });
     __syncthreads();
     if (threadIdx.x == 0) rec_counts[blockIdx.x] = s_nrec;
 }
@@ -165,7 +210,7 @@
 template <int SPW, int U, bool LDSF, int G = 8, bool PRE = false, int CANON = 0>
 __global__ void __launch_bounds__(1024, G == 8 ? 4 : 8)
 screen2_kernel(ReadsView R, KmerSetView S, ScreenRec *__restrict__ recs, uint32_t rec_cap, uint32_t *__restrict__ rec_counts,
-               uint4 *__restrict__ clear, uint64_t clear_vec4)
+               uint4 *__restrict__ clear, uint64_t clear_vec4, uint32_t rev)
 {
     extern __shared__ uint4 s_tab4[];
     constexpr int NS = U * 4 * SPW;
@@ -180,8 +225,9 @@
     const u32x4 *__restrict__ w4 = reinterpret_cast<const u32x4 *>(R.words);
     const uint4 *__restrict__ f2 = reinterpret_cast<const uint4 *>(S.front2);
     const uint4 *__restrict__ f3 = reinterpret_cast<const uint4 *>(S.front3);
-    const uint64_t chunk = (uint64_t)blockDim.x * U;
-    const uint64_t n_chunks = R.n_vec / chunk;
+    const uint64_t chunk = ScreenChunk<U>::VECS;
+    const uint64_t n_chunks = R.n_vec >> ScreenChunk<U>::LOG2;
+    auto chunk_of = [&](uint64_t c) { return rev ? n_chunks - 1 - c : c; };
     const uint32_t idx_lo = LDSF ? stage1_index_lo(S.s, S.bloom_log2w) : 0u, idx_bits = LDSF ? S.bloom_log2w - 2 : 0u;
     const uint32_t lo2 = stage1_index_lo(S.s, S.f2_log2b + 2), b2 = S.f2_log2b;
     const uint32_t lo3 = stage1_index_lo(S.s, S.f3_log2b + 2), b3 = S.f3_log2b;
@@ -191,14 +237,14 @@
     auto load = [&](uint64_t c, u32x4 (&d)[U], uint32_t (&x)[U]) {
 #pragma unroll
         for (int u = 0; u < U; u++) {
-            const uint64_t v = c * chunk + (uint64_t)u * blockDim.x + threadIdx.x;
+            const uint64_t v = chunk_of(c) * chunk + (uint64_t)u * blockDim.x + threadIdx.x;
             d[u] = __builtin_nontemporal_load(&w4[v]);
             if (SPW == 2) x[u] = R.words[4 * v + 4];
         }
     };
     auto record = [&](uint64_t c, uint32_t mask) {
         const uint32_t slot = atomicAdd(&s_nrec, 1u);
-        ScreenRec rec; rec.chunk = (uint32_t)c; rec.tid = threadIdx.x; rec.hitmask = mask; rec.pad = 0;
+        ScreenRec rec; rec.chunk = (uint32_t)chunk_of(c); rec.tid = threadIdx.x; rec.hitmask = mask; rec.pad = 0;
         my_recs[slot] = rec;
     };
     auto samples = [&](const u32x4 (&d)[U], const uint32_t (&x)[U], uint32_t (&sm)[NS]) {
@@ -316,14 +362,11 @@
     uint64_t c = blockIdx.x;
     if (c < n_chunks) load(c, a, ax);
     {
+        if (LDSF || PRE) stage_lds_table<SCREEN_BLOCK>(s_tab4, reinterpret_cast<const uint4 *>(LDSF ? S.bloom : S.pre), nb4);
+        lds_st(&s_ver[lane], 0u); lds_st(&s_qsm[lane], 0u); lds_st(&s_qid[lane], 0u);
+        if (threadIdx.x == 0) s_nrec = 0;
         const uint4 z = make_uint4(0, 0, 0, 0);
         for (uint64_t i = (uint64_t)blockIdx.x * blockDim.x + threadIdx.x; i < clear_vec4; i += cstep * blockDim.x) clear[i] = z;
-        if (LDSF || PRE) {
-            const uint4 *__restrict__ src = reinterpret_cast<const uint4 *>(LDSF ? S.bloom : S.pre);
-            for (uint32_t i = threadIdx.x; i < nb4; i += blockDim.x) s_tab4[i] = src[i];
-        }
-        lds_st(&s_ver[lane], 0u); lds_st(&s_qsm[lane], 0u); lds_st(&s_qid[lane], 0u);
-        if (threadIdx.x == 0) s_nrec = 0;
     }
     __syncthreads();
     if (c < n_chunks) for (;;) {
@@ -357,7 +400,7 @@
 template <int U, int CANON = 0>
 __global__ void __launch_bounds__(1024)
 screen3_kernel(ReadsView R, KmerSetView S, ScreenRec *__restrict__ recs, uint32_t rec_cap, uint32_t *__restrict__ rec_counts,
-               uint4 *__restrict__ clear, uint64_t clear_vec4)
+               uint4 *__restrict__ clear, uint64_t clear_vec4, uint32_t rev, uint64_t nt_turns)
 {
     extern __shared__ uint4 s_tab4[];
     constexpr int NS = U * 4;
@@ -371,8 +414,9 @@
     lds_u16 *s_qid = (lds_u16 *)(s_qch + S3_QN);
     const u32x4 *__restrict__ w4 = reinterpret_cast<const u32x4 *>(R.words);
     const uint4 *__restrict__ f2 = reinterpret_cast<const uint4 *>(S.front2);
-    const uint64_t chunk = (uint64_t)blockDim.x * U;
-    const uint64_t n_chunks = R.n_vec / chunk;
+    const uint64_t chunk = ScreenChunk<U>::VECS;
+    const uint64_t n_chunks = R.n_vec >> ScreenChunk<U>::LOG2;
+    auto chunk_of = [&](uint64_t c) { return rev ? n_chunks - 1 - c : c; };
     const uint32_t idx_lo = stage1_index_lo(S.s, S.bloom_log2w), idx_bits = S.bloom_log2w - 2;
     const uint32_t lo2 = stage1_index_lo(S.s, S.f2_log2b + 2), b2 = S.f2_log2b;
     const uint64_t cstep = gridDim.x;
@@ -380,9 +424,12 @@
     uint32_t q_n = 0;
     uint32_t e_w = 0, t_w = 0;
 
-    auto load = [&](uint64_t c, u32x4 (&d)[U]) {
-#pragma unroll
-        for (int u = 0; u < U; u++) d[u] = __builtin_nontemporal_load(&w4[c * chunk + (uint64_t)u * blockDim.x + threadIdx.x]);
+    auto load = [&](auto nt, uint64_t c, u32x4 (&d)[U]) {
+#pragma unroll
+        for (int u = 0; u < U; u++) {
+            const u32x4 *p = &w4[chunk_of(c) * chunk + (uint64_t)u * blockDim.x + threadIdx.x];
+            d[u] = decltype(nt)::value ? __builtin_nontemporal_load(p) : *p;
+        }
     };
     auto record = [&](uint32_t c32, uint32_t tid, uint32_t mask) {
         const uint32_t slot = atomicAdd(&s_nrec, 1u);
@@ -421,7 +468,7 @@
             const bool roomy = e_w + 256u <= 64u * t_w;
             const bool single = (hitmask & (hitmask - 1u)) == 0;
             const bool direct = hitmask != 0 && ((hitmask & (hitmask << 1)) != 0 || (!single && !roomy));
-            if (direct) { record((uint32_t)c, threadIdx.x, hitmask); todo = 0; }
+            if (direct) { record((uint32_t)chunk_of(c), threadIdx.x, hitmask); todo = 0; }
             e_w += (uint32_t)__popcll(__builtin_amdgcn_ballot_w64(direct));
         }
         for (;;) {
@@ -432,7 +479,7 @@
                 const uint32_t bit = 31u - (uint32_t)__clz(todo), i = (uint32_t)(NS - 1) - bit;
                 const uint32_t lo = (i & 1u) ? ((i & 2u) ? sm[3] : sm[1]) : ((i & 2u) ? sm[2] : sm[0]);
                 const uint32_t hi = (i & 1u) ? ((i & 2u) ? sm[7] : sm[5]) : ((i & 2u) ? sm[6] : sm[4]);
-                lds_st(&s_qsm[off], (i & 4u) ? hi : lo); lds_st(&s_qch[off], (uint32_t)c); s_qid[off] = (unsigned short)(threadIdx.x | (bit << 10));
+                lds_st(&s_qsm[off], (i & 4u) ? hi : lo); lds_st(&s_qch[off], (uint32_t)chunk_of(c)); s_qid[off] = (unsigned short)(threadIdx.x | (bit << 10));
                 todo &= ~(1u << bit);
             }
             q_n += (uint32_t)__popcll(bm);
@@ -444,25 +491,16 @@
 
     u32x4 a[U], b[U];
     uint64_t c = blockIdx.x;
-    if (c < n_chunks) load(c, a);
+    if (c < n_chunks) load(NT, c, a);
     {
+        stage_lds_table<SCREEN_BLOCK>(s_tab4, reinterpret_cast<const uint4 *>(S.bloom), nb4);
+        if (threadIdx.x == 0) s_nrec = 0;
         const uint4 z = make_uint4(0, 0, 0, 0);
         for (uint64_t i = (uint64_t)blockIdx.x * blockDim.x + threadIdx.x; i < clear_vec4; i += cstep * blockDim.x) clear[i] = z;
-        const uint4 *__restrict__ src = reinterpret_cast<const uint4 *>(S.bloom);
-        for (uint32_t i = threadIdx.x; i < nb4; i += blockDim.x) s_tab4[i] = src[i];
-        if (threadIdx.x == 0) s_nrec = 0;
     }
     __syncthreads();
-    if (c < n_chunks) for (;;) {
-        if (c + cstep >= n_chunks) { stage1(c, a); break; }
-        load(c + cstep, b);
-        stage1(c, a);
-        c += cstep;
-        if (c + cstep >= n_chunks) { stage1(c, b); break; }
-        load(c + cstep, a);
-        stage1(c, b);
-        c += cstep;
-    }
+    sweep_turns(c, cstep, n_chunks, nt_turns, [&](auto nt, uint64_t t) { load(nt, t, a); }, [&](auto nt, uint64_t t) { load(nt, t, b); },
+                [&](uint64_t t) { stage1(t, a); }, [&](uint64_t t) { stage1(t, b); });
     while (q_n) drain();
     __syncthreads();
     if (threadIdx.x == 0) rec_counts[blockIdx.x] = s_nrec;
@@ -771,8 +809,7 @@
     {
         const uint32_t nb4 = (1u << S.kb_log2w) >> 2;
         const uint4 *__restrict__ src = reinterpret_cast<const uint4 *>(S.kbloom);
-        uint4 *dst = s_mem4 + HEAD4;
-        for (uint32_t i = threadIdx.x; i < nb4; i += blockDim.x) dst[i] = src[i];
+        stage_lds_table<BLOCK>(s_mem4 + HEAD4, src, nb4);
     }
     __syncthreads();
     const uint32_t kb_shift = 32 - (S.kb_log2w - 1);
@@ -1556,44 +1593,54 @@
     done.fetch_or(bit, std::memory_order_release);
 }
 
+static uint64_t sweep_nt_turns(uint64_t n_chunks, uint64_t grid, uint64_t tail_bytes)
+{
+    const uint64_t round2 = 2 * grid, chunk_bytes = (uint64_t)SCREEN_BLOCK * SCREEN_U * 16, tail = tail_bytes / chunk_bytes;
+    if (round2 == 0) return 0;
+    const uint64_t lo = n_chunks > tail ? n_chunks - tail : 0;
+    const uint64_t up = (lo + round2 - 1) / round2 * round2, down = n_chunks / round2 * round2;
+    return up < down ? up : down;
+}
+
 template <int SPW, int CANON>
 static void launch_screen_spw(const ReadsView &R, const KmerSetView &S, void *recs, uint32_t *rec_counts, int n_cu, hipStream_t st,
-                              const KernelTiming *tm, uint32_t *clear, uint64_t clear_vec4)
+                              const KernelTiming *tm, uint32_t *clear, uint64_t clear_vec4, bool rev, bool keep_tail)
 {
     const int key = screen_grid_key(S.stride, S.front_mode, S.canon);
     const uint64_t grid = screen_grid_for(R, n_cu, key);
     if (grid == 0) return;
     const uint32_t cap = (uint32_t)screen_rec_cap_for(R, n_cu, key);
+    const uint64_t nt_turns = sweep_nt_turns(R.n_vec / ((uint64_t)SCREEN_BLOCK * SCREEN_U), grid, keep_tail ? SWEEP_KEEP_BYTES : 0);
     if constexpr (SPW == 1) if (S.front_mode == 3) {
         const size_t lds = (sizeof(uint32_t) << S.bloom_log2w) + S3_LDS_EXTRA;
         raise_lds_limit_once<&screen3_kernel<SCREEN_U, CANON>>(128 * 1024 + S3_LDS_EXTRA);
         MF_LAUNCH((screen3_kernel<SCREEN_U, CANON>), dim3((unsigned)grid), dim3(SCREEN_BLOCK), lds, st, tm, R, S,
-                  static_cast<ScreenRec *>(recs), cap, rec_counts, reinterpret_cast<uint4 *>(clear), clear ? clear_vec4 : (uint64_t)0);
+                  static_cast<ScreenRec *>(recs), cap, rec_counts, reinterpret_cast<uint4 *>(clear), clear ? clear_vec4 : (uint64_t)0, (uint32_t)rev, nt_turns);
         return;
     }
     if (S.front_mode == 1 || S.front_mode == 3) {
         const size_t lds = (sizeof(uint32_t) << S.bloom_log2w) + S2_LDS_EXTRA;
         raise_lds_limit_once<&screen2_kernel<SPW, SCREEN_U, true, 8, false, CANON>>(128 * 1024 + S2_LDS_EXTRA);
         MF_LAUNCH((screen2_kernel<SPW, SCREEN_U, true, 8, false, CANON>), dim3((unsigned)grid), dim3(SCREEN_BLOCK), lds, st, tm, R, S,
-                  static_cast<ScreenRec *>(recs), cap, rec_counts, reinterpret_cast<uint4 *>(clear), clear ? clear_vec4 : (uint64_t)0);
+                  static_cast<ScreenRec *>(recs), cap, rec_counts, reinterpret_cast<uint4 *>(clear), clear ? clear_vec4 : (uint64_t)0, (uint32_t)rev);
         return;
     }
     if (S.front_mode == 4) {
         const size_t lds = (sizeof(uint32_t) << S.pre_log2w) + S2_LDS_EXTRA;
         raise_lds_limit_once<&screen2_kernel<SPW, SCREEN_U, false, 8, true, CANON>>(128 * 1024 + S2_LDS_EXTRA);
         MF_LAUNCH((screen2_kernel<SPW, SCREEN_U, false, 8, true, CANON>), dim3((unsigned)grid), dim3(SCREEN_BLOCK), lds, st, tm, R, S,
-                  static_cast<ScreenRec *>(recs), cap, rec_counts, reinterpret_cast<uint4 *>(clear), clear ? clear_vec4 : (uint64_t)0);
+                  static_cast<ScreenRec *>(recs), cap, rec_counts, reinterpret_cast<uint4 *>(clear), clear ? clear_vec4 : (uint64_t)0, (uint32_t)rev);
         return;
     }
     if (S.front_mode == 2) {
         MF_LAUNCH((screen2_kernel<SPW, SCREEN_U, false, 4, false, CANON>), dim3((unsigned)grid), dim3(SCREEN_BLOCK), S2_LDS_EXTRA, st, tm, R, S,
-                  static_cast<ScreenRec *>(recs), cap, rec_counts, reinterpret_cast<uint4 *>(clear), clear ? clear_vec4 : (uint64_t)0);
+                  static_cast<ScreenRec *>(recs), cap, rec_counts, reinterpret_cast<uint4 *>(clear), clear ? clear_vec4 : (uint64_t)0, (uint32_t)rev);
         return;
     }
     const size_t lds1 = (sizeof(uint32_t) << S.bloom_log2w) + 16;
     raise_lds_limit_once<&screen_kernel<SPW, SCREEN_U, CANON>>(128 * 1024 + 16);
     MF_LAUNCH((screen_kernel<SPW, SCREEN_U, CANON>), dim3((unsigned)grid), dim3(SCREEN_BLOCK), lds1, st, tm, R, S,
-              static_cast<ScreenRec *>(recs), cap, rec_counts, reinterpret_cast<uint4 *>(clear), clear ? clear_vec4 : (uint64_t)0);
+              static_cast<ScreenRec *>(recs), cap, rec_counts, reinterpret_cast<uint4 *>(clear), clear ? clear_vec4 : (uint64_t)0, (uint32_t)rev, nt_turns);
 }
 
 template <int SPW>
@@ -1611,13 +1658,13 @@
 }
 
 hipError_t launch_screen(const ReadsView &R, const KmerSetView &S, void *recs, uint32_t *rec_counts, int n_cu, hipStream_t st,
-                         const KernelTiming *tm, uint32_t *clear, uint64_t clear_vec4)
-{
-    if (S.stride == 16 && S.canon == 1) launch_screen_spw<1, 1>(R, S, recs, rec_counts, n_cu, st, tm, clear, clear_vec4);
-    else if (S.stride == 16 && S.canon) launch_screen_spw<1, 2>(R, S, recs, rec_counts, n_cu, st, tm, clear, clear_vec4);
-    else if (S.stride == 16) launch_screen_spw<1, 0>(R, S, recs, rec_counts, n_cu, st, tm, clear, clear_vec4);
-    else if (S.canon) launch_screen_spw<2, 2>(R, S, recs, rec_counts, n_cu, st, tm, clear, clear_vec4);
-    else launch_screen_spw<2, 0>(R, S, recs, rec_counts, n_cu, st, tm, clear, clear_vec4);
+                         const KernelTiming *tm, uint32_t *clear, uint64_t clear_vec4, bool rev, bool keep_tail)
+{
+    if (S.stride == 16 && S.canon == 1) launch_screen_spw<1, 1>(R, S, recs, rec_counts, n_cu, st, tm, clear, clear_vec4, rev, keep_tail);
+    else if (S.stride == 16 && S.canon) launch_screen_spw<1, 2>(R, S, recs, rec_counts, n_cu, st, tm, clear, clear_vec4, rev, keep_tail);
+    else if (S.stride == 16) launch_screen_spw<1, 0>(R, S, recs, rec_counts, n_cu, st, tm, clear, clear_vec4, rev, keep_tail);
+    else if (S.canon) launch_screen_spw<2, 2>(R, S, recs, rec_counts, n_cu, st, tm, clear, clear_vec4, rev, keep_tail);
+    else launch_screen_spw<2, 0>(R, S, recs, rec_counts, n_cu, st, tm, clear, clear_vec4, rev, keep_tail);
     return hipGetLastError();
 }
 
diff --git a/mitoflex_amd/csrc/mf_passplan.h b/mitoflex_amd/csrc/mf_passplan.h
--- a/mitoflex_amd/csrc/mf_passplan.h
+++ b/mitoflex_amd/csrc/mf_passplan.h
@@ -16,6 +16,7 @@
     int prot, s, stride, kw, k, s8_finish;
     unsigned thr; int mode; bool count_all, overlap, more;
     PassFeedback fb; int flip, cur, nsets;
+    int sweep = 0; bool sweep_alternate = false;
 };
 enum class PassKind { PROTEIN, FINISH, SPLIT_PIPELINED, ONE_STREAM };
 enum class PassStream { MAIN, FINISH_A, SCREEN_ALT, FINISH_B };
@@ -24,8 +25,17 @@
     PassStream screen_on = PassStream::MAIN, later_on = PassStream::MAIN;
     bool two_streams = false, wait_prev_finish = false, screen = false, screen_clears_bits = false, needs_cand = false, exact_behind_finish = false, exact_coresident = false;
     int flip = 0, cur = 0; bool sample_pass = false;
+    bool rev = false, keep_tail = false; int sweep = 0;
 };
-inline PassPlan plan_pass(const PassKnobs &kn, const PassInputs &in)
+inline PassPlan plan_sweep(PassPlan p, const PassInputs &in)
+{
+    p.sweep = in.sweep;
+    if (p.screen) { p.rev = in.sweep_alternate && (in.sweep & 1); p.keep_tail = in.sweep_alternate; p.sweep = in.sweep ^ 1; }
+    return p;
+}
+inline PassPlan plan_pass_kind(const PassKnobs &kn, const PassInputs &in);
+inline PassPlan plan_pass(const PassKnobs &kn, const PassInputs &in) { return plan_sweep(plan_pass_kind(kn, in), in); }
+inline PassPlan plan_pass_kind(const PassKnobs &kn, const PassInputs &in)
 {
     PassPlan p; p.flip = in.flip; p.cur = p.q_out = in.cur;
     if (in.prot) { p.kind = PassKind::PROTEIN; return p; }
```

Measured after the change: 161.5 billion. -1.1%, worse.
